# Ruslan361/iterative_solvers

Hardware: AMD Instinct MI355X
Metric: cg_iters_per_sec (higher is better)
Workload: dtype f64; 1 GPU; 4096x4096 L-shaped Dirichlet Poisson fp64, matrix-free CG, fixed 2641 iterations; n=4096, unknowns=12574721, rule=rel2

## Files before the change

### include/mi355cg.h

```cpp
#ifndef MI355CG_H
#define MI355CG_H

#include <stddef.h>

#ifdef __cplusplus
extern "C" {
#endif

#define MI355CG_OK            0
#define MI355CG_ERR_INVALID   1
#define MI355CG_ERR_HIP       2
#define MI355CG_ERR_STATE     3

#define MI355CG_F64           0
#define MI355CG_F32_MIXED     1

#define MI355CG_RULE_MSG_MAXNORM  0
#define MI355CG_RULE_REL_2NORM    1

#define MI355CG_STOP_ITERATIONS   0
#define MI355CG_STOP_PRECISION    1
#define MI355CG_STOP_RESIDUAL     2
#define MI355CG_STOP_EXACT_ERROR  3
#define MI355CG_STOP_INTERRUPTED  4
// ... 3 lines not shown
typedef void (*mi355cg_iter_cb)(void *user, int iteration, double precision, double residual, double error);

typedef struct mi355cg_params {
    int    rule;
    int    max_iterations;
    double eps_precision;
    double eps_residual;
    double eps_exact_error;
    double eps_rel;
    int    use_true_solution;
    int    callback_every;
    int    diagnostics;
    int    sync_every;
    int    fixed_iterations;
    double inner_eps;
} mi355cg_params;

typedef struct mi355cg_results {
    int    iterations;
    int    converged;
    int    stop_reason;
    double final_residual_norm;
    double final_precision;
    double final_error_norm;
    double r_norm2;
    double initial_r_norm2;
    double solve_seconds;
    double refine_true_rel;
    int    refine_outer;
    double loop_seconds;
} mi355cg_results;

int  mi355cg_create(int n, int m, double a, double b, double c, double d,
                    int dtype, int device, mi355cg_handle *out);
int  mi355cg_create_csr(long long nrows, const int *row_map, const int *entries, const double *values,
                        int device, mi355cg_handle *out);
int  mi355cg_set_true_solution(mi355cg_handle h, const double *u);
void mi355cg_destroy(mi355cg_handle h);
const char *mi355cg_last_error(void);
const char *mi355cg_version(void);

long long mi355cg_size(mi355cg_handle h);
int  mi355cg_get_rhs(mi355cg_handle h, double *out);
int  mi355cg_get_true_solution(mi355cg_handle h, double *out);
int  mi355cg_get_node_coords(mi355cg_handle h, double *xs, double *ys);
int  mi355cg_set_rhs(mi355cg_handle h, const double *b);
int  mi355cg_setup_on_device(mi355cg_handle h);

int  mi355cg_apply(mi355cg_handle h, const double *x, double *y);
int  mi355cg_apply_device(mi355cg_handle h, const double *x_dev, double *y_dev);

void mi355cg_default_params(mi355cg_params *p, int rule);
int  mi355cg_solve(mi355cg_handle h, const mi355cg_params *params,
                   mi355cg_iter_cb cb, void *user, const volatile int *stop_flag,
                   mi355cg_results *out);
int  mi355cg_get_solution(mi355cg_handle h, double *x);
int  mi355cg_get_recursive_residual(mi355cg_handle h, double *r);
int  mi355cg_get_true_residual(mi355cg_handle h, double *ax_minus_b);

#define MI355CG_PRECOND_NONE    0
#define MI355CG_PRECOND_MG      1
#define MI355CG_PRECOND_MG_ANY  2
int  mi355cg_set_preconditioner(mi355cg_handle h, int kind);
int  mi355cg_apply_preconditioner(mi355cg_handle h, const double *r, double *z);
int  mi355cg_mg_levels(int n, int *levels, int *coarsest_n);
int  mi355cg_mg_hierarchy(int kind, int n, int max_levels, int *levels, int *level_n);

#define MI355CG_CYCLE_F64 0
#define MI355CG_CYCLE_F32 1
int  mi355cg_set_preconditioner_ex(mi355cg_handle h, int kind, int cycle);
int  mi355cg_preconditioner_info(mi355cg_handle h, int *kind, int *cycle, int *levels);

#define MI355CG_BATCH_MAX 64
int  mi355cg_solve_batch(mi355cg_handle h, const mi355cg_params *params, int nrhs, const double *b, double *x,
                         const volatile int *stop_flag, mi355cg_results *out);
int  mi355cg_solve_batch_device(mi355cg_handle h, const mi355cg_params *params, int nrhs, const double *b_dev, double *x_dev,
                                const volatile int *stop_flag, mi355cg_results *out);
int  mi355cg_batch_release(mi355cg_handle h);

int  mi355cg_set_profiling(mi355cg_handle h, int enable);
int  mi355cg_get_kernel_time(mi355cg_handle h, int kernel, double *avg_ms, long long *launches);
int  mi355cg_get_layout(mi355cg_handle h, long long *padded_len, int *pitch_bottom, int *pitch_upper,
                        int *grid_stencil, int *grid_update, int *rows_per_item);

int  mi355cg_slab_rows(int n, int world, int rank, int *y_lo, int *y_hi);
int  mi355cg_create_part(int n, int m, double a, double b, double c, double d, int dtype, int device,
                         int y_lo, int y_hi, int x_lo, int x_hi, mi355cg_handle *out);
int  mi355cg_checksum(mi355cg_handle h, int which, double *out2);
int  mi355cg_create_slab(int n, int m, double a, double b, double c, double d, int dtype, int device,
                         int y_lo, int y_hi, mi355cg_handle *out);
int  mi355cg_owned_range(mi355cg_handle h, long long *packed_begin, long long *packed_len, int *y_lo, int *y_hi);
int  mi355cg_dist_begin(mi355cg_handle h, const mi355cg_params *params, void *stream);
int  mi355cg_dist_reduce(mi355cg_handle h, int which , int with_rows, void *stream);
int  mi355cg_dist_sums_ptr(mi355cg_handle h, int which, void **dev_ptr, int *count );
int  mi355cg_dist_record_layout(mi355cg_handle h, int *header, int *row_slot, int *width);
int  mi355cg_dist_scatter_ghosts(mi355cg_handle h, int vector ,
                                 const double *gathered_records, int nranks, int rank, void *stream);
int  mi355cg_dist_stencil(mi355cg_handle h, const double *gathered_update_sums, int nranks, int estride,
                          int rows , void *stream);
int  mi355cg_dist_flip(mi355cg_handle h);
int  mi355cg_dist_update(mi355cg_handle h, const double *gathered_stencil_sums, int nranks, int estride,
                         int rows , void *stream);
int  mi355cg_dist_update_reads_ghosts(mi355cg_handle h);
int  mi355cg_dist_check(mi355cg_handle h, const double *gathered_update_sums, int nranks, int estride, void *stream);
int  mi355cg_dist_summary(mi355cg_handle h, mi355cg_results *out, int *done);
int  mi355cg_dist_finish(mi355cg_handle h, void *stream);
int  mi355cg_dist_history(mi355cg_handle h, int iteration, double *precision, double *residual, double *error);
int  mi355cg_dist_halo(mi355cg_handle h, int vector ,
                       void **send_lo, void **recv_lo, long long *n_send_lo,
                       void **send_hi, void **recv_hi, long long *n_send_hi);
int  mi355cg_dist_halo_recv_counts(mi355cg_handle h, long long *n_from_lo, long long *n_from_hi);

#define MI355CG_DECOMP_ROWS 0
#define MI355CG_DECOMP_2D   1
typedef struct mi355cg_team_s *mi355cg_team;
typedef struct mi355cg_halo_msg {
    int id;
    int peer;
    int send;
    int kind;
    int y0, y1, x0, x1;
    long long count;
} mi355cg_halo_msg;
int  mi355cg_decompose(int n, int world, int decomp, int rank, int *y_lo, int *y_hi, int *x_lo, int *x_hi);
int  mi355cg_halo_plan(int n, int world, int decomp, int rank, int max_msgs, int *n_msgs, mi355cg_halo_msg *msgs);
int  mi355cg_debug_plan(int n, int world, int decomp, int rank, int which, int *n_panels, int *panels,
                        int *grid, int *n_items, int *cls);
int  mi355cg_team_create_local(int n, int m, double a, double b, double c, double d, int world,
                               const int *devices, int ndevices, int decomp, mi355cg_team *out);
int  mi355cg_team_unique_id(void *id128);
int  mi355cg_team_create_rccl(int n, int m, double a, double b, double c, double d, int world, int rank, int device,
                              const void *id128, int decomp, mi355cg_team *out);
void mi355cg_team_destroy(mi355cg_team t);
int  mi355cg_team_solve(mi355cg_team t, const mi355cg_params *params, mi355cg_iter_cb cb, void *user,
                        const volatile int *stop_flag, mi355cg_results *out);
int  mi355cg_team_info(mi355cg_team t, int *world, int *nlocal, int *decomp, long long *size);
int  mi355cg_team_describe(mi355cg_team t, char *buf, int len);
int  mi355cg_team_part(mi355cg_team t, int local_index, mi355cg_handle *part, int *rank);
int  mi355cg_team_get_vector(mi355cg_team t, int which, double *global_packed);
int  mi355cg_team_checksum(mi355cg_team t, int which, double *out2);
int  mi355cg_team_set_vector(mi355cg_team t, int which, const double *global_packed);
int  mi355cg_team_set_dtype(mi355cg_team t, int dtype);
int  mi355cg_team_setup_on_device(mi355cg_team t);
int  mi355cg_team_set_profiling(mi355cg_team t, int enable);
int  mi355cg_team_phase_times(mi355cg_team t, double *kernel_ms, double *comm_ms, double *wall_ms);

#ifdef __cplusplus
}
#endif
#endif
```

### iterative_solvers_amd/_capi.py

```python
from __future__ import annotations

import ctypes as C
import os

import numpy as np

from . import build as _build

OK, ERR_INVALID, ERR_HIP, ERR_STATE = 0, 1, 2, 3
F64, F32_MIXED = 0, 1
RULE_MSG_MAXNORM, RULE_REL_2NORM = 0, 1
STOP_ITERATIONS, STOP_PRECISION, STOP_RESIDUAL, STOP_EXACT_ERROR, STOP_INTERRUPTED = range(5)

EXPORTS = [
    "mi355cg_create", "mi355cg_create_csr", "mi355cg_set_true_solution", "mi355cg_destroy", "mi355cg_last_error", "mi355cg_version", "mi355cg_size",
    "mi355cg_get_rhs", "mi355cg_get_true_solution", "mi355cg_get_node_coords", "mi355cg_set_rhs",
    "mi355cg_apply", "mi355cg_apply_device", "mi355cg_default_params", "mi355cg_solve",
    "mi355cg_get_solution", "mi355cg_get_recursive_residual", "mi355cg_get_true_residual",
    "mi355cg_set_profiling", "mi355cg_get_kernel_time", "mi355cg_get_layout",
    "mi355cg_slab_rows", "mi355cg_create_slab", "mi355cg_owned_range", "mi355cg_dist_begin",
    "mi355cg_dist_reduce", "mi355cg_dist_sums_ptr", "mi355cg_dist_record_layout", "mi355cg_dist_scatter_ghosts", "mi355cg_dist_stencil", "mi355cg_dist_flip",
    "mi355cg_dist_update", "mi355cg_dist_update_reads_ghosts", "mi355cg_dist_check", "mi355cg_dist_summary", "mi355cg_dist_finish", "mi355cg_dist_history",
    "mi355cg_dist_halo", "mi355cg_dist_halo_recv_counts",
    "mi355cg_create_part", "mi355cg_checksum", "mi355cg_decompose", "mi355cg_halo_plan",
    "mi355cg_team_create_local", "mi355cg_team_unique_id", "mi355cg_team_create_rccl", "mi355cg_team_destroy",
    "mi355cg_team_solve", "mi355cg_team_info", "mi355cg_team_part", "mi355cg_team_get_vector", "mi355cg_team_set_vector", "mi355cg_team_checksum",
    "mi355cg_team_set_profiling", "mi355cg_team_phase_times", "mi355cg_team_describe", "mi355cg_setup_on_device", "mi355cg_team_setup_on_device", "mi355cg_debug_plan",
    "mi355cg_team_set_dtype", "mi355cg_set_preconditioner", "mi355cg_apply_preconditioner", "mi355cg_mg_levels",
    "mi355cg_mg_hierarchy", "mi355cg_set_preconditioner_ex", "mi355cg_preconditioner_info",
    "mi355cg_solve_batch", "mi355cg_solve_batch_device", "mi355cg_batch_release",
]
DECOMP_ROWS, DECOMP_2D = 0, 1
PRECOND_NONE, PRECOND_MG, PRECOND_MG_ANY = 0, 1, 2
CYCLE_F64, CYCLE_F32 = 0, 1
BATCH_MAX = 64


class Params(C.Structure):
    _fields_ = [("rule", C.c_int), ("max_iterations", C.c_int),
                ("eps_precision", C.c_double), ("eps_residual", C.c_double),
                ("eps_exact_error", C.c_double), ("eps_rel", C.c_double),
                ("use_true_solution", C.c_int), ("callback_every", C.c_int),
                ("diagnostics", C.c_int), ("sync_every", C.c_int), ("fixed_iterations", C.c_int),
                ("inner_eps", C.c_double)]


class Results(C.Structure):
    _fields_ = [("iterations", C.c_int), ("converged", C.c_int), ("stop_reason", C.c_int),
                ("final_residual_norm", C.c_double), ("final_precision", C.c_double),
                ("final_error_norm", C.c_double), ("r_norm2", C.c_double),
                ("initial_r_norm2", C.c_double), ("solve_seconds", C.c_double),
                ("refine_true_rel", C.c_double), ("refine_outer", C.c_int), ("loop_seconds", C.c_double)]


class HaloMsg(C.Structure):
    _fields_ = [("id", C.c_int), ("peer", C.c_int), ("send", C.c_int), ("kind", C.c_int),
                ("y0", C.c_int), ("y1", C.c_int), ("x0", C.c_int), ("x1", C.c_int), ("count", C.c_longlong)]


ITER_CB = C.CFUNCTYPE(None, C.c_void_p, C.c_int, C.c_double, C.c_double, C.c_double)
_DP = np.ctypeslib.ndpointer(dtype=np.float64, flags="C_CONTIGUOUS")

_lib = None


class Mi355cgError(RuntimeError):
    def __init__(self, code: int, text: str):
        super().__init__(f"mi355cg error {code}: {text}")
        self.code = code


def lib_path() -> str:
    return _build.LIB_PATH


def load():
    global _lib
    if _lib is not None:
        return _lib
    path = os.environ.get("MI355CG_LIB") or _build.LIB_PATH
    if path == _build.LIB_PATH and _build.needs_build():
        try:
            _build.build()
        except Exception as e:
            if not os.path.exists(path):
                raise RuntimeError(f"libmi355cg.so is missing and could not be built: {e}") from e
    try:
        import torch
    except ImportError:
        pass
    L = C.CDLL(path)
    H = C.c_void_p
    L.mi355cg_create.argtypes = [C.c_int, C.c_int] + [C.c_double] * 4 + [C.c_int, C.c_int, C.POINTER(H)]
    _IPn = np.ctypeslib.ndpointer(dtype=np.int32, flags="C_CONTIGUOUS")
    L.mi355cg_create_csr.argtypes = [C.c_longlong, _IPn, _IPn, _DP, C.c_int, C.POINTER(H)]
    L.mi355cg_set_true_solution.argtypes = [H, _DP]
    L.mi355cg_destroy.argtypes = [H]
    L.mi355cg_destroy.restype = None
    L.mi355cg_last_error.restype = C.c_char_p
    L.mi355cg_version.restype = C.c_char_p
    L.mi355cg_size.argtypes = [H]
    L.mi355cg_size.restype = C.c_longlong
    for name in ("mi355cg_get_rhs", "mi355cg_get_true_solution", "mi355cg_set_rhs",
                 "mi355cg_get_solution", "mi355cg_get_recursive_residual", "mi355cg_get_true_residual"):
        getattr(L, name).argtypes = [H, _DP]
    L.mi355cg_get_node_coords.argtypes = [H, _DP, _DP]
    L.mi355cg_apply.argtypes = [H, _DP, _DP]
    L.mi355cg_apply_device.argtypes = [H, C.c_void_p, C.c_void_p]
    L.mi355cg_default_params.argtypes = [C.POINTER(Params), C.c_int]
    L.mi355cg_default_params.restype = None
    L.mi355cg_solve.argtypes = [H, C.POINTER(Params), ITER_CB, C.c_void_p, C.c_void_p, C.POINTER(Results)]
    L.mi355cg_set_profiling.argtypes = [H, C.c_int]
    L.mi355cg_get_kernel_time.argtypes = [H, C.c_int, C.POINTER(C.c_double), C.POINTER(C.c_longlong)]
    L.mi355cg_get_layout.argtypes = [H, C.POINTER(C.c_longlong)] + [C.POINTER(C.c_int)] * 5
    LLP, IP, VPP = C.POINTER(C.c_longlong), C.POINTER(C.c_int), C.POINTER(C.c_void_p)
    L.mi355cg_slab_rows.argtypes = [C.c_int, C.c_int, C.c_int, IP, IP]
    L.mi355cg_create_slab.argtypes = [C.c_int, C.c_int] + [C.c_double] * 4 + [C.c_int] * 4 + [C.POINTER(H)]
    L.mi355cg_owned_range.argtypes = [H, LLP, LLP, IP, IP]
    L.mi355cg_dist_begin.argtypes = [H, C.POINTER(Params), C.c_void_p]
    L.mi355cg_dist_reduce.argtypes = [H, C.c_int, C.c_int, C.c_void_p]
    L.mi355cg_dist_sums_ptr.argtypes = [H, C.c_int, VPP, IP]
    L.mi355cg_dist_record_layout.argtypes = [H, IP, IP, IP]
    L.mi355cg_dist_scatter_ghosts.argtypes = [H, C.c_int, C.c_void_p, C.c_int, C.c_int, C.c_void_p]
    L.mi355cg_dist_stencil.argtypes = [H, C.c_void_p, C.c_int, C.c_int, C.c_int, C.c_void_p]
    L.mi355cg_dist_flip.argtypes = [H]
    L.mi355cg_dist_update.argtypes = [H, C.c_void_p, C.c_int, C.c_int, C.c_int, C.c_void_p]
    L.mi355cg_dist_update_reads_ghosts.argtypes = [H]
    L.mi355cg_dist_check.argtypes = [H, C.c_void_p, C.c_int, C.c_int, C.c_void_p]
    L.mi355cg_dist_summary.argtypes = [H, C.POINTER(Results), IP]
    L.mi355cg_dist_finish.argtypes = [H, C.c_void_p]
    DBP = C.POINTER(C.c_double)
    L.mi355cg_dist_history.argtypes = [H, C.c_int, DBP, DBP, DBP]
    L.mi355cg_dist_halo.argtypes = [H, C.c_int, VPP, VPP, LLP, VPP, VPP, LLP]
    L.mi355cg_dist_halo_recv_counts.argtypes = [H, LLP, LLP]
    L.mi355cg_create_part.argtypes = [C.c_int, C.c_int] + [C.c_double] * 4 + [C.c_int] * 6 + [C.POINTER(H)]
    L.mi355cg_checksum.argtypes = [H, C.c_int, DBP]
    L.mi355cg_decompose.argtypes = [C.c_int] * 4 + [IP] * 4
    L.mi355cg_halo_plan.argtypes = [C.c_int] * 5 + [IP, C.POINTER(HaloMsg)]
    L.mi355cg_team_create_local.argtypes = [C.c_int, C.c_int] + [C.c_double] * 4 + [C.c_int, IP, C.c_int, C.c_int, C.POINTER(H)]
    L.mi355cg_team_unique_id.argtypes = [C.c_void_p]
    L.mi355cg_team_create_rccl.argtypes = [C.c_int, C.c_int] + [C.c_double] * 4 + [C.c_int, C.c_int, C.c_int, C.c_void_p, C.c_int, C.POINTER(H)]
    L.mi355cg_team_destroy.argtypes = [H]
    L.mi355cg_team_destroy.restype = None
    L.mi355cg_team_solve.argtypes = [H, C.POINTER(Params), ITER_CB, C.c_void_p, C.c_void_p, C.POINTER(Results)]
    L.mi355cg_team_info.argtypes = [H, IP, IP, IP, LLP]
    L.mi355cg_team_part.argtypes = [H, C.c_int, C.POINTER(H), IP]
    L.mi355cg_team_get_vector.argtypes = [H, C.c_int, _DP]
    L.mi355cg_team_set_vector.argtypes = [H, C.c_int, _DP]
    L.mi355cg_team_checksum.argtypes = [H, C.c_int, DBP]
    L.mi355cg_debug_plan.argtypes = [C.c_int] * 5 + [IP, IP, IP, IP, IP]
    L.mi355cg_setup_on_device.argtypes = [H]
    L.mi355cg_team_setup_on_device.argtypes = [H]
    L.mi355cg_team_set_dtype.argtypes = [H, C.c_int]
    L.mi355cg_team_set_profiling.argtypes = [H, C.c_int]
    L.mi355cg_team_phase_times.argtypes = [H, DBP, DBP, DBP]
    L.mi355cg_team_describe.argtypes = [H, C.c_char_p, C.c_int]
    L.mi355cg_set_preconditioner.argtypes = [H, C.c_int]
    L.mi355cg_set_preconditioner_ex.argtypes = [H, C.c_int, C.c_int]
    L.mi355cg_preconditioner_info.argtypes = [H, IP, IP, IP]
    L.mi355cg_apply_preconditioner.argtypes = [H, _DP, _DP]
    L.mi355cg_mg_levels.argtypes = [C.c_int, IP, IP]
    L.mi355cg_mg_hierarchy.argtypes = [C.c_int, C.c_int, C.c_int, IP, IP]
    L.mi355cg_solve_batch.argtypes = [H, C.POINTER(Params), C.c_int, C.c_void_p, C.c_void_p, C.c_void_p, C.POINTER(Results)]
    L.mi355cg_solve_batch_device.argtypes = [H, C.POINTER(Params), C.c_int, C.c_void_p, C.c_void_p, C.c_void_p, C.POINTER(Results)]
    L.mi355cg_batch_release.argtypes = [H]
    _lib = L
    return L


def check(rc: int):
    if rc != OK:
        raise Mi355cgError(rc, load().mi355cg_last_error().decode("utf-8", "replace"))
```

### iterative_solvers_amd/csrc/cg_kernels.h

```cpp
#pragma once
#include <hip/hip_runtime.h>
#include <cfloat>
#include <cmath>

namespace mi355cg {

constexpr int kBlock = 256;
constexpr int kWave = 64;
constexpr int kWaves = kBlock / kWave;
constexpr int kHist = 512;
constexpr int kMaxPanels = 8;
constexpr int kRing = 8;

#ifdef MI355CG_WAVE_TIMING
constexpr int kWtWaves = 16384, kWtStamps = 6;
__device__ unsigned long long g_wave_dbg[2][kWtStamps * kWtWaves];
#define MI355CG_WT_BEGIN unsigned long long wt_[kWtStamps]; for (int i_ = 0; i_ < kWtStamps; ++i_) wt_[i_] = 0; wt_[0] = wall_clock64();
#define MI355CG_WT_STAMP(I) wt_[I] = wall_clock64();
#define MI355CG_WT_MID wt_[kWtStamps - 2] = wall_clock64();
#define MI355CG_WT_END(K) do { if ((threadIdx.x & 63) == 0) { const int w_ = blockIdx.x * 4 + threadIdx.x / 64; \
    if (w_ < kWtWaves) { wt_[kWtStamps - 1] = wall_clock64(); for (int i_ = 0; i_ < kWtStamps; ++i_) g_wave_dbg[K][kWtStamps * w_ + i_] = wt_[i_]; } } } while (0)
#else
#define MI355CG_WT_BEGIN
#define MI355CG_WT_STAMP(I)
// ... 63 lines not shown
struct RuleParams {
    int rule;
    int max_iterations;
    double eps_precision, eps_residual, eps_exact_error, eps_rel;
    int use_u;
    int fixed_iterations;
};

enum { FA_PAP = 0, FA_RZ = 1, FA_LO = 2, FA_COUNT = 4 };
enum { FB_RR = 0, FB_D2 = 1, FB_E2 = 2, FB_LO = 3, FB_RMAX = 6, FB_DMAX = 7, FB_EMAX = 8, FB_COUNT = 9 };
constexpr int kNumSumsA = 2, kNumSumsB = 3;
constexpr int FB_STOP = FB_COUNT, FB_LL_COUNT = FB_COUNT + 1;

struct dd { double hi, lo; };
__device__ inline dd dd_zero() { return dd{0.0, 0.0}; }
__device__ inline dd two_sum(double a, double b) { const double s = a + b, bb = s - a; return dd{s, (a - (s - bb)) + (b - bb)}; }
__device__ inline dd dd_add(dd a, dd b) {
    const dd s = two_sum(a.hi, b.hi);
    const double lo = s.lo + (a.lo + b.lo);
    const double hi = s.hi + lo;
    return dd{hi, lo - (hi - s.hi)};
}
__device__ inline void dd_acc_prod(dd& acc, double a, double b) {
#ifdef MI355CG_PLAIN_DOT
    acc.hi += a * b;
#elif defined(MI355CG_DOT2)
    const double p = a * b;
    const dd s = two_sum(acc.hi, p);
    acc.hi = s.hi;
    acc.lo += s.lo + fma(a, b, -p);
#else
    const double p = a * b;
    acc = dd_add(acc, dd{p, fma(a, b, -p)});
#endif
}
__device__ inline double dd_value(dd a) { return a.hi + a.lo; }

__device__ inline double wave_sum(double v) {
#pragma unroll
    for (int o = 32; o > 0; o >>= 1) v += __shfl_down(v, o, kWave);
    return v;
}
__device__ inline double wave_max(double v) {
#pragma unroll
    for (int o = 32; o > 0; o >>= 1) v = fmax(v, __shfl_down(v, o, kWave));
    return v;
}
template <bool IS_MAX>
__device__ inline double block_reduce(double v, double* lds ) {
    v = IS_MAX ? wave_max(v) : wave_sum(v);
    const int lane = threadIdx.x & (kWave - 1), w = threadIdx.x / kWave;
    __syncthreads();
    if (lane == 0) lds[w] = v;
    __syncthreads();
    double t = lds[0];
#pragma unroll
    for (int k = 1; k < kWaves; ++k) t = IS_MAX ? fmax(t, lds[k]) : t + lds[k];
    return t;
}
template <bool IS_MAX>
__device__ inline double reduce_parts(const double* __restrict__ part, int n, int es, double* lds) {
    double v = 0.0;
    for (int i = threadIdx.x; i < n; i += kBlock) v = IS_MAX ? fmax(v, part[(long long)i * es]) : v + part[(long long)i * es];
    return block_reduce<IS_MAX>(v, lds);
}

__device__ inline dd wave_sum_dd(dd v) {
#pragma unroll
    for (int o = 32; o > 0; o >>= 1) v = dd_add(v, dd{__shfl_down(v.hi, o, kWave), __shfl_down(v.lo, o, kWave)});
    return v;
}
__device__ inline dd block_reduce_dd(dd v, double* lds) {
    v = wave_sum_dd(v);
    const int lane = threadIdx.x & (kWave - 1), w = threadIdx.x / kWave;
    __syncthreads();
    if (lane == 0) { lds[2 * w] = v.hi; lds[2 * w + 1] = v.lo; }
    __syncthreads();
    dd t{lds[0], lds[1]};
#pragma unroll
    for (int k = 1; k < kWaves; ++k) t = dd_add(t, dd{lds[2 * k], lds[2 * k + 1]});
    return t;
}
struct PreParts { double hi0, lo0, hi1, lo1; };
__device__ inline PreParts prefetch_parts(const double* __restrict__ part_hi, const double* __restrict__ part_lo, int n, int es) {
    PreParts p{0.0, 0.0, 0.0, 0.0};
    const int i0 = threadIdx.x, i1 = threadIdx.x + kBlock;
    if (i0 < n) { p.hi0 = part_hi[(long long)i0 * es]; p.lo0 = part_lo[(long long)i0 * es]; }
    if (i1 < n) { p.hi1 = part_hi[(long long)i1 * es]; p.lo1 = part_lo[(long long)i1 * es]; }
    return p;
}
__device__ inline dd reduce_parts_dd_pre(const PreParts& pre, const double* __restrict__ part_hi, const double* __restrict__ part_lo, int n, int es, double* lds) {
    dd v = dd_zero();
    if ((int)threadIdx.x < n) v = dd_add(v, dd{pre.hi0, pre.lo0});
    if ((int)threadIdx.x + kBlock < n) v = dd_add(v, dd{pre.hi1, pre.lo1});
    for (int i = threadIdx.x + 2 * kBlock; i < n; i += kBlock) v = dd_add(v, dd{part_hi[(long long)i * es], part_lo[(long long)i * es]});
    return block_reduce_dd(v, lds);
}
struct PreMax { double v0, v1; };
__device__ inline PreMax prefetch_max(const double* __restrict__ part, int n, int es) {
    PreMax p{0.0, 0.0};
    if ((int)threadIdx.x < n) p.v0 = part[(long long)threadIdx.x * es];
    if ((int)threadIdx.x + kBlock < n) p.v1 = part[(long long)(threadIdx.x + kBlock) * es];
    return p;
}
template <bool IS_MAX> __device__ inline double block_reduce(double v, double* lds);
__device__ inline double reduce_max_pre(const PreMax& pre, const double* __restrict__ part, int n, int es, double* lds) {
    double v = fmax(pre.v0, pre.v1);
    for (int i = threadIdx.x + 2 * kBlock; i < n; i += kBlock) v = fmax(v, part[(long long)i * es]);
    return block_reduce<true>(v, lds);
}
__device__ inline dd reduce_parts_dd(const double* __restrict__ part_hi, const double* __restrict__ part_lo, int n, int es, double* lds) {
    dd v = dd_zero();
    for (int i = threadIdx.x; i < n; i += kBlock) v = dd_add(v, dd{part_hi[(long long)i * es], part_lo[(long long)i * es]});
    return block_reduce_dd(v, lds);
}

struct Decision { int done, reason, converged; double beta, rr, rnorm2, r0norm, rmax, dmax, emax, d2, e2; };

__device__ inline Decision decide_after_update(const StateLite& s, const RuleParams& rp, double rr, double rmax,
                                               double dmax, double emax, double d2, double e2, bool stop = false) {
    Decision d;
    d.rr = rr; d.rnorm2 = sqrt(rr); d.rmax = rmax; d.dmax = dmax; d.emax = emax; d.d2 = d2; d.e2 = e2;
    d.r0norm = s.first ? d.rnorm2 : s.r0norm;
    d.done = 0; d.reason = 0 ; d.converged = 0; d.beta = 0.0;
    if (rp.rule == 1 ) {
        const bool go = s.it < rp.max_iterations && (rp.fixed_iterations || d.rnorm2 > rp.eps_rel * d.r0norm);
        if (!go) { d.done = 1; d.converged = d.rnorm2 <= rp.eps_rel * d.r0norm; }
        if (!s.first) d.beta = rr / s.rr;
    } else {
        if (s.it >= 1 && !rp.fixed_iterations) {
            if (rp.eps_precision > 0 && dmax < rp.eps_precision) { d.done = 1; d.converged = 1; d.reason = 1; }
            else if (rp.eps_residual > 0 && rmax < rp.eps_residual) { d.done = 1; d.converged = 1; d.reason = 2; }
            else if (rp.eps_exact_error > 0 && rp.use_u && emax < rp.eps_exact_error) { d.done = 1; d.converged = 1; d.reason = 3; }
        }
        if (!d.done && !(s.it < rp.max_iterations)) d.done = 1;
        if (!s.first) d.beta = (d.rnorm2 * d.rnorm2) / s.rz;
    }
    if (!d.done && (stop || s.stop)) { d.done = 1; d.reason = 4 ; d.converged = 0; }
    return d;
}

__device__ inline void write_state_after_decision(CgState* out, HistEntry* hist, const CgState* in, const StateLite& s, const Decision& d) {
    copy_state(out, in);
    CgState* o = out;
    o->rr_prev = s.rr; o->rr = d.rr; o->rnorm2 = d.rnorm2; o->r0norm = d.r0norm; o->beta = d.beta;
    o->rmax = d.rmax; o->dmax = d.dmax; o->emax = d.emax; o->d2 = d.d2; o->e2 = d.e2;
    o->done = d.done; o->reason = d.reason; o->converged = d.converged;
    if (hist) {
        HistEntry* h = hist + (s.it % kHist);
        h->dmax = d.dmax; h->rmax = d.rmax; h->emax = d.emax; h->rnorm2 = d.rnorm2; h->d2 = d.d2; h->e2 = d.e2;
    }
}

__device__ inline Decision reduce_and_decide(const StateLite& s, const RuleParams& rp, const double* partB,
                                             int nB, int strideB, int esB, int want_diag, double* lds, const PreParts* pre_rr = nullptr,
                                             const PreMax* pre_max = nullptr ) {
    const double rr = pre_rr ? dd_value(reduce_parts_dd_pre(*pre_rr, partB + FB_RR * strideB, partB + (FB_RR + FB_LO) * strideB, nB, esB, lds))
                             : dd_value(reduce_parts_dd(partB + FB_RR * strideB, partB + (FB_RR + FB_LO) * strideB, nB, esB, lds));
    double rmax = 0, dmax = 0, emax = 0, d2 = 0, e2 = 0;
    if (rp.rule == 0 || want_diag) {
        if (pre_max) {
            rmax = reduce_max_pre(pre_max[0], partB + FB_RMAX * strideB, nB, esB, lds);
            dmax = reduce_max_pre(pre_max[1], partB + FB_DMAX * strideB, nB, esB, lds);
            if (rp.use_u) emax = reduce_max_pre(pre_max[2], partB + FB_EMAX * strideB, nB, esB, lds);
        } else {
            rmax = reduce_parts<true>(partB + FB_RMAX * strideB, nB, esB, lds);
            dmax = reduce_parts<true>(partB + FB_DMAX * strideB, nB, esB, lds);
            if (rp.use_u) emax = reduce_parts<true>(partB + FB_EMAX * strideB, nB, esB, lds);
        }
    }
    if (want_diag) {
        d2 = dd_value(reduce_parts_dd(partB + FB_D2 * strideB, partB + (FB_D2 + FB_LO) * strideB, nB, esB, lds));
        if (rp.use_u) e2 = dd_value(reduce_parts_dd(partB + FB_E2 * strideB, partB + (FB_E2 + FB_LO) * strideB, nB, esB, lds));
    }
    return decide_after_update(s, rp, rr, rmax, dmax, emax, d2, e2);
}
typedef unsigned long long u64;
constexpr int kRecWords = 16;
// ... 125 lines not shown
    }
    if (a.which == 1) {
#pragma unroll
        for (int k = 0; k < 4; ++k) {
            const double t = block_reduce<true>(mx[k], lds);
            if (threadIdx.x == 0) rec[k < 3 ? FB_RMAX + k : kRecStopWord] = t;
        }
    }
    __syncthreads();
    publish_record(rec, a.rs);
}

__device__ inline Decision decide_from_records(const StateLite& s, const RuleParams& rp, const double* recs, int world, bool use_max, bool want_diag) {
    dd rr = dd_zero(), d2 = dd_zero(), e2 = dd_zero();
    double rmax = 0, dmax = 0, emax = 0, stop = 0;
    for (int j = 0; j < world; ++j) {
        const double* R = recs + j * kRecWords;
        rr = dd_add(rr, dd{R[FB_RR], R[FB_RR + FB_LO]});
        d2 = dd_add(d2, dd{R[FB_D2], R[FB_D2 + FB_LO]});
        e2 = dd_add(e2, dd{R[FB_E2], R[FB_E2 + FB_LO]});
        rmax = fmax(rmax, R[FB_RMAX]); dmax = fmax(dmax, R[FB_DMAX]); emax = fmax(emax, R[FB_EMAX]);
        stop = fmax(stop, R[kRecStopWord]);
    }
    if (!use_max) { rmax = 0; dmax = 0; emax = 0; }
    if (!rp.use_u) { emax = 0; e2 = dd_zero(); }
    if (!want_diag) { d2 = dd_zero(); e2 = dd_zero(); }
    return decide_after_update(s, rp, dd_value(rr), rmax, dmax, emax, dd_value(d2), dd_value(e2), stop > 0.0);
}
__device__ inline void alpha_from_records(const StateLite& s, int rule, const double* recs, int world, double* alpha, double* rz_out) {
    dd pap = dd_zero(), rz = dd_zero();
    for (int j = 0; j < world; ++j) {
        const double* R = recs + j * kRecWords;
        pap = dd_add(pap, dd{R[FA_PAP], R[FA_PAP + FA_LO]});
        rz = dd_add(rz, dd{R[FA_RZ], R[FA_RZ + FA_LO]});
    }
    if (rule == 0) { *rz_out = dd_value(rz); *alpha = *rz_out / dd_value(pap); }
    else { *rz_out = 0.0; *alpha = s.rr / dd_value(pap); }
}
__device__ inline void own_record_B(double* recs, int me, const double* partB, int nB, int strideB, int level, double* lds,
                                    const PreParts* pre_rr = nullptr, const PreMax* pre_max = nullptr) {
    double* R = recs + me * kRecWords;
    if (threadIdx.x < kRecWords) R[threadIdx.x] = 0.0;
    const dd rr = pre_rr ? reduce_parts_dd_pre(*pre_rr, partB + FB_RR * strideB, partB + (FB_RR + FB_LO) * strideB, nB, 1, lds)
                         : reduce_parts_dd(partB + FB_RR * strideB, partB + (FB_RR + FB_LO) * strideB, nB, 1, lds);
    double rmax = 0, dmax = 0, emax = 0;
    dd d2 = dd_zero(), e2 = dd_zero();
    if (level >= 1) {
        if (pre_max) {
            rmax = reduce_max_pre(pre_max[0], partB + FB_RMAX * strideB, nB, 1, lds);
            dmax = reduce_max_pre(pre_max[1], partB + FB_DMAX * strideB, nB, 1, lds);
            emax = reduce_max_pre(pre_max[2], partB + FB_EMAX * strideB, nB, 1, lds);
        } else {
            rmax = reduce_parts<true>(partB + FB_RMAX * strideB, nB, 1, lds);
            dmax = reduce_parts<true>(partB + FB_DMAX * strideB, nB, 1, lds);
            emax = reduce_parts<true>(partB + FB_EMAX * strideB, nB, 1, lds);
        }
    }
    if (level >= 2) {
        d2 = reduce_parts_dd(partB + FB_D2 * strideB, partB + (FB_D2 + FB_LO) * strideB, nB, 1, lds);
        e2 = reduce_parts_dd(partB + FB_E2 * strideB, partB + (FB_E2 + FB_LO) * strideB, nB, 1, lds);
    }
    __syncthreads();
    if (threadIdx.x == 0) {
        R[FB_RR] = rr.hi; R[FB_RR + FB_LO] = rr.lo; R[FB_D2] = d2.hi; R[FB_D2 + FB_LO] = d2.lo; R[FB_E2] = e2.hi; R[FB_E2 + FB_LO] = e2.lo;
        R[FB_RMAX] = rmax; R[FB_DMAX] = dmax; R[FB_EMAX] = emax;
    }
}
__device__ inline void fail_transport(CgState* out, const CgState* in) {
    copy_state(out, in);
    out->done = 1; out->reason = kReasonTransport; out->converged = 0;
}

constexpr int kQueueSubs = 8;
constexpr int kQueuePitch = 64;
struct QueueSpec {
    int* mine;
    int* other;
};
__device__ inline int queue_take(int* q, int lane) {
    int v = 0;
    if (lane == 0) v = __hip_atomic_fetch_add(q, 1, __ATOMIC_RELAXED, __HIP_MEMORY_SCOPE_AGENT);
    return v;
}

template <typename T>
struct StencilArgs {
    Geom g;
    WorkList wl;
    const T* r;
    const T* pin;
    T* pout;
    T* ap;
    const double* partB; int nB, strideB, esB;
    RecSrc src;
    double* partA; int strideA, slotA;
    const CgState* s_in; CgState* s_out;
    HistEntry* hist;
    RuleParams rp;
    int want_diag;
    int store_ghosts;
    FlagSpec fl;
    QueueSpec dq;
};

template <typename T, int VEC> struct VecOf { typedef T type __attribute__((ext_vector_type(VEC))); };

constexpr int kOob = (int)0x80000000;
typedef __amdgpu_buffer_rsrc_t rsrc_t;
__device__ inline rsrc_t make_rsrc(const void* base) {
    return __builtin_amdgcn_make_buffer_rsrc(const_cast<void*>(base), 0, 0x7fffffff, 0x00020000);
}
template <typename V> __device__ inline V buf_load(rsrc_t r, int voff, int soff) {
    if constexpr (sizeof(V) == 16) return __builtin_bit_cast(V, __builtin_amdgcn_raw_buffer_load_b128(r, voff, soff, 0));
    else if constexpr (sizeof(V) == 8) return __builtin_bit_cast(V, __builtin_amdgcn_raw_buffer_load_b64(r, voff, soff, 0));
    else { static_assert(sizeof(V) == 4, "buf_load: 4, 8 or 16 bytes"); return __builtin_bit_cast(V, __builtin_amdgcn_raw_buffer_load_b32(r, voff, soff, 0)); }
}
template <typename V> __device__ inline void buf_store(V v, rsrc_t r, int voff, int soff) {
    typedef unsigned int u4 __attribute__((ext_vector_type(4)));
    typedef unsigned int u2 __attribute__((ext_vector_type(2)));
    if constexpr (sizeof(V) == 16) {
        u4 d = __builtin_bit_cast(u4, v);
        __builtin_amdgcn_raw_buffer_store_b128(d, r, voff, soff, 0);
        asm volatile("s_nop 1" : "+v"(d));
    }
    else if constexpr (sizeof(V) == 8) __builtin_amdgcn_raw_buffer_store_b64(__builtin_bit_cast(u2, v), r, voff, soff, 0);
    else { static_assert(sizeof(V) == 4, "buf_store: 4, 8 or 16 bytes"); __builtin_amdgcn_raw_buffer_store_b32(__builtin_bit_cast(unsigned int, v), r, voff, soff, 0); }
}
__device__ inline int dpp_from_below(int v) { return __builtin_amdgcn_update_dpp(0, v, 0x138 , 0xf, 0xf, false); }
__device__ inline int dpp_from_above(int v) { return __builtin_amdgcn_update_dpp(0, v, 0x130 , 0xf, 0xf, false); }
__device__ inline float lane_below(float v) { return __builtin_bit_cast(float, dpp_from_below(__builtin_bit_cast(int, v))); }
__device__ inline float lane_above(float v) { return __builtin_bit_cast(float, dpp_from_above(__builtin_bit_cast(int, v))); }
__device__ inline double lane_below(double v) {
    const unsigned long long u = __builtin_bit_cast(unsigned long long, v);
    const unsigned lo = (unsigned)dpp_from_below((int)(unsigned)u), hi = (unsigned)dpp_from_below((int)(unsigned)(u >> 32));
    return __builtin_bit_cast(double, ((unsigned long long)hi << 32) | lo);
}
__device__ inline double lane_above(double v) {
    const unsigned long long u = __builtin_bit_cast(unsigned long long, v);
    const unsigned lo = (unsigned)dpp_from_above((int)(unsigned)u), hi = (unsigned)dpp_from_above((int)(unsigned)(u >> 32));
    return __builtin_bit_cast(double, ((unsigned long long)hi << 32) | lo);
}
template <typename T> __device__ inline int row_step(const Geom& g, int y) { return (y + 1 <= g.half ? g.Pb : g.Pu) * (int)sizeof(T); }

template <typename T> __device__ inline int lane_off(const Geom& g, int x, bool bottom_row) {
    return (x < g.xlim && x >= (bottom_row ? g.cb : 0)) ? x * (int)sizeof(T) : kOob;
}
template <typename T, int VEC> __device__ inline int edge_off(const Geom& g, int x, int lane, bool bottom_row) {
    const int xe = lane == 0 ? x - 1 : x + VEC;
    const bool edge = lane == 0 || lane == kWave - 1;
    return (edge && xe >= (bottom_row ? g.cb : 0) && xe < g.xlim) ? xe * (int)sizeof(T) : kOob;
}

struct Item { int strip, ya, yb, gc; };
__device__ inline Item decode_item(const WorkList& wl, int item) {
    Panel P = wl.p[0];
#pragma unroll
    for (int k = 1; k < kMaxPanels; ++k) if (k < wl.np && item >= wl.p[k].item0) P = wl.p[k];
    const int local = item - P.item0;
    const int chunk = local / P.ns;
    Item it;
    it.strip = P.s0 + (local - chunk * P.ns);
    it.ya = P.y0 + chunk * P.ty;
    it.yb = min(P.y1, it.ya + P.ty - 1);
    it.gc = (it.strip == P.s0 ? (P.gc & 1) : 0) | (it.strip == P.s0 + P.ns - 1 ? (P.gc & 2) : 0);
    return it;
}

struct ItemAddr {
    int nrows, ystart;
    long long base_el;
    int so_first, so_c0;
    int gc; bool bot;
    int x;
    int vo_own, ve_own, vo_first, vo_last;
};
template <typename T, int VEC, bool DESC>
__device__ inline ItemAddr item_addr(const Geom& g, const Item& it, int lane) {
    constexpr int DIR = DESC ? -1 : 1;
    ItemAddr A;
    A.x = it.strip * (kWave * VEC) + lane * VEC;
    A.nrows = it.yb - it.ya + 1;
    A.ystart = DESC ? it.yb : it.ya;
    const int y0 = it.ya - 1;
    A.base_el = row_off(g, y0) - g.base0;
    A.bot = it.ya <= g.half;
    A.vo_own = lane_off<T>(g, A.x, A.bot);
    A.ve_own = edge_off<T, VEC>(g, A.x, lane, A.bot);
    A.vo_first = lane_off<T>(g, A.x, A.ystart - DIR <= g.half);
    A.vo_last = lane_off<T>(g, A.x, A.ystart + DIR * A.nrows <= g.half);
    A.so_first = DESC ? (int)((row_off(g, it.yb + 1) - row_off(g, y0)) * (long long)sizeof(T)) : 0;
    A.so_c0 = DESC ? (int)((row_off(g, it.yb) - row_off(g, y0)) * (long long)sizeof(T)) : row_step<T>(g, y0);
    A.gc = it.gc;
    return A;
}

template <typename T, int VEC, bool FUSED, bool MSG, int DEPTH, bool NOAP, bool GC>
__global__ __launch_bounds__(kBlock) void k_stencil(const StencilArgs<T> a) {
    static_assert(DEPTH >= 1 && DEPTH <= 3, "the compute cursor takes its item from the fetch cursor: DEPTH <= rows fetched per item (>= 3)");
    typedef typename VecOf<T, VEC>::type vec_t;
    __shared__ double lds[2 * kWaves];
    const Geom& g = a.g;
    const int lane = threadIdx.x & (kWave - 1);
    const int wave = __builtin_amdgcn_readfirstlane(threadIdx.x / kWave);
    const ItemSeq seq = item_seq(a.wl, wave);
    MI355CG_WT_BEGIN
    struct Raw { vec_t r, p; T re, pe; };

    int f_item = seq.first;
    bool f_have = f_item < seq.end;
    ItemAddr F{};
    int f_idx = 0, f_so = 0, f_y = 0;
    rsrc_t rs_p = make_rsrc(a.pin), rs_r = make_rsrc(a.pin);
    const int dq_nsub = min(kQueueSubs, (int)(gridDim.x / kXcds)), dq_sub = (int)(blockIdx.x / kXcds) % dq_nsub;
    int* const dq = a.dq.mine ? a.dq.mine + ((int)(blockIdx.x % kXcds) * kQueueSubs + dq_sub) * kQueuePitch : nullptr;
    if (a.dq.other && blockIdx.x == 0 && threadIdx.x < kXcds * kQueueSubs) a.dq.other[threadIdx.x * kQueuePitch] = 0;
    int dq_ticket = 0;
    auto enter = [&](int item) {
        if (dq) dq_ticket = queue_take(dq, lane);
        F = item_addr<T, VEC, false>(g, decode_item(a.wl, item), lane);
        rs_p = make_rsrc(a.pin + F.base_el);
        rs_r = make_rsrc(FUSED ? a.r + F.base_el : a.pin + F.base_el);
        f_idx = -1; f_so = F.so_first; f_y = F.ystart - 1;
    };
    auto fetch = [&]() -> Raw {
        if (f_have && f_idx > F.nrows) {
            f_item = dq ? seq.begin + seq.step + __builtin_amdgcn_readfirstlane(dq_ticket) * dq_nsub + dq_sub : f_item + seq.step;
            f_have = f_item < seq.end;
            if (f_have) enter(f_item);
        }
        const bool own = f_idx >= 0 && f_idx < F.nrows;
        int vo = own ? F.vo_own : (f_idx < 0 ? F.vo_first : F.vo_last);
        int ve = own ? F.ve_own : kOob;
        if (!f_have) { vo = kOob; ve = kOob; }
        Raw w;
        w.p = buf_load<vec_t>(rs_p, vo, f_so);
        if (FUSED) w.r = buf_load<vec_t>(rs_r, vo, f_so);
        else for (int j = 0; j < VEC; ++j) w.r[j] = (T)0;
        w.pe = buf_load<T>(rs_p, ve, f_so);
        if (FUSED) w.re = buf_load<T>(rs_r, ve, f_so); else w.re = (T)0;
        f_so += row_step<T>(g, f_y); ++f_y; ++f_idx;
        return w;
    };

    bool c_have = f_have;
    ItemAddr C{};
    int c_idx = -1, c_so = 0, c_y = 0, c_ve_gc = kOob;
    bool in_j[VEC];
#pragma unroll
    for (int j = 0; j < VEC; ++j) in_j[j] = false;
    rsrc_t rs_po = make_rsrc(a.pin), rs_ap = make_rsrc(a.pin);
    auto promote = [&]() {
        C = F;
        rs_po = make_rsrc(FUSED ? a.pout + C.base_el : a.pin + C.base_el);
        rs_ap = make_rsrc(NOAP ? a.pin + C.base_el : a.ap + C.base_el);
        c_idx = -1; c_so = C.so_c0; c_y = C.ystart;
        const int xint0 = C.bot ? g.half + 1 : 1;
#pragma unroll
        for (int j = 0; j < VEC; ++j) in_j[j] = (C.x + j >= xint0) && (C.x + j <= g.N - 1);
        if (GC) c_ve_gc = ((lane == 0 && (C.gc & 1)) || (lane == kWave - 1 && (C.gc & 2))) ? C.ve_own : kOob;
    };

    if (f_have) { enter(f_item); promote(); }
    Raw q[DEPTH];
#pragma unroll
    for (int k = 0; k < DEPTH; ++k) q[k] = fetch();

    T beta = (T)0;
    if (FUSED && a.src.mbox) {
        __shared__ double recs[kMaxRecDst * kRecWords];
        const PreParts pre = prefetch_parts(a.partB + FB_RR * a.strideB, a.partB + (FB_RR + FB_LO) * a.strideB, a.nB, 1);
        PreMax pmax[3] = {{0, 0}, {0, 0}, {0, 0}};
        if (MSG) {
#pragma unroll
            for (int k = 0; k < 3; ++k) pmax[k] = prefetch_max(a.partB + (FB_RMAX + k) * a.strideB, a.nB, 1);
        }
        const StateLite s = load_state_lite(a.s_in);
        if (s.done) {
            if (threadIdx.x == 0) { store_flagged_zero(a.fl, a.slotA + blockIdx.x, FA_COUNT); if (blockIdx.x == 0) copy_state(a.s_out, a.s_in); }
            return;
        }
        MI355CG_WT_STAMP(1)
        own_record_B(recs, a.src.me, a.partB, a.nB, a.strideB, MSG ? 1 : 0, lds, &pre, MSG ? pmax : nullptr);
        if (!gather_records(a.src, recs)) {
            if (threadIdx.x == 0) { store_flagged_zero(a.fl, a.slotA + blockIdx.x, FA_COUNT); if (blockIdx.x == 0) fail_transport(a.s_out, a.s_in); }
            return;
        }
        const Decision d = decide_from_records(s, a.rp, recs, a.src.world, MSG, false);
        MI355CG_WT_STAMP(2)
        if (blockIdx.x == 0 && threadIdx.x == 0) write_state_after_decision(a.s_out, a.hist, a.s_in, s, d);
        if (d.done) { if (threadIdx.x == 0) store_flagged_zero(a.fl, a.slotA + blockIdx.x, FA_COUNT); return; }
        beta = (T)d.beta;
    } else if (FUSED) {
        const PreParts pre = prefetch_parts(a.partB + FB_RR * a.strideB, a.partB + (FB_RR + FB_LO) * a.strideB, a.nB, a.esB);
        PreMax pmax[3] = {{0, 0}, {0, 0}, {0, 0}};
        if (MSG) {
#pragma unroll
            for (int k = 0; k < 3; ++k) pmax[k] = prefetch_max(a.partB + (FB_RMAX + k) * a.strideB, a.nB, a.esB);
        }
        const StateLite s = load_state_lite(a.s_in);
        if (s.done) { if (blockIdx.x == 0 && threadIdx.x == 0) copy_state(a.s_out, a.s_in); return; }
        MI355CG_WT_STAMP(1)
        const Decision d = reduce_and_decide(s, a.rp, a.partB, a.nB, a.strideB, a.esB, a.want_diag, lds, &pre, MSG ? pmax : nullptr);
        MI355CG_WT_STAMP(2)
        if (blockIdx.x == 0 && threadIdx.x == 0) write_state_after_decision(a.s_out, a.hist, a.s_in, s, d);
        if (d.done) return;
        beta = (T)d.beta;
    }

    MI355CG_WT_MID
    const T cA = (T)g.A, cxk = (T)g.xk, cyk = (T)g.yk;
    dd acc_pap = dd_zero(), acc_rz = dd_zero();
    auto is_ghost = [&](int yy) { return (yy == g.y_lo - 1 || yy == g.y_hi + 1) && yy >= 1 && yy <= g.N - 1; };
    vec_t pn_b, pn_c, r_c;
    T pne_c = (T)0;
#pragma unroll
    for (int j = 0; j < VEC; ++j) { pn_b[j] = (T)0; pn_c[j] = (T)0; r_c[j] = (T)0; }

    while (c_have) {
#pragma unroll
        for (int k = 0; k < DEPTH; ++k) {
            if (c_have) {
                const Raw w = q[k];
                q[k] = fetch();
                vec_t pn; T pne;
                if (FUSED) {
#pragma unroll
                    for (int j = 0; j < VEC; ++j) pn[j] = w.r[j] + beta * w.p[j];
                    pne = w.re + beta * w.pe;
                } else { pn = w.p; pne = w.pe; }

                if (c_idx < 0) {
                    pn_b = pn;
                    if (FUSED && a.store_ghosts && is_ghost(C.ystart - 1)) buf_store(pn, rs_po, C.vo_first, C.so_first);
                } else if (c_idx == 0) {
                    pn_c = pn; pne_c = pne; r_c = w.r;
                } else {
                    T left0 = lane_below(pn_c[VEC - 1]);
                    T rightL = lane_above(pn_c[0]);
                    if (lane == 0) left0 = pne_c;
                    if (lane == kWave - 1) rightL = pne_c;
                    vec_t out;
#pragma unroll
                    for (int j = 0; j < VEC; ++j) {
                        const T c = pn_c[j];
                        const T L = j == 0 ? left0 : pn_c[j - 1];
                        const T R = j == VEC - 1 ? rightL : pn_c[j + 1];
                        T v = cA * c;
                        v = v + cxk * L;
                        v = v + cxk * R;
                        v = v + cyk * pn[j];
                        v = v + cyk * pn_b[j];
                        out[j] = in_j[j] ? v : (T)0;
                        dd_acc_prod(acc_pap, (double)c, (double)out[j]);
                        if (MSG) dd_acc_prod(acc_rz, (double)r_c[j], (double)c);
                    }
                    if (!NOAP) buf_store(out, rs_ap, C.vo_own, c_so);
                    if (FUSED) buf_store(pn_c, rs_po, C.vo_own, c_so);
                    if (FUSED && GC) buf_store(pne_c, rs_po, c_ve_gc, c_so);
                    c_so += row_step<T>(g, c_y); ++c_y;
                    pn_b = pn_c; pn_c = pn; pne_c = pne; r_c = w.r;
                }
                if (c_idx == C.nrows) {
                    if (FUSED && a.store_ghosts && is_ghost(c_y)) buf_store(pn, rs_po, C.vo_last, c_so);
                    c_have = f_have;
                    if (c_have) promote();
                } else ++c_idx;
            }
        }
    }

    MI355CG_WT_END(0);
    const dd tp = block_reduce_dd(acc_pap, lds);
    dd tz = dd_zero();
    if (MSG) tz = block_reduce_dd(acc_rz, lds);
    if (threadIdx.x == 0 && a.partA) {
        const int b = a.slotA + blockIdx.x, st = a.strideA;
        a.partA[FA_PAP * st + b] = tp.hi; a.partA[(FA_PAP + FA_LO) * st + b] = tp.lo;
        a.partA[FA_RZ * st + b] = tz.hi;  a.partA[(FA_RZ + FA_LO) * st + b] = tz.lo;
        if (FUSED && a.fl.part) { const double v[FA_COUNT] = {tp.hi, tz.hi, tp.lo, tz.lo}; store_flagged(a.fl, b, FA_COUNT, v); }
    }
}

template <typename T>
struct UpdateArgs {
    long long begin, nvec;
    T* x; T* r; const T* p; const T* ap; const T* u;
    const double* partA; int nA, strideA, esA;
    double* partB; int strideB;
    const CgState* s_in; CgState* s_out;
    int rule;
    int init;
    double r0norm_resume;
};

template <typename T, int VEC, bool HAS_U>
__global__ __launch_bounds__(kBlock) void k_update(const UpdateArgs<T> a) {
    typedef typename VecOf<T, VEC>::type vec_t;
    __shared__ double lds[2 * kWaves];
    StateLite s{};
    double alpha_d = 0.0, rz = 0.0;
    if (a.init == 1) {
        s.first = 1; s.it = 0;
    } else if (a.init == 2) {
        s = load_state_lite(a.s_in);
    } else {
        s = load_state_lite(a.s_in);
        if (s.done) { if (blockIdx.x == 0 && threadIdx.x == 0) copy_state(a.s_out, a.s_in); return; }
        const double pap = dd_value(reduce_parts_dd(a.partA + FA_PAP * a.strideA, a.partA + (FA_PAP + FA_LO) * a.strideA, a.nA, a.esA, lds));
        if (a.rule == 0) {
            rz = dd_value(reduce_parts_dd(a.partA + FA_RZ * a.strideA, a.partA + (FA_RZ + FA_LO) * a.strideA, a.nA, a.esA, lds));
            alpha_d = rz / pap;
        } else {
            alpha_d = s.rr / pap;
        }
    }
    const T alpha = (T)alpha_d;

    dd s_rr = dd_zero(), s_d2 = dd_zero(), s_e2 = dd_zero();
    double s_rmax = 0, s_dmax = 0, s_emax = 0;
    const long long stride = (long long)gridDim.x * kBlock;
    vec_t* __restrict__ X = reinterpret_cast<vec_t*>(a.x);
    vec_t* __restrict__ R = reinterpret_cast<vec_t*>(a.r);
    const vec_t* __restrict__ Pp = reinterpret_cast<const vec_t*>(a.p);
    const vec_t* __restrict__ Q = reinterpret_cast<const vec_t*>(a.ap);
    const vec_t* __restrict__ Uu = reinterpret_cast<const vec_t*>(a.u);

    auto elem = [&](long long i, const vec_t& x0, const vec_t& pv, const vec_t& r0, const vec_t& qv, const vec_t& uv) {
        vec_t xn, rn;
#pragma unroll
        for (int j = 0; j < VEC; ++j) {
            xn[j] = x0[j] + alpha * pv[j];
            rn[j] = r0[j] - alpha * qv[j];
            const double rd = (double)rn[j];
            dd_acc_prod(s_rr, rd, rd);
            s_rmax = fmax(s_rmax, fabs(rd));
            const double dx = (double)(xn[j] - x0[j]);
            s_dmax = fmax(s_dmax, fabs(dx));
            dd_acc_prod(s_d2, dx, dx);
            if (HAS_U) {
                const double ee = (double)(xn[j] - uv[j]);
                s_emax = fmax(s_emax, fabs(ee));
                dd_acc_prod(s_e2, ee, ee);
            }
        }
        X[i] = xn; R[i] = rn;
    };
    long long i = a.begin + (long long)blockIdx.x * kBlock + threadIdx.x;
    const long long end = a.begin + a.nvec;
    for (; i + stride < end; i += 2 * stride) {
        const long long j0 = i, j1 = i + stride;
        const vec_t xa = X[j0], pa = Pp[j0], ra = R[j0], qa = Q[j0];
        const vec_t xb = X[j1], pb = Pp[j1], rb = R[j1], qb = Q[j1];
        vec_t ua{}, ub{}; if (HAS_U) { ua = Uu[j0]; ub = Uu[j1]; }
        elem(j0, xa, pa, ra, qa, ua);
        elem(j1, xb, pb, rb, qb, ub);
    }
    if (i < end) {
        const vec_t x0 = X[i], pv = Pp[i], r0 = R[i], qv = Q[i];
        vec_t uv{}; if (HAS_U) uv = Uu[i];
        elem(i, x0, pv, r0, qv, uv);
    }

    const dd t_rr = block_reduce_dd(s_rr, lds);
// ... 16 lines not shown
            } else {
                copy_state(a.s_out, a.s_in);
                if (a.init == 2) {
                    if (s.done) o->rr = s.rr_prev;
                    o->done = 0; o->reason = 0; o->converged = 0; o->alpha = 0.0; o->r0norm = a.r0norm_resume;
                    for (int i = 0; i < kRing; ++i) o->alpha_hist[i] = 0.0;
                } else { o->it = s.it + 1; o->first = 0; o->alpha = alpha_d; o->rz = rz; o->alpha_hist[(s.it + 1) & (kRing - 1)] = alpha_d; }
            }
        }
    }
}

template <typename T>
struct FreshArgs {
    long long begin, nvec;
    const T* b; T* x; T* r; T* p0; const T* u;
    double* partB; int strideB;
    CgState* s_out;
};
template <typename T, int VEC, bool HAS_U>
__global__ __launch_bounds__(kBlock) void k_init_fresh(const FreshArgs<T> a) {
    typedef typename VecOf<T, VEC>::type vec_t;
    __shared__ double lds[2 * kWaves];
    dd s_rr = dd_zero(), s_e2 = dd_zero();
    double s_rmax = 0, s_emax = 0;
    const long long stride = (long long)gridDim.x * kBlock;
    const vec_t* __restrict__ B = reinterpret_cast<const vec_t*>(a.b);
    const vec_t* __restrict__ Uu = reinterpret_cast<const vec_t*>(a.u);
    vec_t* __restrict__ X = reinterpret_cast<vec_t*>(a.x);
    vec_t* __restrict__ R = reinterpret_cast<vec_t*>(a.r);
    vec_t* __restrict__ P = reinterpret_cast<vec_t*>(a.p0);
    vec_t zero;
#pragma unroll
    for (int j = 0; j < VEC; ++j) zero[j] = (T)0;
    const long long end = a.begin + a.nvec;
    for (long long i = a.begin + (long long)blockIdx.x * kBlock + threadIdx.x; i < end; i += stride) {
        const vec_t bv = B[i];
        vec_t uv; if (HAS_U) uv = Uu[i];
#pragma unroll
        for (int j = 0; j < VEC; ++j) {
            const double rd = (double)bv[j];
            dd_acc_prod(s_rr, rd, rd);
            s_rmax = fmax(s_rmax, fabs(rd));
            if (HAS_U) {
                const double ee = (double)((T)0 - uv[j]);
                s_emax = fmax(s_emax, fabs(ee));
                dd_acc_prod(s_e2, ee, ee);
            }
        }
        X[i] = zero; R[i] = bv; P[i] = zero;
    }
    const dd t_rr = block_reduce_dd(s_rr, lds);
    const double t_rmax = block_reduce<true>(s_rmax, lds);
    double t_emax = 0; dd t_e2 = dd_zero();
    if (HAS_U) { t_emax = block_reduce<true>(s_emax, lds); t_e2 = block_reduce_dd(s_e2, lds); }
    if (threadIdx.x == 0) {
        const int b = blockIdx.x, st = a.strideB;
        a.partB[FB_RR * st + b] = t_rr.hi; a.partB[(FB_RR + FB_LO) * st + b] = t_rr.lo;
        a.partB[FB_D2 * st + b] = 0.0; a.partB[(FB_D2 + FB_LO) * st + b] = 0.0;
        a.partB[FB_E2 * st + b] = t_e2.hi; a.partB[(FB_E2 + FB_LO) * st + b] = t_e2.lo;
        a.partB[FB_RMAX * st + b] = t_rmax; a.partB[FB_DMAX * st + b] = 0.0; a.partB[FB_EMAX * st + b] = t_emax;
        if (blockIdx.x == 0) { *a.s_out = CgState{}; a.s_out->first = 1; }
    }
}

template <typename T>
struct UpdateStArgs {
    Geom g;
    WorkList wl;
    const T* p;
    const T* pprev[kRing - 1];
    T* r; T* x; const T* u;
    const double* partA; int nA, strideA, esA;
    RecSrc src;
    double* partB; int strideB, slotB;
    const CgState* s_in; CgState* s_out;
    int rule;
    int reverse;
    const int* stop_req;
    FlagSpec fl;
    QueueSpec dq;
};

template <typename T, int VEC, int XM, bool HAS_U, int DEPTH, bool DESC>
__global__ __launch_bounds__(kBlock) void k_update_st(const UpdateStArgs<T> a) {
    static_assert(DEPTH >= 1 && DEPTH <= 3, "see k_stencil");
    typedef typename VecOf<T, VEC>::type vec_t;
    __shared__ double lds[2 * kWaves];
    const Geom& g = a.g;
    const int lane = threadIdx.x & (kWave - 1);
    const int wave = __builtin_amdgcn_readfirstlane(threadIdx.x / kWave);
    const ItemSeq seq = item_seq(a.wl, wave);
    MI355CG_WT_BEGIN
    int stop_word = 0;
    if (blockIdx.x == 0 && a.stop_req) stop_word = scalar_load(a.stop_req);
    constexpr bool FULL = XM == 1;
    constexpr int NP = XM >= 2 ? XM - 1 : 0;
    struct Raw { vec_t p, r, x, u, pp[NP > 0 ? NP : 1]; T pe; };

    int f_item = seq.first;
    bool f_have = f_item < seq.end;
    ItemAddr F{};
    int f_idx = 0, f_so = 0, f_y = 0;
    rsrc_t rs_p = make_rsrc(a.p), rs_r = rs_p, rs_x = rs_p, rs_u = rs_p;
    rsrc_t rs_pp[NP > 0 ? NP : 1] = {rs_p};
    const int dq_nsub = min(kQueueSubs, (int)(gridDim.x / kXcds)), dq_sub = (int)(blockIdx.x / kXcds) % dq_nsub;
    int* const dq = a.dq.mine ? a.dq.mine + ((int)(blockIdx.x % kXcds) * kQueueSubs + dq_sub) * kQueuePitch : nullptr;
    if (a.dq.other && blockIdx.x == 0 && threadIdx.x < kXcds * kQueueSubs) a.dq.other[threadIdx.x * kQueuePitch] = 0;
    int dq_ticket = 0;
    auto enter = [&](int idx) {
        if (dq) dq_ticket = queue_take(dq, lane);
        F = item_addr<T, VEC, DESC>(g, decode_item(a.wl, a.reverse ? seq.end - 1 - (idx - seq.begin) : idx), lane);
        rs_p = make_rsrc(a.p + F.base_el);
        rs_r = make_rsrc(a.r + F.base_el);
        rs_x = make_rsrc(XM != 0 ? a.x + F.base_el : a.p + F.base_el);
#pragma unroll
        for (int i = 0; i < NP; ++i) rs_pp[i] = make_rsrc(a.pprev[i] + F.base_el);
        rs_u = make_rsrc((FULL && HAS_U) ? a.u + F.base_el : a.p + F.base_el);
        f_idx = -1; f_so = F.so_first; f_y = DESC ? F.ystart + 1 : F.ystart - 1;
    };
    auto fetch = [&]() -> Raw {
        if (f_have && f_idx > F.nrows) {
            f_item = dq ? seq.begin + seq.step + __builtin_amdgcn_readfirstlane(dq_ticket) * dq_nsub + dq_sub : f_item + seq.step;
            f_have = f_item < seq.end;
            if (f_have) enter(f_item);
        }
        const bool own = f_have && f_idx >= 0 && f_idx < F.nrows;
        int vo = own ? F.vo_own : (f_idx < 0 ? F.vo_first : F.vo_last);
        if (!f_have) vo = kOob;
        const int vown = own ? F.vo_own : kOob;
        Raw w;
        w.p = buf_load<vec_t>(rs_p, vo, f_so);
        w.r = buf_load<vec_t>(rs_r, vown, f_so);
        if (XM != 0) w.x = buf_load<vec_t>(rs_x, vown, f_so);
#pragma unroll
        for (int i = 0; i < NP; ++i) w.pp[i] = buf_load<vec_t>(rs_pp[i], vown, f_so);
        if (FULL && HAS_U) w.u = buf_load<vec_t>(rs_u, vown, f_so);
        w.pe = buf_load<T>(rs_p, own ? F.ve_own : kOob, f_so);
        if (DESC) { f_so -= row_step<T>(g, f_y - 1); --f_y; } else { f_so += row_step<T>(g, f_y); ++f_y; }
        ++f_idx;
        return w;
    };

    bool c_have = f_have;
    ItemAddr C{};
    int c_idx = -1, c_so = 0, c_y = 0;
    bool in_j[VEC];
#pragma unroll
    for (int j = 0; j < VEC; ++j) in_j[j] = false;
    rsrc_t rs_ro = rs_p, rs_xo = rs_p;
    auto promote = [&]() {
        C = F;
        rs_ro = make_rsrc(a.r + C.base_el);
        rs_xo = make_rsrc(XM != 0 ? a.x + C.base_el : a.p + C.base_el);
        c_idx = -1; c_so = C.so_c0; c_y = C.ystart;
        const int xint0 = C.bot ? g.half + 1 : 1;
#pragma unroll
        for (int j = 0; j < VEC; ++j) in_j[j] = (C.x + j >= xint0) && (C.x + j <= g.N - 1);
    };

    if (f_have) { enter(f_item); promote(); }
    Raw q[DEPTH];
#pragma unroll
    for (int k = 0; k < DEPTH; ++k) q[k] = fetch();

    double alpha_d, rz = 0.0;
    StateLite s;
    if (a.src.mbox) {
        __shared__ double recs[kMaxRecDst * kRecWords];
        const PreParts pre = prefetch_parts(a.partA + FA_PAP * a.strideA, a.partA + (FA_PAP + FA_LO) * a.strideA, a.nA, 1);
        PreParts pre_rz{0, 0, 0, 0};
        if (FULL) pre_rz = prefetch_parts(a.partA + FA_RZ * a.strideA, a.partA + (FA_RZ + FA_LO) * a.strideA, a.nA, 1);
        s = load_state_lite(a.s_in);
        if (s.done) {
            if (threadIdx.x == 0) { store_flagged_zero(a.fl, a.slotB + blockIdx.x, FB_LL_COUNT); if (blockIdx.x == 0) copy_state(a.s_out, a.s_in); }
            return;
        }
        {
            double* R = recs + a.src.me * kRecWords;
            if (threadIdx.x < kRecWords) R[threadIdx.x] = 0.0;
            const dd pap = reduce_parts_dd_pre(pre, a.partA + FA_PAP * a.strideA, a.partA + (FA_PAP + FA_LO) * a.strideA, a.nA, 1, lds);
            dd rzd = dd_zero();
            if (a.rule == 0) rzd = FULL ? reduce_parts_dd_pre(pre_rz, a.partA + FA_RZ * a.strideA, a.partA + (FA_RZ + FA_LO) * a.strideA, a.nA, 1, lds)
                                        : reduce_parts_dd(a.partA + FA_RZ * a.strideA, a.partA + (FA_RZ + FA_LO) * a.strideA, a.nA, 1, lds);
            __syncthreads();
            if (threadIdx.x == 0) { R[FA_PAP] = pap.hi; R[FA_PAP + FA_LO] = pap.lo; R[FA_RZ] = rzd.hi; R[FA_RZ + FA_LO] = rzd.lo; }
        }
        if (!gather_records(a.src, recs)) {
            if (threadIdx.x == 0) { store_flagged_zero(a.fl, a.slotB + blockIdx.x, FB_LL_COUNT); if (blockIdx.x == 0) fail_transport(a.s_out, a.s_in); }
            return;
        }
        alpha_from_records(s, a.rule, recs, a.src.world, &alpha_d, &rz);
    } else {
        const PreParts pre = prefetch_parts(a.partA + FA_PAP * a.strideA, a.partA + (FA_PAP + FA_LO) * a.strideA, a.nA, a.esA);
        PreParts pre_rz{0, 0, 0, 0};
        if (FULL) pre_rz = prefetch_parts(a.partA + FA_RZ * a.strideA, a.partA + (FA_RZ + FA_LO) * a.strideA, a.nA, a.esA);
        s = load_state_lite(a.s_in);
        if (s.done) { if (blockIdx.x == 0 && threadIdx.x == 0) copy_state(a.s_out, a.s_in); return; }
        const double pap = dd_value(reduce_parts_dd_pre(pre, a.partA + FA_PAP * a.strideA, a.partA + (FA_PAP + FA_LO) * a.strideA, a.nA, a.esA, lds));
        if (a.rule == 0) {
            rz = FULL ? dd_value(reduce_parts_dd_pre(pre_rz, a.partA + FA_RZ * a.strideA, a.partA + (FA_RZ + FA_LO) * a.strideA, a.nA, a.esA, lds))
                      : dd_value(reduce_parts_dd(a.partA + FA_RZ * a.strideA, a.partA + (FA_RZ + FA_LO) * a.strideA, a.nA, a.esA, lds));
            alpha_d = rz / pap;
        } else {
            alpha_d = s.rr / pap;
        }
    }
    const T alpha = (T)alpha_d;
    MI355CG_WT_MID
    T aprev[NP > 0 ? NP : 1] = {(T)0};
#pragma unroll
    for (int i = 0; i < NP; ++i) aprev[i] = (T)scalar_load(&a.s_in->alpha_hist[(s.it - i) & (kRing - 1)]);
    const T cA = (T)g.A, cxk = (T)g.xk, cyk = (T)g.yk;
    dd s_rr = dd_zero(), s_d2 = dd_zero(), s_e2 = dd_zero();
    double s_rmax = 0, s_dmax = 0, s_emax = 0;
    vec_t p_b;
    Raw c;
#pragma unroll
    for (int j = 0; j < VEC; ++j) { p_b[j] = (T)0; c.p[j] = (T)0; c.r[j] = (T)0; c.x[j] = (T)0; c.u[j] = (T)0; for (int i = 0; i < (NP > 0 ? NP : 1); ++i) c.pp[i][j] = (T)0; }
    c.pe = (T)0;

    while (c_have) {
#pragma unroll
        for (int k = 0; k < DEPTH; ++k) {
            if (c_have) {
                const Raw w = q[k];
                q[k] = fetch();
                if (c_idx < 0) {
                    p_b = w.p;
                } else if (c_idx == 0) {
                    c = w;
                } else {
                    T left0 = lane_below(c.p[VEC - 1]);
                    T rightL = lane_above(c.p[0]);
                    if (lane == 0) left0 = c.pe;
                    if (lane == kWave - 1) rightL = c.pe;
                    const vec_t& top = DESC ? p_b : w.p;
                    const vec_t& bot = DESC ? w.p : p_b;
                    vec_t rn, xn;
#pragma unroll
                    for (int j = 0; j < VEC; ++j) {
                        const T cc = c.p[j];
                        const T L = j == 0 ? left0 : c.p[j - 1];
                        const T R = j == VEC - 1 ? rightL : c.p[j + 1];
                        T v = cA * cc;
                        v = v + cxk * L;
                        v = v + cxk * R;
                        v = v + cyk * top[j];
                        v = v + cyk * bot[j];
                        const T apj = in_j[j] ? v : (T)0;
                        rn[j] = c.r[j] - alpha * apj;
                        const double rd = (double)rn[j];
                        dd_acc_prod(s_rr, rd, rd);
                        s_rmax = fmax(s_rmax, fabs(rd));
                        if (XM >= 2) {
                            T t = c.x[j];
#pragma unroll
                            for (int i = NP - 1; i >= 0; --i) t = t + aprev[i] * c.pp[i][j];
                            xn[j] = t + alpha * cc;
                        }
                        if (FULL) {
                            xn[j] = c.x[j] + alpha * cc;
                            const double dx = (double)(xn[j] - c.x[j]);
                            s_dmax = fmax(s_dmax, fabs(dx));
                            dd_acc_prod(s_d2, dx, dx);
                            if (HAS_U) {
                                const double ee = (double)(xn[j] - c.u[j]);
                                s_emax = fmax(s_emax, fabs(ee));
                                dd_acc_prod(s_e2, ee, ee);
                            }
                        }
                    }
                    buf_store(rn, rs_ro, C.vo_own, c_so);
                    if (XM != 0) buf_store(xn, rs_xo, C.vo_own, c_so);
                    if (DESC) { c_so -= row_step<T>(g, c_y - 1); --c_y; } else { c_so += row_step<T>(g, c_y); ++c_y; }
                    p_b = c.p; c = w;
                }
                if (c_idx == C.nrows) {
                    c_have = f_have;
                    if (c_have) promote();
                } else ++c_idx;
            }
        }
    }

    MI355CG_WT_END(1);
    const dd t_rr = block_reduce_dd(s_rr, lds);
    const double t_rmax = block_reduce<true>(s_rmax, lds);
    double t_dmax = 0, t_emax = 0; dd t_d2 = dd_zero(), t_e2 = dd_zero();
    if (FULL) { t_dmax = block_reduce<true>(s_dmax, lds); t_d2 = block_reduce_dd(s_d2, lds); }
    if (FULL && HAS_U) { t_emax = block_reduce<true>(s_emax, lds); t_e2 = block_reduce_dd(s_e2, lds); }
    if (threadIdx.x == 0) {
        const int b = a.slotB + blockIdx.x, st = a.strideB;
        a.partB[FB_RR * st + b] = t_rr.hi; a.partB[(FB_RR + FB_LO) * st + b] = t_rr.lo;
        a.partB[FB_D2 * st + b] = t_d2.hi; a.partB[(FB_D2 + FB_LO) * st + b] = t_d2.lo;
        a.partB[FB_E2 * st + b] = t_e2.hi; a.partB[(FB_E2 + FB_LO) * st + b] = t_e2.lo;
        a.partB[FB_RMAX * st + b] = t_rmax; a.partB[FB_DMAX * st + b] = t_dmax; a.partB[FB_EMAX * st + b] = t_emax;
        if (a.fl.part) {
            const double v[FB_LL_COUNT] = {t_rr.hi, t_d2.hi, t_e2.hi, t_rr.lo, t_d2.lo, t_e2.lo, t_rmax, t_dmax, t_emax, (blockIdx.x == 0 && stop_word) ? 1.0 : 0.0};
            store_flagged(a.fl, b, FB_LL_COUNT, v);
        }
        if (blockIdx.x == 0) {
            copy_state(a.s_out, a.s_in);
            CgState* o = a.s_out;
            o->it = s.it + 1; o->first = 0; o->alpha = alpha_d; o->rz = rz; o->alpha_hist[(s.it + 1) & (kRing - 1)] = alpha_d;
            o->stop = stop_word != 0;
        }
    }
}

struct CheckArgs {
    const double* partB; int nB, strideB, esB;
    RecSrc src;
    const CgState* s_in;
    CgState* summary;
    HistEntry* hist;
    RuleParams rp;
    int want_diag;
};
__global__ __launch_bounds__(kBlock) void k_check(const CheckArgs a) {
    __shared__ double lds[2 * kWaves];
    const StateLite s = load_state_lite(a.s_in);
    if (s.done) { if (threadIdx.x == 0) copy_state(a.summary, a.s_in); return; }
    Decision d;
    if (a.src.mbox) {
        __shared__ double recs[kMaxRecDst * kRecWords];
        own_record_B(recs, a.src.me, a.partB, a.nB, a.strideB, 2, lds);
        if (!gather_records(a.src, recs)) { if (threadIdx.x == 0) fail_transport(a.summary, a.s_in); return; }
        d = decide_from_records(s, a.rp, recs, a.src.world, true, true);
    } else d = reduce_and_decide(s, a.rp, a.partB, a.nB, a.strideB, a.esB, 1, lds);
    if (threadIdx.x == 0) write_state_after_decision(a.summary, a.hist, a.s_in, s, d);
}

template <typename T> struct FlushArgs { const T* p[kRing - 1]; T a[kRing - 1]; int n; };
template <typename T, int VEC>
__global__ __launch_bounds__(kBlock) void k_flush_x(const Geom g, const WorkList wl, T* x, const FlushArgs<T> f) {
    typedef typename VecOf<T, VEC>::type vec_t;
    const int lane = threadIdx.x & (kWave - 1);
    const int wave = __builtin_amdgcn_readfirstlane(threadIdx.x / kWave);
    for (int item = blockIdx.x * kWaves + wave; item < wl.nitems; item += gridDim.x * kWaves) {
        const Item it = decode_item(wl, item);
        const int x0 = it.strip * (kWave * VEC) + lane * VEC;
        if (x0 < (it.ya <= g.half ? g.cb : 0) || x0 >= g.xlim) continue;
        for (int y = it.ya; y <= it.yb; ++y) {
            const long long off = row_off(g, y) - g.base0 + x0;
            vec_t xn = *reinterpret_cast<const vec_t*>(x + off);
#pragma unroll
            for (int k = 0; k < kRing - 1; ++k) if (k < f.n) {
                const vec_t pv = *reinterpret_cast<const vec_t*>(f.p[k] + off);
#pragma unroll
                for (int j = 0; j < VEC; ++j) xn[j] = xn[j] + f.a[k] * pv[j];
            }
            *reinterpret_cast<vec_t*>(x + off) = xn;
        }
    }
}

template <typename T, int VEC>
__global__ __launch_bounds__(kBlock) void k_checksum(const Geom g, const WorkList wl, const T* v, double* part) {
    typedef typename VecOf<T, VEC>::type vec_t;
    __shared__ double lds[2 * kWaves];
    const int lane = threadIdx.x & (kWave - 1);
    const int wave = __builtin_amdgcn_readfirstlane(threadIdx.x / kWave);
    dd s1 = dd_zero(), s2 = dd_zero();
    for (int item = blockIdx.x * kWaves + wave; item < wl.nitems; item += gridDim.x * kWaves) {
        const Item it = decode_item(wl, item);
        const int x0 = it.strip * (kWave * VEC) + lane * VEC;
        if (x0 < (it.ya <= g.half ? g.cb : 0) || x0 >= g.xlim) continue;
        for (int y = it.ya; y <= it.yb; ++y) {
            const vec_t t = *reinterpret_cast<const vec_t*>(v + (row_off(g, y) - g.base0 + x0));
#pragma unroll
            for (int j = 0; j < VEC; ++j) { s1 = dd_add(s1, dd{(double)t[j], 0.0}); dd_acc_prod(s2, (double)t[j], (double)t[j]); }
        }
    }
    const dd t1 = block_reduce_dd(s1, lds), t2 = block_reduce_dd(s2, lds);
    if (threadIdx.x == 0) {
        const int n = gridDim.x, b = blockIdx.x;
        part[b] = t1.hi; part[n + b] = t1.lo; part[2 * n + b] = t2.hi; part[3 * n + b] = t2.lo;
    }
}

template <typename T>
__global__ __launch_bounds__(kBlock) void k_err_maxnorm(long long begin, long long len, const T* x, const T* u, double* part) {
    __shared__ double lds[2 * kWaves];
    const long long stride = (long long)gridDim.x * kBlock;
    double m = 0.0;
    for (long long i = begin + (long long)blockIdx.x * kBlock + threadIdx.x; i < begin + len; i += stride)
        m = fmax(m, fabs((double)(x[i] - u[i])));
    const double t = block_reduce<true>(m, lds);
    if (threadIdx.x == 0) part[blockIdx.x] = t;
}
// ... 130 lines not shown
```

### iterative_solvers_amd/csrc/mi355cg.hip

```cpp
#include "../../include/mi355cg.h"
#include "cg_kernels.h"
#include "csr_kernels.h"
#include "grid_setup.h"
#include "mg_kernels.h"
#include "mg_batch_kernels.h"
#include "mg_kernels_f32.h"

#include <algorithm>
#include <cfloat>
#include <chrono>
#include <cstdarg>
#include <cstdint>
#include <cstdio>
#include <cstdlib>
#include <cstring>
#include <string>
#include <thread>
#include <vector>

using namespace mi355cg;

namespace {

thread_local std::string g_err;
// ... 39 lines not shown
struct MgLevel32 { float *rhs = nullptr, *a = nullptr, *out = nullptr; MgCoef32 c{}; float scale = 0.f; int vec = 1; };
struct MgHier {
    int kind = 0;
    int cycle = MI355CG_CYCLE_F64;
    std::vector<MgLevel> lv;
    std::vector<MgLevel32> lv32;
    float* inv32 = nullptr;
    int ncoarse = 0;
    double* inv = nullptr;
    int* coff = nullptr;
    double *z = nullptr, *p[2] = {nullptr, nullptr}, *q = nullptr;
    double* part = nullptr;
    double* part_h = nullptr;
};

struct MgBatchLevel { long long rhs = -1, a = -1, out = -1; };
struct MgBatchWs {
    int cap = 0;
    long long stride = 0;
    double* base = nullptr;
    long long x = 0, r = 0, z = 0, p[2] = {0, 0}, q = 0;
    std::vector<MgBatchLevel> lv;
    double* part = nullptr;
    double* red = nullptr;
    double* red_h = nullptr;
    double* stage = nullptr;
    int stage_cap = 0;
};

}

struct mi355cg_ctx {
    int device = 0;
    int dtype = MI355CG_F64;
    hipStream_t stream = nullptr;
    GridParams gp;
    Geom g{};
    int s_lo = 0, s_hi = 0;
    long long storage_len = 0;
    long long pk_begin = 0, pk_len = 0;
    PackGeom pg{};
    Plan whole, interior, edge;
    Plan whole32;
    int depth = 2;
    bool has_gc = false;
    int nB_own = 0;
    int strideA = 0, strideB = 0;

    double *x = nullptr, *r = nullptr, *p[kRing] = {}, *ap = nullptr, *b = nullptr, *u = nullptr;
    int xsteps = 4;
    double* scratch[2] = {nullptr, nullptr};
    float *xf = nullptr, *rf = nullptr, *pf[kRing] = {}, *apf = nullptr;
    double* packed = nullptr;
    double *partA = nullptr, *partB = nullptr, *partR = nullptr;
    double *sumsA = nullptr, *sumsB = nullptr;
    int rec_width = 0;
    mi355cg_params dist_prm{};
    bool dist_active = false, is_slab = false;
    CgState *sA = nullptr, *sB = nullptr, *summary = nullptr;
    int* qctr = nullptr;
    int dyn_rows = 0;
    int* stop_h = nullptr;
    int* stop_dev = nullptr;
    HistEntry* hist = nullptr;
    CgState* summary_h = nullptr;
    HistEntry* hist_h = nullptr;
    double* partR_h = nullptr;

    std::vector<double> rhs_h, u_h;
    bool host_rhs_valid = true, host_u_valid = true;
    bool have_u_dev = false, solved = false;
    bool is_csr = false;
    long long csr_n = 0, csr_nnz = 0;
    int *csr_row_map = nullptr, *csr_entries = nullptr; double* csr_values = nullptr;
    int grid_csr = 0, grid_update = 0;
    int cur = 0;
    int nA_dist = 0;

    struct ChunkGraph { int m, cur; std::vector<char> flags; hipGraphExec_t exec; };
    std::vector<ChunkGraph> graphs;
    mi355cg_params graph_prm{};
    bool graph_stop = false;
    int use_graph = -1;

    hipEvent_t ev_loop[2] = {nullptr, nullptr};
    MgHier* mg = nullptr;
    MgBatchWs* batch = nullptr;
    bool profiling = false;
    EventPool events;
    std::vector<std::pair<hipEvent_t, hipEvent_t>> ev_pairs[2];
    double kernel_ms[2] = {0, 0};
    long long kernel_launches[2] = {0, 0};
};

namespace {

long long phys_start(const Geom& g, int y) { return row_off(g, y) + (y <= g.half ? g.cb : 0); }
long long phys_end(const Geom& g, int y) { return phys_start(g, y) + (y <= g.half ? g.Pb : g.Pu); }
int strips_total(const GridParams& gp, int vec) { return (gp.n - 1) / (kWave * vec) + 1; }
int first_bottom_strip(const GridParams& gp, int vec) { return (gp.half + 1) / (kWave * vec); }

void own_cols(const mi355cg_ctx* c, int y, int* xa, int* xb) {
    const int lo = y <= c->gp.half ? c->gp.half + 1 : 1, hi = c->gp.n;
    *xa = std::max(lo, c->s_lo * kStripCols);
    *xb = std::max(*xa, std::min(hi, c->s_hi * kStripCols));
}

void build_geom(mi355cg_ctx* c, int vec, int y_lo, int y_hi) {
    Geom& g = c->g;
    const GridParams& gp = c->gp;
    g.N = gp.n; g.half = gp.half;
    g.Pu = (int)round_up(g.N + 1, 32);
    g.cb = g.half & ~31;
    g.Pb = g.Pu - g.cb;
    g.xlim = (int)round_up(g.N + 1, vec);
    g.y_lo = y_lo; g.y_hi = y_hi;
    g.base0 = 0;
    g.base0 = phys_start(g, y_lo - 1);
    c->storage_len = phys_end(g, y_hi + 1) - g.base0;
    g.own_begin = phys_start(g, y_lo) - g.base0;
    g.own_len = phys_end(g, y_hi) - phys_start(g, y_lo);
    g.A = gp.A; g.xk = gp.x_k; g.yk = gp.y_k;
    PackGeom& pg = c->pg;
    pg.g = g;
    const int yb0 = y_lo, yb1 = std::min(y_hi, gp.half), yu0 = std::max(y_lo, gp.half + 1), yu1 = y_hi;
    int xa = 0, xb = 0;
    pg.nb_rows = std::max(0, yb1 - yb0 + 1); pg.yb0 = yb0;
    own_cols(c, gp.half, &xa, &xb); pg.xb0 = xa; pg.wb = pg.nb_rows ? xb - xa : 0;
    pg.nu_rows = std::max(0, yu1 - yu0 + 1); pg.yu0 = yu0;
    own_cols(c, gp.half + 1, &xa, &xb); pg.xu0 = xa; pg.wu = pg.nu_rows ? xb - xa : 0;
    pg.pk_len = (long long)pg.nb_rows * pg.wb + (long long)pg.nu_rows * pg.wu;
    c->pk_len = pg.pk_len;
    c->pk_begin = packed_row_begin(gp, y_lo);
}

struct Rect { int y0, y1, s0, s1, gc; };
int region_rects(const GridParams& gp, int vec, int ya, int yb, int sa, int sb, Rect out[2]) {
    const int ns_all = strips_total(gp, vec), s0b = first_bottom_strip(gp, vec);
    int nr = 0;
    sb = std::min(sb, ns_all);
    if (ya <= gp.half && yb >= 1) {
        const int s0 = std::max(sa, s0b);
        if (s0 < sb) out[nr++] = Rect{std::max(ya, 1), std::min(yb, gp.half), s0, sb, (sa > s0b ? 1 : 0) | (sb < ns_all ? 2 : 0)};
    }
    if (yb > gp.half && sa < sb)
        out[nr++] = Rect{std::max(ya, gp.half + 1), std::min(yb, gp.n - 1), sa, sb, (sa > 0 ? 1 : 0) | (sb < ns_all ? 2 : 0)};
    return nr;
}

long long add_panel(WorkList& wl, int y0, int y1, int s0, int s1, int ty, int gc) {
    const int rows = y1 - y0 + 1, ns = s1 - s0;
    if (rows <= 0 || ns <= 0) return 0;
    if (ty <= 0) return (long long)rows * ns;
    if (wl.np >= kMaxPanels) return 0;
    Panel& P = wl.p[wl.np++];
    P.y0 = y0; P.y1 = y1; P.s0 = s0; P.ns = ns; P.gc = gc;
    P.nchunks = (rows + ty - 1) / ty;
    P.ty = (rows + P.nchunks - 1) / P.nchunks;
    P.nchunks = (rows + P.ty - 1) / P.ty;
    P.item0 = wl.nitems;
    wl.nitems += P.ns * P.nchunks;
    return (long long)rows * ns;
}

Plan make_plan(const std::vector<Rect>& rects, int max_rows, int fixed_ty = 0, int dyn_rows = 0) {
    Plan pl{};
    const int target_waves = std::max(kWaves, env_int("MI355CG_WAVES", 2048));
    const int max_blocks = std::max(1, env_int("MI355CG_BLOCKS", 512));
    const int waves = std::min(target_waves, max_blocks * kWaves);
    const long long item_rows = std::max(1, env_int("MI355CG_ITEM_ROWS", max_rows));
    long long strip_rows = 0;
    WorkList dry{};
    for (auto& r : rects) strip_rows += add_panel(dry, r.y0, r.y1, r.s0, r.s1, 0, 0);
    if (strip_rows == 0) return pl;
    const bool classes = env_int("MI355CG_XCD_CLASSES", 1) != 0 && fixed_ty == 0 && max_blocks >= kXcds && strip_rows >= 4LL * waves;
    auto build = [&](int ty) {
        WorkList wl{};
        wl.ncls = 1;
        for (auto& r : rects) add_panel(wl, r.y0, r.y1, r.s0, r.s1, ty, r.gc);
        if (classes) {
            wl.ncls = kXcds;
            for (int k = 0; k <= kXcds; ++k) wl.cls0[k] = (int)((long long)wl.nitems * k / kXcds);
        }
        return wl;
    };
    auto fits = [&](const WorkList& wl, long long rounds) {
        if (wl.ncls == kXcds) { for (int k = 0; k < kXcds; ++k) if (wl.cls0[k + 1] - wl.cls0[k] > rounds * (waves / kXcds)) return false; return true; }
        return wl.nitems <= rounds * waves;
    };
    int ty = fixed_ty;
    if (ty <= 0 && dyn_rows > 0 && classes) {
        ty = dyn_rows;
        pl.wl = build(ty);
    } else if (ty <= 0) {
        const long long rounds = std::max<long long>(1, (strip_rows + waves * item_rows - 1) / (waves * item_rows));
        ty = (int)std::max<long long>(std::min<long long>(8, item_rows), (strip_rows + rounds * waves - 1) / (rounds * waves));
        for (int tries = 0; tries < 64; ++tries) {
            pl.wl = build(ty);
            if (fits(pl.wl, rounds)) break;
            ++ty;
        }
    } else {
        pl.wl = build(ty);
    }
    pl.ty = ty;
    pl.grid = std::max(1, std::min(max_blocks, (pl.wl.nitems + kWaves - 1) / kWaves));
    if (pl.wl.ncls == kXcds) pl.grid = std::min(max_blocks / kXcds * kXcds, (pl.grid + kXcds - 1) / kXcds * kXcds);
    return pl;
}
constexpr int kMaxRowsF64 = 800, kMaxRowsF32 = 64;

void build_plans(mi355cg_ctx* c) {
    const Geom& g = c->g;
    const GridParams& gp = c->gp;
    Rect rr[2];
    const int nr = region_rects(gp, 2, g.y_lo, g.y_hi, c->s_lo, c->s_hi, rr);
    std::vector<Rect> whole(rr, rr + nr);
    c->whole = make_plan(whole, kMaxRowsF64);
    c->dyn_rows = std::max(0, env_int("MI355CG_DYN_ROWS", c->whole.ty >= 96 ? 16 : 0));
    if (c->dyn_rows > 0) {
        const Plan dyn = make_plan(whole, kMaxRowsF64, 0, c->dyn_rows);
        if (dyn.wl.ncls == kXcds && dyn.wl.nitems >= 2 * kWaves * dyn.grid) c->whole = dyn; else c->dyn_rows = 0;
    }
    c->has_gc = false;
    for (auto& r : whole) if (r.gc) c->has_gc = true;
    std::vector<Rect> inner, rows, cols;
    for (auto& r : whole) {
        const int yi0 = std::max(r.y0, g.y_lo + 1), yi1 = std::min(r.y1, g.y_hi - 1);
        const int si0 = r.s0 + ((r.gc & 1) ? 1 : 0), si1 = r.s1 - ((r.gc & 2) ? 1 : 0);
        if (r.y0 <= g.y_lo && g.y_lo <= r.y1) rows.push_back(Rect{g.y_lo, g.y_lo, r.s0, r.s1, r.gc});
        if (g.y_hi > g.y_lo && r.y0 <= g.y_hi && g.y_hi <= r.y1) rows.push_back(Rect{g.y_hi, g.y_hi, r.s0, r.s1, r.gc});
        if (yi0 > yi1) continue;
        if (si0 < si1) inner.push_back(Rect{yi0, yi1, si0, si1, 0});
        if (si0 >= si1) { cols.push_back(Rect{yi0, yi1, r.s0, r.s1, r.gc}); continue; }
        if (r.gc & 1) cols.push_back(Rect{yi0, yi1, r.s0, r.s0 + 1, 1});
        if (r.gc & 2) cols.push_back(Rect{yi0, yi1, r.s1 - 1, r.s1, 2});
    }
    c->interior = make_plan(inner, kMaxRowsF64);
    Plan e_rows = make_plan(rows, kMaxRowsF64, 1), e_cols = make_plan(cols, kMaxRowsF64, c->interior.ty > 0 ? c->interior.ty : 0);
    c->edge = e_rows;
    c->edge.wl.ncls = 1;
    for (int k = 0; k < e_cols.wl.np && c->edge.wl.np < kMaxPanels; ++k) {
        Panel P = e_cols.wl.p[k];
        P.item0 = c->edge.wl.nitems;
        c->edge.wl.p[c->edge.wl.np++] = P;
        c->edge.wl.nitems += P.ns * P.nchunks;
    }
    c->edge.grid = std::max(1, std::min(std::max(1, env_int("MI355CG_BLOCKS", 512)), (c->edge.wl.nitems + kWaves - 1) / kWaves));
    if (c->edge.wl.nitems == 0) c->edge.grid = 0;
    if (c->dtype == MI355CG_F32_MIXED || (c->s_lo == 0 && c->s_hi == strips_total(gp, 2))) {
        Rect r4[2];
        const int n4 = region_rects(gp, 4, g.y_lo, g.y_hi, 0, strips_total(gp, 4), r4);
        c->whole32 = make_plan(std::vector<Rect>(r4, r4 + n4), kMaxRowsF32);
    }
    c->depth = env_int("MI355CG_DEPTH", 3) == 2 ? 2 : 3;
    c->use_graph = env_int("MI355CG_GRAPH", -1);
    c->nB_own = c->whole.grid;
}

int flat_grid(long long n) { return (int)std::max<long long>(1, std::min<long long>(2048, (n + kBlock - 1) / kBlock)); }

struct PartSrc { const double* ptr; int n, fstride, estride; RecSrc rec; };
struct Where { hipStream_t stream; const Plan* plan; int slot; };

Where whole_part(const mi355cg_ctx* c) { return Where{c->stream, &c->whole, 0}; }
PartSrc own_partB(const mi355cg_ctx* c) { return PartSrc{c->partB, c->nB_own, c->strideB, 1}; }
PartSrc own_partA(const mi355cg_ctx* c) { return PartSrc{c->partA, c->whole.grid, c->strideA, 1}; }

template <typename T, int VEC> Geom kernel_geom(const mi355cg_ctx* c) { Geom g = c->g; g.xlim = (int)round_up(c->g.N + 1, VEC); return g; }

template <typename T, int VEC>
void launch_apply(const mi355cg_ctx* c, const T* v, T* out, const Where& w) {
    if (w.plan->wl.nitems == 0) return;
    StencilArgs<T> a{};
    a.g = kernel_geom<T, VEC>(c); a.wl = w.plan->wl;
    a.pin = v; a.ap = out; a.partA = nullptr;
    hipLaunchKernelGGL((k_stencil<T, VEC, false, false, 2, false, false>), dim3(w.plan->grid), dim3(kBlock), 0, w.stream, a);
}

struct IterCfg { RuleParams rp; int want_diag; bool has_u; bool x2 = false; };

template <typename T, int VEC>
void launch_iteration_stencil(mi355cg_ctx* c, const IterCfg& cfg, const T* r, T* const p[kRing], const Where& w, const PartSrc& pb, const FlagSpec* fl = nullptr) {
    if (w.plan->wl.nitems == 0) return;
    StencilArgs<T> a{};
    a.g = kernel_geom<T, VEC>(c); a.wl = w.plan->wl;
    a.r = r; a.pin = p[c->cur]; a.pout = p[(c->cur + 1) % c->xsteps]; a.ap = nullptr;
    a.partB = pb.ptr; a.nB = pb.n; a.strideB = pb.fstride; a.esB = pb.estride; a.src = pb.rec;
    a.partA = c->partA; a.strideA = c->strideA; a.slotA = w.slot;
    a.s_in = c->sB; a.s_out = c->sA; a.hist = c->hist; a.rp = cfg.rp; a.want_diag = cfg.want_diag;
    a.store_ghosts = c->is_slab ? 1 : 0;
    if (fl) a.fl = *fl;
    if (VEC == 2 && c->dyn_rows > 0 && w.plan == &c->whole) a.dq = QueueSpec{c->qctr, c->qctr + kXcds * kQueueSubs * kQueuePitch};
    const dim3 grid(w.plan->grid), block(kBlock);
    const bool msg = cfg.rp.rule == MI355CG_RULE_MSG_MAXNORM, gc = c->has_gc, d3 = c->depth == 3;
#define MI355CG_ST(MSG, D, GC) hipLaunchKernelGGL((k_stencil<T, VEC, true, MSG, D, true, GC>), grid, block, 0, w.stream, a)
    if constexpr (VEC == 2) {
        if (msg) { if (gc) { if (d3) MI355CG_ST(true, 3, true); else MI355CG_ST(true, 2, true); } else { if (d3) MI355CG_ST(true, 3, false); else MI355CG_ST(true, 2, false); } }
        else     { if (gc) { if (d3) MI355CG_ST(false, 3, true); else MI355CG_ST(false, 2, true); } else { if (d3) MI355CG_ST(false, 3, false); else MI355CG_ST(false, 2, false); } }
    } else {
        if (d3) MI355CG_ST(false, 3, false); else MI355CG_ST(false, 2, false);
    }
#undef MI355CG_ST
}

template <typename T, int VEC>
void launch_iteration_update(mi355cg_ctx* c, const IterCfg& cfg, T* x, T* r, T* const p[kRing], const T* u, const Where& w, const PartSrc& pa, const FlagSpec* fl = nullptr) {
    if (w.plan->wl.nitems == 0) return;
    UpdateStArgs<T> a{};
    a.g = kernel_geom<T, VEC>(c); a.wl = w.plan->wl;
    a.p = p[c->cur]; a.r = r; a.x = x; a.u = u;
    for (int i = 0; i < kRing - 1; ++i) a.pprev[i] = p[(c->cur + 2 * kRing * c->xsteps - 1 - i) % c->xsteps];
    a.partA = pa.ptr; a.nA = pa.n; a.strideA = pa.fstride; a.esA = pa.estride; a.src = pa.rec;
    a.partB = c->partB; a.strideB = c->strideB; a.slotB = w.slot;
    a.s_in = c->sA; a.s_out = c->sB; a.rule = cfg.rp.rule; a.reverse = 1;
    if (fl) a.fl = *fl;
    if (VEC == 2 && c->dyn_rows > 0 && w.plan == &c->whole) a.dq = QueueSpec{c->qctr + kXcds * kQueueSubs * kQueuePitch, c->qctr};
    a.stop_req = w.slot == 0 ? c->stop_dev : nullptr;
    const dim3 grid(w.plan->grid), block(kBlock);
    const bool d3 = c->depth == 3 && !(cfg.x2 && c->cur == 0 && c->xsteps == 8);
#define MI355CG_UST(XM, HASU) do { if (d3) hipLaunchKernelGGL((k_update_st<T, VEC, XM, HASU, 3, true>), grid, block, 0, w.stream, a); \
                                   else hipLaunchKernelGGL((k_update_st<T, VEC, XM, HASU, 2, true>), grid, block, 0, w.stream, a); } while (0)
    if (cfg.x2) {
        if (c->cur != 0) MI355CG_UST(0, false); else if (c->xsteps == 8) MI355CG_UST(8, false); else if (c->xsteps == 4) MI355CG_UST(4, false); else MI355CG_UST(2, false);
    }
    else if constexpr (VEC == 2) { if (cfg.has_u) MI355CG_UST(1, true); else MI355CG_UST(1, false); }
#undef MI355CG_UST
}

template <typename T, int VEC>
void launch_update_flat(mi355cg_ctx* c, const IterCfg& cfg, T* x, T* r, const T* p, const T* ap, const T* u, hipStream_t stream,
                        int grid, double resume_r0norm = -1.0) {
    UpdateArgs<T> a{};
    a.begin = c->g.own_begin / VEC; a.nvec = c->g.own_len / VEC;
    a.x = x; a.r = r; a.p = p; a.ap = ap; a.u = u;
    a.partA = c->partA; a.nA = 0; a.strideA = c->strideA; a.esA = 1;
    a.partB = c->partB; a.strideB = c->strideB;
    a.s_in = c->sA; a.s_out = c->sB; a.rule = cfg.rp.rule; a.init = 1;
    if (resume_r0norm >= 0.0) { a.init = 2; a.r0norm_resume = resume_r0norm; a.s_in = c->sB; }
    if (cfg.has_u) hipLaunchKernelGGL((k_update<T, VEC, true>), dim3(grid), dim3(kBlock), 0, stream, a);
    else hipLaunchKernelGGL((k_update<T, VEC, false>), dim3(grid), dim3(kBlock), 0, stream, a);
}

template <typename T, int VEC>
void launch_flush_x(const mi355cg_ctx* c, const Plan& plan, T* x, T* const p[kRing], const CgState& fin, hipStream_t stream) {
    const int pending = fin.it % c->xsteps;
    if (plan.wl.nitems == 0 || pending == 0) return;
    FlushArgs<T> f{};
    f.n = pending;
    for (int j = 0; j < pending; ++j) { const int k = fin.it - pending + 1 + j; f.p[j] = p[k % c->xsteps]; f.a[j] = (T)fin.alpha_hist[k & (kRing - 1)]; }
    hipLaunchKernelGGL((k_flush_x<T, VEC>), dim3(std::max(1, std::min(1024, (plan.wl.nitems + kWaves - 1) / kWaves))), dim3(kBlock), 0, stream,
                       kernel_geom<T, VEC>(c), plan.wl, x, f);
}

void launch_check(mi355cg_ctx* c, const IterCfg& cfg, hipStream_t stream, const PartSrc& pb) {
    CheckArgs a{};
    a.partB = pb.ptr; a.nB = pb.n; a.strideB = pb.fstride; a.esB = pb.estride; a.src = pb.rec;
    a.s_in = c->sB; a.summary = c->summary; a.hist = c->hist; a.rp = cfg.rp; a.want_diag = cfg.want_diag;
    hipLaunchKernelGGL(k_check, dim3(1), dim3(kBlock), 0, stream, a);
}

IterCfg make_cfg(const mi355cg_params* prm) {
    IterCfg cfg{};
    const bool msg = prm->rule == MI355CG_RULE_MSG_MAXNORM;
    cfg.rp.rule = prm->rule; cfg.rp.max_iterations = prm->max_iterations;
    cfg.rp.eps_precision = prm->eps_precision; cfg.rp.eps_residual = prm->eps_residual;
    cfg.rp.eps_exact_error = prm->eps_exact_error; cfg.rp.eps_rel = prm->eps_rel;
    cfg.rp.fixed_iterations = prm->fixed_iterations;
    const bool diag = !msg && prm->diagnostics;
    cfg.has_u = (msg && prm->use_true_solution) || diag;
    cfg.rp.use_u = cfg.has_u ? 1 : 0;
    cfg.want_diag = diag ? 1 : 0;
    cfg.x2 = !msg && !diag;
    return cfg;
}

template <typename T>
int upload_packed(mi355cg_ctx* c, const double* host_packed, T* storage) {
    if (c->is_csr) {
        HIPCK(hipMemcpyAsync(storage, host_packed, sizeof(double) * c->pk_len, hipMemcpyHostToDevice, c->stream));
        HIPCK(hipStreamSynchronize(c->stream));
        return MI355CG_OK;
    }
    if (c->is_slab) HIPCK(hipDeviceSynchronize());
    if (c->pk_len == 0) return MI355CG_OK;
    HIPCK(hipMemcpyAsync(c->packed, host_packed, sizeof(double) * c->pk_len, hipMemcpyHostToDevice, c->stream));
    hipLaunchKernelGGL((k_unpack<T>), dim3(flat_grid(c->pk_len)), dim3(kBlock), 0, c->stream, c->pg, c->packed, storage);
    HIPCK(hipGetLastError());
    HIPCK(hipStreamSynchronize(c->stream));
    return MI355CG_OK;
}
template <typename T>
int download_packed(mi355cg_ctx* c, const T* storage, double* host_packed) {
    if (c->is_csr) {
        HIPCK(hipMemcpyAsync(host_packed, storage, sizeof(double) * c->pk_len, hipMemcpyDeviceToHost, c->stream));
        HIPCK(hipStreamSynchronize(c->stream));
        return MI355CG_OK;
    }
    if (c->is_slab) HIPCK(hipDeviceSynchronize());
    if (c->pk_len == 0) return MI355CG_OK;
    hipLaunchKernelGGL((k_pack<T>), dim3(flat_grid(c->pk_len)), dim3(kBlock), 0, c->stream, c->pg, storage, c->packed);
    HIPCK(hipGetLastError());
    HIPCK(hipMemcpyAsync(host_packed, c->packed, sizeof(double) * c->pk_len, hipMemcpyDeviceToHost, c->stream));
    HIPCK(hipStreamSynchronize(c->stream));
    return MI355CG_OK;
}

int alloc_vec(double** p, long long n) {
    HIPCK(hipMalloc((void**)p, sizeof(double) * n));
    HIPCK(hipMemset(*p, 0, sizeof(double) * n));
    return MI355CG_OK;
}

int ensure_host_copies(mi355cg_ctx* c) {
    if (!c->host_rhs_valid) { c->rhs_h.resize(c->pk_len); if (int rc = download_packed<double>(c, c->b, c->rhs_h.data())) return rc; c->host_rhs_valid = true; }
    if (!c->host_u_valid) { c->u_h.resize(c->pk_len); if (int rc = download_packed<double>(c, c->u, c->u_h.data())) return rc; c->host_u_valid = true; }
    return MI355CG_OK;
}
int ensure_f32_vectors(mi355cg_ctx* c) {
    if (c->xsteps > 4) return fail(MI355CG_ERR_INVALID, "MI355CG_XSTEPS=8 is fp64 only");
    if (c->whole32.wl.nitems == 0) return fail(MI355CG_ERR_INVALID, "the fp32 kernels march 256-column strips: a part of a 2-D decomposition (cut on 128 columns) cannot run them; use row slabs");
    if (c->g.own_begin % 4 != 0 || c->g.own_len % 4 != 0) return fail(MI355CG_ERR_STATE, "a part's owned range is not a whole number of float4");
    float** fv[] = {&c->xf, &c->apf, &c->pf[0], &c->pf[1], &c->pf[2], &c->pf[3]};
    for (int k = 0; k < 2 + c->xsteps; ++k) {
        if (*fv[k]) continue;
        if (hipMalloc((void**)fv[k], sizeof(float) * c->storage_len) != hipSuccess || hipMemset(*fv[k], 0, sizeof(float) * c->storage_len) != hipSuccess)
            return fail(MI355CG_ERR_HIP, "fp32 vector allocation failed");
    }
    HIPCK(hipDeviceSynchronize());
    return MI355CG_OK;
}

int ensure_u_on_device(mi355cg_ctx* c) {
    if (c->have_u_dev) return MI355CG_OK;
    if (!c->host_u_valid) return fail(MI355CG_ERR_STATE, "no exact solution on host or device");
    if (int rc = upload_packed<double>(c, c->u_h.data(), c->u)) return rc;
    c->have_u_dev = true;
    return MI355CG_OK;
}
int ensure_scratch(mi355cg_ctx* c) {
    for (auto& s : c->scratch) if (!s) { if (int rc = alloc_vec(&s, c->storage_len)) return rc; }
    HIPCK(hipDeviceSynchronize());
// ... 819 lines not shown
    if (nrhs < 1 || nrhs > MI355CG_BATCH_MAX) return fail(MI355CG_ERR_INVALID, "a batch has 1 .. %d right-hand sides, not %d", MI355CG_BATCH_MAX, nrhs);
    if (prm->rule != MI355CG_RULE_MSG_MAXNORM && prm->rule != MI355CG_RULE_REL_2NORM) return fail(MI355CG_ERR_INVALID, "unknown rule %d", prm->rule);
    if (prm->use_true_solution) return fail(MI355CG_ERR_INVALID, "a batch has no per-system exact solution: use_true_solution must be 0");
    if (prm->diagnostics) return fail(MI355CG_ERR_INVALID, "a batch has no callbacks: diagnostics must be 0");
    const size_t bytes = sizeof(double) * (size_t)c->gp.size * (size_t)nrhs;
    const uintptr_t bb = (uintptr_t)b, xb = (uintptr_t)x;
    if (bb < xb + bytes && xb < bb + bytes) return fail(MI355CG_ERR_INVALID, "x overlaps b");
    if (!c->mg) return fail(MI355CG_ERR_STATE, "no preconditioner is set on this handle (mi355cg_set_preconditioner): a batch is multigrid-preconditioned CG");
    if (c->mg->cycle != MI355CG_CYCLE_F64) return fail(MI355CG_ERR_INVALID, "a batch runs the fp64 V-cycle: this handle's preconditioner was set with MI355CG_CYCLE_F32");
    return MI355CG_OK;
}

}

extern "C" {

const char* mi355cg_last_error(void) { return g_err.c_str(); }
const char* mi355cg_version(void) { return "mi355cg 0.2 (gfx950)"; }

static int create_impl(int n, int m, double a, double b, double c_, double d, int dtype, int device,
                       int y_lo, int y_hi, int s_lo, int s_hi, bool part, mi355cg_handle* out) {
    if (!out) return fail(MI355CG_ERR_INVALID, "out is null");
    *out = nullptr;
    if (dtype != MI355CG_F64 && dtype != MI355CG_F32_MIXED) return fail(MI355CG_ERR_INVALID, "unknown dtype %d", dtype);
    GridParams gp;
    if (!grid_params_init(&gp, n, m, a, b, c_, d))
        return fail(MI355CG_ERR_INVALID, "grid %dx%d rejected: the L-shaped index map is only consistent for n == m, even, >= 6", n, m);
    int ndev = 0;
    if (hipGetDeviceCount(&ndev) != hipSuccess || ndev <= 0)
        return fail(MI355CG_ERR_HIP, "no HIP device available (libmi355cg has no CPU fallback)");
    if (device < 0 || device >= ndev) return fail(MI355CG_ERR_INVALID, "device %d out of range (0..%d)", device, ndev - 1);
    HIPCK(hipSetDevice(device));

    const int ns_all = strips_total(gp, 2);
    if (!part) { y_lo = 1; y_hi = gp.n - 1; s_lo = 0; s_hi = ns_all; }
    if (y_lo < 1 || y_hi > gp.n - 1 || y_lo > y_hi)
        return fail(MI355CG_ERR_INVALID, "part rows [%d, %d] outside 1..%d", y_lo, y_hi, gp.n - 1);
    if (s_lo < 0 || s_hi > ns_all || s_lo >= s_hi)
        return fail(MI355CG_ERR_INVALID, "part strips [%d, %d) outside 0..%d", s_lo, s_hi, ns_all);
    if (dtype == MI355CG_F32_MIXED && part) return fail(MI355CG_ERR_INVALID, "F32_MIXED is single-GPU only");
    mi355cg_ctx* c = new mi355cg_ctx();
    c->device = device; c->dtype = dtype; c->gp = gp; c->is_slab = part;
    c->s_lo = s_lo; c->s_hi = s_hi;
    build_geom(c, 2, y_lo, y_hi);
    build_plans(c);
    c->strideA = std::max({c->whole.grid, c->interior.grid + c->edge.grid, c->whole32.grid, 1});
    c->strideB = c->strideA;

    int rc = MI355CG_OK;
    auto cleanup = [&]() { mi355cg_destroy(c); return rc; };
    if (hipStreamCreateWithFlags(&c->stream, hipStreamNonBlocking) != hipSuccess) { rc = fail(MI355CG_ERR_HIP, "hipStreamCreate failed"); return cleanup(); }
    const long long L = c->storage_len;
    { const int m = env_int("MI355CG_XSTEPS", 4); c->xsteps = m == 2 ? 2 : ((m == 8 && dtype == MI355CG_F64) ? 8 : 4); }
    double** vecs[] = {&c->x, &c->r, &c->p[0], &c->p[1], &c->ap, &c->b, &c->u, &c->p[2], &c->p[3], &c->p[4], &c->p[5], &c->p[6], &c->p[7]};
    for (int k = 0; k < 7 + (c->xsteps - 2); ++k) if ((rc = alloc_vec(vecs[k], L))) return cleanup();
    if (dtype == MI355CG_F32_MIXED) {
        float** fv[] = {&c->xf, &c->rf, &c->pf[0], &c->pf[1], &c->apf, &c->pf[2], &c->pf[3], &c->pf[4], &c->pf[5], &c->pf[6], &c->pf[7]};
        const int nfv = 5 + (c->xsteps - 2);
        for (int k = 0; k < nfv; ++k) {
            float** v = fv[k];
            if (hipMalloc((void**)v, sizeof(float) * L) != hipSuccess || hipMemset(*v, 0, sizeof(float) * L) != hipSuccess) {
                rc = fail(MI355CG_ERR_HIP, "fp32 vector allocation failed"); return cleanup();
            }
        }
    }
    if ((rc = alloc_vec(&c->packed, std::max<long long>(c->pk_len, 1)))) return cleanup();
    if ((rc = alloc_vec(&c->partA, (long long)FA_COUNT * c->strideA))) return cleanup();
    if ((rc = alloc_vec(&c->partB, (long long)FB_COUNT * c->strideB))) return cleanup();
    if ((rc = alloc_vec(&c->partR, 2048))) return cleanup();
    c->rec_width = kRecHeader + 2 * c->g.Pu;
    if ((rc = alloc_vec(&c->sumsA, c->rec_width))) return cleanup();
    if ((rc = alloc_vec(&c->sumsB, c->rec_width))) return cleanup();
    if (hipMalloc((void**)&c->sA, sizeof(CgState)) != hipSuccess || hipMalloc((void**)&c->sB, sizeof(CgState)) != hipSuccess ||
        hipMalloc((void**)&c->summary, sizeof(CgState)) != hipSuccess || hipMalloc((void**)&c->hist, sizeof(HistEntry) * kHist) != hipSuccess ||
        hipHostMalloc((void**)&c->summary_h, sizeof(CgState)) != hipSuccess || hipHostMalloc((void**)&c->hist_h, sizeof(HistEntry) * kHist) != hipSuccess ||
        hipHostMalloc((void**)&c->partR_h, sizeof(double) * 2048) != hipSuccess) {
        rc = fail(MI355CG_ERR_HIP, "state allocation failed"); return cleanup();
    }
    hipMemset(c->sA, 0, sizeof(CgState)); hipMemset(c->sB, 0, sizeof(CgState)); hipMemset(c->summary, 0, sizeof(CgState));
    hipMemset(c->hist, 0, sizeof(HistEntry) * kHist);
    if (hipMalloc((void**)&c->qctr, sizeof(int) * 2 * kXcds * kQueueSubs * kQueuePitch) != hipSuccess || hipMemset(c->qctr, 0, sizeof(int) * 2 * kXcds * kQueueSubs * kQueuePitch) != hipSuccess) { rc = fail(MI355CG_ERR_HIP, "queue counter allocation failed"); return cleanup(); }
    if (hipHostMalloc((void**)&c->stop_h, sizeof(int)) != hipSuccess) { rc = fail(MI355CG_ERR_HIP, "stop word allocation failed"); return cleanup(); }
    *c->stop_h = 0;
    HIPCK(hipDeviceSynchronize());

    if (env_int("MI355CG_DEVICE_SETUP", 0)) {
        c->host_rhs_valid = false; c->host_u_valid = false;
        if ((rc = mi355cg_setup_on_device(c))) return cleanup();
    } else {
        c->rhs_h.resize(c->pk_len); c->u_h.resize(c->pk_len);
        grid_fill_box(gp, c->g.y_lo, c->g.y_hi, s_lo * kStripCols, s_hi == ns_all ? gp.n : s_hi * kStripCols, c->rhs_h.data(), c->u_h.data(), nullptr, nullptr);
        if ((rc = upload_packed<double>(c, c->rhs_h.data(), c->b))) return cleanup();
    }
    *out = c;
    return MI355CG_OK;
}

int mi355cg_create(int n, int m, double a, double b, double c_, double d, int dtype, int device, mi355cg_handle* out) {
    return create_impl(n, m, a, b, c_, d, dtype, device, 0, 0, 0, 0, false, out);
}
int mi355cg_create_slab(int n, int m, double a, double b, double c_, double d, int dtype, int device,
                        int y_lo, int y_hi, mi355cg_handle* out) {
    GridParams gp;
    if (!grid_params_init(&gp, n, m, a, b, c_, d)) return fail(MI355CG_ERR_INVALID, "grid %dx%d rejected: the L-shaped index map is only consistent for n == m, even, >= 6", n, m);
    return create_impl(n, m, a, b, c_, d, dtype, device, y_lo, y_hi, 0, strips_total(gp, 2), true, out);
}
int mi355cg_create_part(int n, int m, double a, double b, double c_, double d, int dtype, int device,
                        int y_lo, int y_hi, int x_lo, int x_hi, mi355cg_handle* out) {
    GridParams gp;
    if (!grid_params_init(&gp, n, m, a, b, c_, d)) return fail(MI355CG_ERR_INVALID, "grid %dx%d rejected: the L-shaped index map is only consistent for n == m, even, >= 6", n, m);
    const int ns_all = strips_total(gp, 2);
    if (x_lo % kStripCols != 0 || (x_hi % kStripCols != 0 && x_hi < gp.n))
        return fail(MI355CG_ERR_INVALID, "part columns [%d, %d): x-cuts must be multiples of %d", x_lo, x_hi, kStripCols);
    return create_impl(n, m, a, b, c_, d, dtype, device, y_lo, y_hi, x_lo / kStripCols, x_hi >= gp.n ? ns_all : x_hi / kStripCols, true, out);
}

int mi355cg_create_csr(long long nrows, const int* row_map, const int* entries, const double* values,
                       int device, mi355cg_handle* out) {
    if (!out) return fail(MI355CG_ERR_INVALID, "out is null");
    *out = nullptr;
    if (nrows <= 0 || !row_map || !entries || !values) return fail(MI355CG_ERR_INVALID, "bad CSR arguments");
    if (row_map[0] != 0) return fail(MI355CG_ERR_INVALID, "row_map[0] must be 0");
    const long long nnz = row_map[nrows];
    for (long long i = 0; i < nrows; ++i) if (row_map[i + 1] < row_map[i]) return fail(MI355CG_ERR_INVALID, "row_map is not monotone at row %lld", i);
    for (long long j = 0; j < nnz; ++j) if (entries[j] < 0 || entries[j] >= nrows) return fail(MI355CG_ERR_INVALID, "column index %d out of range at entry %lld", entries[j], j);
    int ndev = 0;
    if (hipGetDeviceCount(&ndev) != hipSuccess || ndev <= 0) return fail(MI355CG_ERR_HIP, "no HIP device available (libmi355cg has no CPU fallback)");
    if (device < 0 || device >= ndev) return fail(MI355CG_ERR_INVALID, "device %d out of range (0..%d)", device, ndev - 1);
    HIPCK(hipSetDevice(device));
    mi355cg_ctx* c = new mi355cg_ctx();
    c->device = device; c->dtype = MI355CG_F64; c->is_csr = true;
    c->csr_n = nrows; c->csr_nnz = nnz;
    c->gp.size = nrows; c->pk_begin = 0; c->pk_len = nrows; c->storage_len = nrows; c->pg.pk_len = nrows;
    c->g.own_begin = 0; c->g.own_len = nrows;
    const long long nblk = (nrows + kBlock - 1) / kBlock;
    c->grid_csr = (int)std::max<long long>(1, std::min<long long>(2048, nblk));
    c->grid_update = (int)std::max<long long>(1, std::min<long long>(512, nblk));
    c->strideA = c->grid_csr; c->strideB = c->grid_update; c->nB_own = c->grid_update;
    int rc = MI355CG_OK;
    auto cleanup = [&]() { mi355cg_destroy(c); return rc; };
    if (hipStreamCreateWithFlags(&c->stream, hipStreamNonBlocking) != hipSuccess) { rc = fail(MI355CG_ERR_HIP, "hipStreamCreate failed"); return cleanup(); }
    double** vecs[] = {&c->x, &c->r, &c->p[0], &c->p[1], &c->ap, &c->b, &c->u};
    for (auto v : vecs) if ((rc = alloc_vec(v, nrows))) return cleanup();
    if ((rc = alloc_vec(&c->partA, (long long)FA_COUNT * c->strideA))) return cleanup();
    if ((rc = alloc_vec(&c->partB, (long long)FB_COUNT * c->strideB))) return cleanup();
    if ((rc = alloc_vec(&c->partR, 2048))) return cleanup();
    if (hipMalloc((void**)&c->csr_row_map, sizeof(int) * (nrows + 1)) != hipSuccess || hipMalloc((void**)&c->csr_entries, sizeof(int) * std::max<long long>(nnz, 1)) != hipSuccess ||
        hipMalloc((void**)&c->csr_values, sizeof(double) * std::max<long long>(nnz, 1)) != hipSuccess ||
        hipMalloc((void**)&c->sA, sizeof(CgState)) != hipSuccess || hipMalloc((void**)&c->sB, sizeof(CgState)) != hipSuccess ||
        hipMalloc((void**)&c->summary, sizeof(CgState)) != hipSuccess || hipMalloc((void**)&c->hist, sizeof(HistEntry) * kHist) != hipSuccess ||
        hipHostMalloc((void**)&c->summary_h, sizeof(CgState)) != hipSuccess || hipHostMalloc((void**)&c->hist_h, sizeof(HistEntry) * kHist) != hipSuccess ||
        hipHostMalloc((void**)&c->partR_h, sizeof(double) * 2048) != hipSuccess) {
        rc = fail(MI355CG_ERR_HIP, "allocation failed"); return cleanup();
    }
    if (hipMemcpy(c->csr_row_map, row_map, sizeof(int) * (nrows + 1), hipMemcpyHostToDevice) != hipSuccess ||
        hipMemcpy(c->csr_entries, entries, sizeof(int) * nnz, hipMemcpyHostToDevice) != hipSuccess ||
        hipMemcpy(c->csr_values, values, sizeof(double) * nnz, hipMemcpyHostToDevice) != hipSuccess) {
        rc = fail(MI355CG_ERR_HIP, "CSR upload failed"); return cleanup();
    }
    hipMemset(c->sA, 0, sizeof(CgState)); hipMemset(c->sB, 0, sizeof(CgState)); hipMemset(c->summary, 0, sizeof(CgState));
    hipMemset(c->hist, 0, sizeof(HistEntry) * kHist);
    HIPCK(hipDeviceSynchronize());
    c->rhs_h.assign(nrows, 0.0); c->u_h.assign(nrows, 0.0);
    *out = c;
    return MI355CG_OK;
}

int mi355cg_set_true_solution(mi355cg_handle c, const double* u) {
    if (!c || !u) return fail(MI355CG_ERR_INVALID, "null argument");
    HIPCK(hipSetDevice(c->device));
    c->host_u_valid = true;
    c->u_h.resize(c->pk_len);
    std::memcpy(c->u_h.data(), u, sizeof(double) * c->pk_len);
    if (int rc = upload_packed<double>(c, c->u_h.data(), c->u)) return rc;
    c->have_u_dev = true;
    return MI355CG_OK;
}

void mi355cg_destroy(mi355cg_handle c) {
    if (!c) return;
    hipSetDevice(c->device);
    if (c->stream) hipStreamSynchronize(c->stream);
    void* dev[] = {c->x, c->r, c->p[0], c->p[1], c->p[2], c->p[3], c->p[4], c->p[5], c->p[6], c->p[7], c->ap, c->b, c->u, c->scratch[0], c->scratch[1], c->xf, c->rf,
                   c->pf[0], c->pf[1], c->pf[2], c->pf[3], c->pf[4], c->pf[5], c->pf[6], c->pf[7], c->apf,
                   c->packed, c->partA, c->partB, c->partR, c->sumsA, c->sumsB, c->sA, c->sB, c->summary, c->hist, c->qctr};
    for (void* p : dev) if (p) hipFree(p);
    if (c->csr_row_map) hipFree(c->csr_row_map);
    if (c->csr_entries) hipFree(c->csr_entries);
    if (c->csr_values) hipFree(c->csr_values);
    if (c->summary_h) hipHostFree(c->summary_h);
    if (c->hist_h) hipHostFree(c->hist_h);
    if (c->partR_h) hipHostFree(c->partR_h);
    if (c->stop_h) hipHostFree(c->stop_h);
    clear_graphs(c);
    mg_batch_free(c);
    mg_free(c->mg);
    c->events.destroy();
    for (hipEvent_t e : c->ev_loop) if (e) hipEventDestroy(e);
    if (c->stream) hipStreamDestroy(c->stream);
    delete c;
}

long long mi355cg_size(mi355cg_handle c) { return c ? c->gp.size : -1; }

int mi355cg_get_rhs(mi355cg_handle c, double* out) {
    if (!c || !out) return fail(MI355CG_ERR_INVALID, "null argument");
    if (int rc = ensure_host_copies(c)) return rc;
    std::memcpy(out, c->rhs_h.data(), sizeof(double) * c->pk_len);
    return MI355CG_OK;
}
int mi355cg_get_true_solution(mi355cg_handle c, double* out) {
    if (!c || !out) return fail(MI355CG_ERR_INVALID, "null argument");
    if (int rc = ensure_host_copies(c)) return rc;
    std::memcpy(out, c->u_h.data(), sizeof(double) * c->pk_len);
    return MI355CG_OK;
}
int mi355cg_get_node_coords(mi355cg_handle c, double* xs, double* ys) {
    if (!c || !xs || !ys) return fail(MI355CG_ERR_INVALID, "null argument");
    if (c->is_csr) return fail(MI355CG_ERR_INVALID, "a CSR handle has no grid coordinates");
    const int ns_all = strips_total(c->gp, 2);
    grid_fill_box(c->gp, c->g.y_lo, c->g.y_hi, c->s_lo * kStripCols, c->s_hi == ns_all ? c->gp.n : c->s_hi * kStripCols, nullptr, nullptr, xs, ys);
    return MI355CG_OK;
}
int mi355cg_setup_on_device(mi355cg_handle c) {
    if (!c) return fail(MI355CG_ERR_INVALID, "null handle");
    if (c->is_csr) return fail(MI355CG_ERR_INVALID, "a CSR handle has no grid to set up");
    HIPCK(hipSetDevice(c->device));
    if (c->is_slab) HIPCK(hipDeviceSynchronize());
    SetupArgs s{};
    s.pg = c->pg; s.a = c->gp.a; s.c = c->gp.c; s.x_step = c->gp.x_step; s.y_step = c->gp.y_step; s.xk = c->gp.x_k; s.yk = c->gp.y_k;
    s.n = c->gp.n; s.m = c->gp.m;
    if (c->pk_len > 0) hipLaunchKernelGGL(k_setup, dim3(flat_grid(c->pk_len)), dim3(kBlock), 0, c->stream, s, c->b, c->u);
    HIPCK(hipGetLastError());
    HIPCK(hipStreamSynchronize(c->stream));
    c->have_u_dev = true; c->host_rhs_valid = false; c->host_u_valid = false;
    return MI355CG_OK;
}
int mi355cg_set_rhs(mi355cg_handle c, const double* b) {
    if (!c || !b) return fail(MI355CG_ERR_INVALID, "null argument");
    HIPCK(hipSetDevice(c->device));
    c->host_rhs_valid = true;
    c->rhs_h.resize(c->pk_len);
    std::memcpy(c->rhs_h.data(), b, sizeof(double) * c->pk_len);
    return upload_packed<double>(c, c->rhs_h.data(), c->b);
}

int mi355cg_apply_device(mi355cg_handle c, const double* x_dev, double* y_dev) {
    if (!c || !x_dev || !y_dev) return fail(MI355CG_ERR_INVALID, "null argument");
    if (c->is_slab) return fail(MI355CG_ERR_STATE, "this handle owns one part of a decomposed grid: use the mi355cg_team_* / mi355cg_dist_* entry points");
    HIPCK(hipSetDevice(c->device));
    if (c->is_csr) {
        launch_csr_spmv(c, x_dev, y_dev, nullptr, nullptr, nullptr);
        HIPCK(hipGetLastError());
        HIPCK(hipStreamSynchronize(c->stream));
        return MI355CG_OK;
    }
    if (int rc = ensure_scratch(c)) return rc;
    hipLaunchKernelGGL((k_unpack<double>), dim3(flat_grid(c->pk_len)), dim3(kBlock), 0, c->stream, c->pg, x_dev, c->scratch[0]);
    launch_apply<double, 2>(c, c->scratch[0], c->scratch[1], whole_part(c));
    hipLaunchKernelGGL((k_pack<double>), dim3(flat_grid(c->pk_len)), dim3(kBlock), 0, c->stream, c->pg, c->scratch[1], y_dev);
    HIPCK(hipGetLastError());
    HIPCK(hipStreamSynchronize(c->stream));
    return MI355CG_OK;
}

int mi355cg_apply(mi355cg_handle c, const double* x, double* y) {
    if (!c || !x || !y) return fail(MI355CG_ERR_INVALID, "null argument");
    if (c->is_slab) return fail(MI355CG_ERR_STATE, "this handle owns one part of a decomposed grid: use the mi355cg_team_* / mi355cg_dist_* entry points");
// ... 38 lines not shown
    if (diag) if (int rc = ensure_scratch(c)) return rc;

    const auto t0 = std::chrono::steady_clock::now();
    c->events.reset(); c->ev_pairs[0].clear(); c->ev_pairs[1].clear();

    c->cur = 0;
    if (c->qctr && c->dyn_rows > 0) HIPCK(hipMemsetAsync(c->qctr, 0, sizeof(int) * 2 * kXcds * kQueueSubs * kQueuePitch, c->stream));
    {
        FreshArgs<double> f{};
        f.begin = c->g.own_begin / 2; f.nvec = c->g.own_len / 2;
        f.b = c->b; f.x = c->x; f.r = c->r; f.p0 = c->p[0]; f.u = c->u;
        f.partB = c->partB; f.strideB = c->strideB; f.s_out = c->sB;
        if (cfg.has_u) hipLaunchKernelGGL((k_init_fresh<double, 2, true>), dim3(c->whole.grid), dim3(kBlock), 0, c->stream, f);
        else hipLaunchKernelGGL((k_init_fresh<double, 2, false>), dim3(c->whole.grid), dim3(kBlock), 0, c->stream, f);
    }
    HIPCK(hipGetLastError());

    *c->stop_h = 0;
    c->stop_dev = nullptr;
    if (stop_flag) HIPCK(hipHostGetDevicePointer((void**)&c->stop_dev, c->stop_h, 0));
    auto wait_stream = [&]() -> int {
        if (!stop_flag) { HIPCK(hipStreamSynchronize(c->stream)); return MI355CG_OK; }
        for (;;) {
            if (*stop_flag) *c->stop_h = 1;
            const hipError_t q = hipStreamQuery(c->stream);
            if (q == hipSuccess) break;
            if (q != hipErrorNotReady) HIPCK(q);
            std::this_thread::yield();
        }
        return MI355CG_OK;
    };
    auto poll = [&]() -> int {
        launch_check(c, cfg, c->stream, own_partB(c));
        HIPCK(hipMemcpyAsync(c->summary_h, c->summary, sizeof(CgState), hipMemcpyDeviceToHost, c->stream));
        HIPCK(hipMemcpyAsync(c->hist_h, c->hist, sizeof(HistEntry) * kHist, hipMemcpyDeviceToHost, c->stream));
        return wait_stream();
    };
    *c->summary_h = CgState{};
    if (msg && cb) {
        if (int rc = poll()) return rc;
        cb(user, 0, DBL_MAX, c->summary_h->rmax, cfg.has_u ? c->summary_h->emax : DBL_MAX);
    }
    if (!c->ev_loop[0]) { HIPCK(hipEventCreate(&c->ev_loop[0])); HIPCK(hipEventCreate(&c->ev_loop[1])); }
    HIPCK(hipEventRecord(c->ev_loop[0], c->stream));

    const int every = prm->callback_every;
    auto need_u = [&](int it) { return diag || cfg.rp.eps_exact_error > 0 || it == 1 || (every > 0 && it % every == 0); };
    int sync_every = prm->sync_every > 0 ? prm->sync_every : (msg ? 100 : 200);
    sync_every = std::min(sync_every, kHist);
    int it_done = 0;
    bool interrupted = false;
    bool first_chunk = cb != nullptr || stop_flag != nullptr;
    if (std::memcmp(&c->graph_prm, prm, sizeof *prm) != 0 || c->graph_stop != (stop_flag != nullptr)) {
        clear_graphs(c); c->graph_prm = *prm; c->graph_stop = stop_flag != nullptr;
    }
    const bool graph_ok = !c->profiling && !diag &&
                          (c->use_graph == 1 || (c->use_graph < 0 && c->g.own_len < (4LL << 20) && prm->max_iterations >= 4 * sync_every));
    while (!c->summary_h->done) {
        if (stop_flag && *stop_flag) { interrupted = true; break; }
        int m = std::min(sync_every, prm->max_iterations - it_done);
        if (msg && every > 0) m = std::min(m, every - it_done % every);
        if (first_chunk) { m = 1; first_chunk = false; }
        if (m <= 0) m = 1;
        auto enqueue_chunk = [&]() -> int {
            for (int k = 0; k < m; ++k) {
                hipEvent_t e0 = nullptr;
                prof_begin(c, &e0);
                launch_iteration_stencil<double, 2>(c, cfg, c->r, c->p, whole_part(c), own_partB(c));
                c->cur = (c->cur + 1) % c->xsteps;
                prof_end(c, 0, e0);
                prof_begin(c, &e0);
                IterCfg ucfg = cfg;
                ucfg.has_u = cfg.has_u && need_u(it_done + k + 1);
                launch_iteration_update<double, 2>(c, ucfg, c->x, c->r, c->p, c->u, whole_part(c), own_partA(c));
                prof_end(c, 1, e0);
                if (diag) {
                    launch_apply<double, 2>(c, c->x, c->scratch[0], whole_part(c));
                    hipLaunchKernelGGL((k_resid2<double>), dim3(1024), dim3(kBlock), 0, c->stream, c->g.own_begin, c->g.own_len, c->b, c->scratch[0], c->partR);
                    hipLaunchKernelGGL(k_resid2_hist, dim3(1), dim3(kBlock), 0, c->stream, c->partR, 1024, c->sB, c->hist);
                }
            }
            return MI355CG_OK;
        };
        if (graph_ok && m >= 8) {
            std::vector<char> flags(m);
            for (int k = 0; k < m; ++k) flags[k] = cfg.has_u && need_u(it_done + k + 1);
            mi355cg_ctx::ChunkGraph* hit = nullptr;
            for (auto& g : c->graphs) if (g.m == m && g.cur == c->cur && g.flags == flags) hit = &g;
            if (!hit) {
                hipGraph_t graph = nullptr; hipGraphExec_t exec = nullptr;
                const int cur0 = c->cur;
                HIPCK(hipStreamBeginCapture(c->stream, hipStreamCaptureModeThreadLocal));
                const int rc = enqueue_chunk();
                const hipError_t e1 = hipStreamEndCapture(c->stream, &graph);
                c->cur = cur0;
                if (rc) return rc;
                HIPCK(e1);
                HIPCK(hipGraphInstantiate(&exec, graph, nullptr, nullptr, 0));
                HIPCK(hipGraphDestroy(graph));
                c->graphs.push_back({m, cur0, flags, exec});
                hit = &c->graphs.back();
            }
            HIPCK(hipGraphLaunch(hit->exec, c->stream));
            c->cur = (c->cur + m) % c->xsteps;
        } else {
            if (int rc = enqueue_chunk()) return rc;
        }
        HIPCK(hipGetLastError());
        if (int rc = poll()) return rc;
        const int it_now = c->summary_h->it;
        if (cb) for (int it = it_done + 1; it <= it_now; ++it) {
            const HistEntry& h = c->hist_h[it % kHist];
            if (diag) {
                cb(user, it - 1, std::sqrt(h.d2), std::sqrt(h.tr2), std::sqrt(h.e2));
            } else if (msg) {
                const bool stopped_here = c->summary_h->done && c->summary_h->reason != MI355CG_STOP_ITERATIONS &&
                                          c->summary_h->reason != MI355CG_STOP_INTERRUPTED && it == it_now;
                if ((it == 1 || (every > 0 && it % every == 0)) && !stopped_here) cb(user, it, h.dmax, h.rmax, cfg.has_u ? h.emax : DBL_MAX);
            }
        }
        it_done = it_now;
    }
    HIPCK(hipEventRecord(c->ev_loop[1], c->stream));
    CgState fin = *c->summary_h;
    c->stop_dev = nullptr;
    if (fin.done && fin.reason == MI355CG_STOP_INTERRUPTED) interrupted = true;
    c->cur = fin.it % c->xsteps;
    if (cfg.x2) {
        launch_flush_x<double, 2>(c, c->whole, c->x, c->p, fin, c->stream);
        HIPCK(hipGetLastError());
        HIPCK(hipStreamSynchronize(c->stream));
    }
    if (cfg.has_u && fin.it > 0 && !need_u(fin.it)) {
        hipLaunchKernelGGL((k_err_maxnorm<double>), dim3(1024), dim3(kBlock), 0, c->stream, c->g.own_begin, c->g.own_len, c->x, c->u, c->partR);
        HIPCK(hipGetLastError());
        HIPCK(hipMemcpyAsync(c->partR_h, c->partR, sizeof(double) * 1024, hipMemcpyDeviceToHost, c->stream));
        HIPCK(hipStreamSynchronize(c->stream));
        double m = 0; for (int i = 0; i < 1024; ++i) m = std::max(m, c->partR_h[i]);
        fin.emax = m;
    }
    c->solved = true;
    prof_collect(c);
#ifdef MI355CG_WAVE_TIMING
    if (const char* path = getenv("MI355CG_WAVE_TIMING_OUT")) {
        std::vector<unsigned long long> buf(2 * kWtStamps * kWtWaves);
        HIPCK(hipMemcpyFromSymbol(buf.data(), HIP_SYMBOL(g_wave_dbg), buf.size() * sizeof(unsigned long long)));
        if (FILE* f = fopen(path, "wb")) { fwrite(buf.data(), sizeof(unsigned long long), buf.size(), f); fclose(f); }
    }
#endif
    mi355cg_results res{};
    res.iterations = fin.it;
    res.converged = interrupted ? 0 : fin.converged;
    res.stop_reason = interrupted ? MI355CG_STOP_INTERRUPTED : fin.reason;
    res.final_residual_norm = fin.rmax;
    res.final_precision = fin.it > 0 ? fin.dmax : DBL_MAX;
    res.final_error_norm = cfg.has_u ? fin.emax : DBL_MAX;
    res.r_norm2 = fin.rnorm2;
    res.initial_r_norm2 = fin.r0norm;
    res.solve_seconds = std::chrono::duration<double>(std::chrono::steady_clock::now() - t0).count();
    { float ms = 0; HIPCK(hipEventSynchronize(c->ev_loop[1])); if (hipEventElapsedTime(&ms, c->ev_loop[0], c->ev_loop[1]) == hipSuccess) res.loop_seconds = 1e-3 * ms; }
    if (msg && cb) cb(user, res.iterations, res.final_precision, res.final_residual_norm, res.final_error_norm);
    if (out) *out = res;
    return MI355CG_OK;
}

int mi355cg_get_solution(mi355cg_handle c, double* x) {
    if (!c || !x) return fail(MI355CG_ERR_INVALID, "null argument");
    if (!c->solved) return fail(MI355CG_ERR_STATE, "no solve has run on this handle");
    HIPCK(hipSetDevice(c->device));
    return download_packed<double>(c, c->x, x);
}
int mi355cg_get_recursive_residual(mi355cg_handle c, double* r) {
    if (!c || !r) return fail(MI355CG_ERR_INVALID, "null argument");
    if (!c->solved) return fail(MI355CG_ERR_STATE, "no solve has run on this handle");
    HIPCK(hipSetDevice(c->device));
    return download_packed<double>(c, c->r, r);
}
int mi355cg_get_true_residual(mi355cg_handle c, double* out) {
    if (!c || !out) return fail(MI355CG_ERR_INVALID, "null argument");
    if (c->is_slab) return fail(MI355CG_ERR_STATE, "this handle owns one part of a decomposed grid: use the mi355cg_team_* / mi355cg_dist_* entry points");
    if (!c->solved) return fail(MI355CG_ERR_STATE, "no solve has run on this handle");
    HIPCK(hipSetDevice(c->device));
    if (int rc = ensure_scratch(c)) return rc;
    if (c->is_csr) launch_csr_spmv(c, c->x, c->scratch[0], nullptr, nullptr, nullptr);
    else launch_apply<double, 2>(c, c->x, c->scratch[0], whole_part(c));
    hipLaunchKernelGGL((k_sub<double>), dim3(flat_grid(c->g.own_len)), dim3(kBlock), 0, c->stream, c->g.own_begin, c->g.own_len, c->scratch[0], c->b, c->scratch[1]);
    HIPCK(hipGetLastError());
    return download_packed<double>(c, c->scratch[1], out);
}

int mi355cg_set_profiling(mi355cg_handle c, int enable) {
    if (!c) return fail(MI355CG_ERR_INVALID, "null handle");
    c->profiling = enable != 0;
    return MI355CG_OK;
}
int mi355cg_get_kernel_time(mi355cg_handle c, int kernel, double* avg_ms, long long* launches) {
    if (!c || kernel < 0 || kernel > 1) return fail(MI355CG_ERR_INVALID, "bad argument");
    if (avg_ms) *avg_ms = c->kernel_ms[kernel];
    if (launches) *launches = c->kernel_launches[kernel];
    return MI355CG_OK;
}
int mi355cg_get_layout(mi355cg_handle c, long long* padded_len, int* pitch_bottom, int* pitch_upper,
                       int* grid_stencil, int* grid_update, int* rows_per_item) {
    if (!c) return fail(MI355CG_ERR_INVALID, "null handle");
    if (padded_len) *padded_len = c->g.own_len;
    if (pitch_bottom) *pitch_bottom = c->g.Pb;
    if (pitch_upper) *pitch_upper = c->g.Pu;
    if (grid_stencil) *grid_stencil = c->whole.grid;
    if (grid_update) *grid_update = c->whole.grid;
    if (rows_per_item) *rows_per_item = c->whole.ty;
    return MI355CG_OK;
}

int mi355cg_mg_levels(int n, int* levels, int* coarsest_n) {
    std::vector<int> ns;
    if (int rc = mg_shape(MI355CG_PRECOND_MG, n, &ns)) return rc;
    if (levels) *levels = (int)ns.size();
    if (coarsest_n) *coarsest_n = ns.back();
    return MI355CG_OK;
}

int mi355cg_mg_hierarchy(int kind, int n, int max_levels, int* levels, int* level_n) {
    if (max_levels < 0 || (max_levels > 0 && !level_n)) return fail(MI355CG_ERR_INVALID, "level_n must hold max_levels >= 0 entries");
    std::vector<int> ns;
    if (int rc = mg_shape(kind, n, &ns)) return rc;
    if (levels) *levels = (int)ns.size();
    for (int l = 0; l < (int)ns.size() && l < max_levels; ++l) level_n[l] = ns[l];
    return MI355CG_OK;
}

int mi355cg_set_preconditioner(mi355cg_handle c, int kind) { return mi355cg_set_preconditioner_ex(c, kind, MI355CG_CYCLE_F64); }

int mi355cg_set_preconditioner_ex(mi355cg_handle c, int kind, int cycle) {
    if (!c) return fail(MI355CG_ERR_INVALID, "null handle");
    if (kind != MI355CG_PRECOND_NONE && kind != MI355CG_PRECOND_MG && kind != MI355CG_PRECOND_MG_ANY)
        return fail(MI355CG_ERR_INVALID, "unknown preconditioner kind %d (MI355CG_PRECOND_NONE = 0, MI355CG_PRECOND_MG = 1, "
                    "MI355CG_PRECOND_MG_ANY = 2)", kind);
    HIPCK(hipSetDevice(c->device));
    if (kind == MI355CG_PRECOND_NONE) {
        mg_batch_free(c);
        if (c->mg) { HIPCK(hipStreamSynchronize(c->stream)); mg_free(c->mg); c->mg = nullptr; }
        return MI355CG_OK;
    }
    if (c->is_csr) return fail(MI355CG_ERR_INVALID, "the multigrid preconditioner needs the grid operator: a CSR handle has no grid");
    if (c->is_slab) return fail(MI355CG_ERR_INVALID, "the multigrid preconditioner is single-GPU only: this handle owns one part of a decomposed grid");
    if (c->dtype != MI355CG_F64) return fail(MI355CG_ERR_INVALID, "the multigrid preconditioner is fp64 only: this handle was created with MI355CG_F32_MIXED");
    std::vector<int> ns;
    if (int rc = mg_shape(kind, c->gp.n, &ns)) return rc;
    if (cycle != MI355CG_CYCLE_F64 && cycle != MI355CG_CYCLE_F32)
        return fail(MI355CG_ERR_INVALID, "unknown V-cycle precision %d (MI355CG_CYCLE_F64 = 0, MI355CG_CYCLE_F32 = 1)", cycle);
    mg_batch_free(c);
    if (c->mg && c->mg->cycle == cycle) { c->mg->kind = kind; return MI355CG_OK; }
    if (!c->mg) return mg_build(c, kind, &c->mg, cycle);
    HIPCK(hipStreamSynchronize(c->stream));
    MgHier* H = nullptr;
    if (int rc = mg_build(c, kind, &H, cycle)) return rc;
    mg_free(c->mg);
    c->mg = H;
    return MI355CG_OK;
}

int mi355cg_preconditioner_info(mi355cg_handle c, int* kind, int* cycle, int* levels) {
    if (!c) return fail(MI355CG_ERR_INVALID, "null handle");
    if (kind) *kind = c->mg ? c->mg->kind : MI355CG_PRECOND_NONE;
    if (cycle) *cycle = c->mg ? c->mg->cycle : MI355CG_CYCLE_F64;
    if (levels) *levels = c->mg ? (int)c->mg->lv.size() : 0;
    return MI355CG_OK;
}

int mi355cg_apply_preconditioner(mi355cg_handle c, const double* r, double* z) {
    if (!c || !r || !z) return fail(MI355CG_ERR_INVALID, "null argument");
    if (!c->mg) return fail(MI355CG_ERR_STATE, "no preconditioner is set on this handle (mi355cg_set_preconditioner)");
    HIPCK(hipSetDevice(c->device));
    if (int rc = upload_packed<double>(c, r, c->mg->q)) return rc;
    if (c->mg->cycle == MI355CG_CYCLE_F32) {
        double rmax = 0;
        for (long long i = 0; i < c->pk_len; ++i) rmax = std::max(rmax, std::fabs(r[i]));
        if (int rc = mg_apply32(c, c->mg->q, c->mg->z, rmax)) return rc;
    } else
    mg_vcycle(c, 0, c->mg->q, c->mg->z, nullptr);
    HIPCK(hipGetLastError());
    return download_packed<double>(c, c->mg->z, z);
}

int mi355cg_solve_batch_device(mi355cg_handle c, const mi355cg_params* prm, int nrhs, const double* b_dev, double* x_dev,
                               const volatile int* stop_flag, mi355cg_results* out) {
    if (int rc = batch_check(c, prm, nrhs, b_dev, x_dev, out)) return rc;
    HIPCK(hipSetDevice(c->device));
    if (int rc = mg_batch_ensure(c, nrhs, 0)) return rc;
    return solve_mg_batch(c, prm, nrhs, b_dev, x_dev, stop_flag, out);
}

// ... 265 lines not shown
```

### iterative_solvers_amd/solver.py

```python
from __future__ import annotations

import ctypes as C
import enum
import sys
from dataclasses import dataclass, field
from typing import Callable, Optional

import numpy as np

from . import _capi

DBL_MAX = sys.float_info.max
BATCH_MAX = _capi.BATCH_MAX


class StopCriterion(enum.IntEnum):
    ITERATIONS = 0
    PRECISION = 1
    RESIDUAL = 2
    EXACT_ERROR = 3
    INTERRUPTED = 4


_STOP_TEXT = {
# ... 92 lines not shown
        return res

    def set_preconditioner(self, kind: int, cycle: int = _capi.CYCLE_F64):
        rc = self._lib.mi355cg_set_preconditioner_ex(self._h, int(kind), int(cycle))
        if rc == _capi.ERR_INVALID:
            raise ValueError(self._lib.mi355cg_last_error().decode())
        _capi.check(rc)

    def preconditioner_info(self):
        k, cy, lv = C.c_int(), C.c_int(), C.c_int()
        _capi.check(self._lib.mi355cg_preconditioner_info(self._h, C.byref(k), C.byref(cy), C.byref(lv)))
        return k.value, cy.value, lv.value

    def apply_preconditioner(self, r):
        r = np.ascontiguousarray(r, dtype=np.float64)
        if r.shape != (self.size,):
            raise ValueError(f"vector has shape {r.shape}, expected ({self.size},)")
        z = np.empty(self.size)
        _capi.check(self._lib.mi355cg_apply_preconditioner(self._h, r, z))
        return z

    @staticmethod
    def _check_batch(b, size):
        on_device = not isinstance(b, np.ndarray)
        if on_device:
            if not (type(b).__module__.split(".")[0] == "torch" and hasattr(b, "data_ptr")):
                raise ValueError(f"a batch of right-hand sides is a NumPy array or a CUDA torch tensor, not {type(b).__name__}")
            import torch
            if not b.is_cuda:
                raise ValueError("a torch batch must be in device memory (a CPU tensor: pass tensor.numpy())")
            if b.dtype != torch.float64:
                raise ValueError(f"batch has dtype {b.dtype}, expected torch.float64")
            if not b.is_contiguous():
                raise ValueError("batch tensor must be contiguous")
        elif b.dtype != np.float64:
            raise ValueError(f"batch has dtype {b.dtype}, expected float64")
        shape = tuple(b.shape)
        if len(shape) != 2 or shape[1] != size:
            raise ValueError(f"batch has shape {shape}, expected (nrhs, {size})")
        if not 1 <= shape[0] <= _capi.BATCH_MAX:
            raise ValueError(f"a batch has 1 .. {_capi.BATCH_MAX} right-hand sides, not {shape[0]}")
        return shape[0], on_device

    def solve_batch(self, params: _capi.Params, b, stop_flag: Optional[C.c_int] = None):
        nrhs, on_device = self._check_batch(b, self.size)
        res = (_capi.Results * nrhs)()
        sp = C.cast(C.pointer(stop_flag), C.c_void_p) if stop_flag is not None else None
        if on_device:
            import torch
            if b.device.index != self._device:
                raise ValueError(f"batch is on {b.device}, the handle on device {self._device}")
            x = torch.empty_like(b)
            torch.cuda.current_stream(b.device).synchronize()
            rc = self._lib.mi355cg_solve_batch_device(self._h, C.byref(params), nrhs, b.data_ptr(), x.data_ptr(), sp, res)
        else:
            b = np.ascontiguousarray(b)
            x = np.empty_like(b)
            rc = self._lib.mi355cg_solve_batch(self._h, C.byref(params), nrhs, b.ctypes.data, x.ctypes.data, sp, res)
        if rc == _capi.ERR_INVALID:
            raise ValueError(self._lib.mi355cg_last_error().decode())
        _capi.check(rc)
        return x, list(res)

    def batch_release(self):
        _capi.check(self._lib.mi355cg_batch_release(self._h))

    def setup_on_device(self):
        _capi.check(self._lib.mi355cg_setup_on_device(self._h))

    def set_profiling(self, on: bool):
        _capi.check(self._lib.mi355cg_set_profiling(self._h, 1 if on else 0))

    def kernel_time(self, kernel: int):
        ms, n = C.c_double(), C.c_longlong()
        _capi.check(self._lib.mi355cg_get_kernel_time(self._h, kernel, C.byref(ms), C.byref(n)))
        return ms.value, n.value

    def layout(self):
        L = C.c_longlong()
        v = [C.c_int() for _ in range(5)]
        _capi.check(self._lib.mi355cg_get_layout(self._h, C.byref(L), *[C.byref(i) for i in v]))
        return {"padded_len": L.value, "pitch_bottom": v[0].value, "pitch_upper": v[1].value,
                "grid_stencil": v[2].value, "grid_update": v[3].value, "rows_per_item": v[4].value}


def default_params(rule: int) -> _capi.Params:
    p = _capi.Params()
    _capi.load().mi355cg_default_params(C.byref(p), rule)
    return p


def mg_levels(n: int):
    L, nc = C.c_int(), C.c_int()
    lib = _capi.load()
    rc = lib.mi355cg_mg_levels(int(n), C.byref(L), C.byref(nc))
    if rc == _capi.ERR_INVALID:
        raise ValueError(lib.mi355cg_last_error().decode())
    _capi.check(rc)
    return L.value, nc.value


def mg_hierarchy(n: int, kind: int = _capi.PRECOND_MG_ANY):
    L = C.c_int()
    buf = (C.c_int * 64)()
    lib = _capi.load()
    rc = lib.mi355cg_mg_hierarchy(int(kind), int(n), len(buf), C.byref(L), buf)
    if rc == _capi.ERR_INVALID:
        raise ValueError(lib.mi355cg_last_error().decode())
    _capi.check(rc)
    return tuple(buf[:L.value])


class MatrixFreeSystem:

    def __init__(self, m, n, a, b, c, d, device: int = 0, dtype: int = _capi.F64):
        self.n, self.m = n, m
        self.domain = (a, b, c, d)
        self._handle = _Handle(n, m, a, b, c, d, dtype=dtype, device=device)

    def get_rhs(self) -> np.ndarray: return self._handle.rhs()
    def get_true_solution_vector(self) -> np.ndarray: return self._handle.true_solution()
    def size(self) -> int: return self._handle.size

    def apply(self, x, y=None) -> np.ndarray:
        out = self._handle.apply(x)
        if y is not None:
            y[...] = out
            return y
        return out

    def __mul__(self, x): return self.apply(x)

    def set_preconditioner(self, kind: int, cycle: int = _capi.CYCLE_F64):
        self._handle.set_preconditioner(kind, cycle)

    def preconditioner_info(self):
        return self._handle.preconditioner_info()

    def solve_batch(self, b, eps: float = 1e-6, max_iterations: int = 10000, rule: int = _capi.RULE_REL_2NORM, params=None):
        if params is None:
            params = default_params(rule)
            params.max_iterations = max_iterations
            params.eps_rel = params.eps_precision = params.eps_residual = eps
            params.use_true_solution = 0
        return self._handle.solve_batch(params, b)

    def batch_release(self):
        self._handle.batch_release()


class GridSystem(MatrixFreeSystem):

    def get_matrix(self): return self
    def get_x_coords(self): return self._handle.node_coords()[0]
    def get_y_coords(self): return self._handle.node_coords()[1]

    def get_node_coordinates(self, solution_index: int):
        if solution_index < 0 or solution_index >= self.size():
            return (0.0, 0.0)
        xs, ys = self._handle.node_coords()
        return (float(xs[solution_index]), float(ys[solution_index]))


class CrsMatrix:

    def __init__(self, row_map, entries, values, device: int = 0):
# ... 179 lines not shown
```

Before: 7144 iters/s.

## Add persistent chunk kernel fusing CG phases with grid seams and LDS-resident residual rows

Adds a persistent kernel that runs the stencil and update phases of several CG iterations in one launch. It separates them with grid-wide seam barriers instead of one launch per phase, and keeps part of each wave's residual rows resident in LDS so they are not re-read from HBM. The aim is to remove per-iteration launch and graph overhead and cut memory traffic on the memory-bound fp64 stencil. In exchange it relies on co-residency of all workgroups, adds a seam timeout fallback path, and lowers occupancy because of the large dynamic LDS.

```diff
diff --git a/include/mi355cg.h b/include/mi355cg.h
--- a/include/mi355cg.h
+++ b/include/mi355cg.h
@@ -109,6 +109,7 @@
 int  mi355cg_get_kernel_time(mi355cg_handle h, int kernel, double *avg_ms, long long *launches);
 int  mi355cg_get_layout(mi355cg_handle h, long long *padded_len, int *pitch_bottom, int *pitch_upper,
                         int *grid_stencil, int *grid_update, int *rows_per_item);
+int  mi355cg_get_loop_info(mi355cg_handle h, int *persistent, int *resident_rows, int *rows_per_item);
 
 int  mi355cg_slab_rows(int n, int world, int rank, int *y_lo, int *y_hi);
 int  mi355cg_create_part(int n, int m, double a, double b, double c, double d, int dtype, int device,
diff --git a/iterative_solvers_amd/_capi.py b/iterative_solvers_amd/_capi.py
--- a/iterative_solvers_amd/_capi.py
+++ b/iterative_solvers_amd/_capi.py
@@ -28,7 +28,7 @@
     "mi355cg_team_set_profiling", "mi355cg_team_phase_times", "mi355cg_team_describe", "mi355cg_setup_on_device", "mi355cg_team_setup_on_device", "mi355cg_debug_plan",
     "mi355cg_team_set_dtype", "mi355cg_set_preconditioner", "mi355cg_apply_preconditioner", "mi355cg_mg_levels",
     "mi355cg_mg_hierarchy", "mi355cg_set_preconditioner_ex", "mi355cg_preconditioner_info",
-    "mi355cg_solve_batch", "mi355cg_solve_batch_device", "mi355cg_batch_release",
+    "mi355cg_solve_batch", "mi355cg_solve_batch_device", "mi355cg_batch_release", "mi355cg_get_loop_info",
 ]
 DECOMP_ROWS, DECOMP_2D = 0, 1
 PRECOND_NONE, PRECOND_MG, PRECOND_MG_ANY = 0, 1, 2
@@ -164,6 +164,7 @@
     L.mi355cg_solve_batch.argtypes = [H, C.POINTER(Params), C.c_int, C.c_void_p, C.c_void_p, C.c_void_p, C.POINTER(Results)]
     L.mi355cg_solve_batch_device.argtypes = [H, C.POINTER(Params), C.c_int, C.c_void_p, C.c_void_p, C.c_void_p, C.POINTER(Results)]
     L.mi355cg_batch_release.argtypes = [H]
+    L.mi355cg_get_loop_info.argtypes = [H, IP, IP, IP]
     _lib = L
     return L
 
diff --git a/iterative_solvers_amd/csrc/cg_kernels.h b/iterative_solvers_amd/csrc/cg_kernels.h
--- a/iterative_solvers_amd/csrc/cg_kernels.h
+++ b/iterative_solvers_amd/csrc/cg_kernels.h
@@ -169,18 +169,24 @@
     return t;
 }
 struct PreParts { double hi0, lo0, hi1, lo1; };
+template <bool FRESH> __device__ inline double ld_part(const double* p) {
+    if constexpr (FRESH) return __builtin_bit_cast(double, __hip_atomic_load(reinterpret_cast<const unsigned long long*>(p), __ATOMIC_RELAXED, __HIP_MEMORY_SCOPE_AGENT));
+    else return *p;
+}
+template <bool FRESH = false>
 __device__ inline PreParts prefetch_parts(const double* __restrict__ part_hi, const double* __restrict__ part_lo, int n, int es) {
     PreParts p{0.0, 0.0, 0.0, 0.0};
     const int i0 = threadIdx.x, i1 = threadIdx.x + kBlock;
-    if (i0 < n) { p.hi0 = part_hi[(long long)i0 * es]; p.lo0 = part_lo[(long long)i0 * es]; }
-    if (i1 < n) { p.hi1 = part_hi[(long long)i1 * es]; p.lo1 = part_lo[(long long)i1 * es]; }
+    if (i0 < n) { p.hi0 = ld_part<FRESH>(part_hi + (long long)i0 * es); p.lo0 = ld_part<FRESH>(part_lo + (long long)i0 * es); }
+    if (i1 < n) { p.hi1 = ld_part<FRESH>(part_hi + (long long)i1 * es); p.lo1 = ld_part<FRESH>(part_lo + (long long)i1 * es); }
     return p;
 }
+template <bool FRESH = false>
 __device__ inline dd reduce_parts_dd_pre(const PreParts& pre, const double* __restrict__ part_hi, const double* __restrict__ part_lo, int n, int es, double* lds) {
     dd v = dd_zero();
     if ((int)threadIdx.x < n) v = dd_add(v, dd{pre.hi0, pre.lo0});
     if ((int)threadIdx.x + kBlock < n) v = dd_add(v, dd{pre.hi1, pre.lo1});
-    for (int i = threadIdx.x + 2 * kBlock; i < n; i += kBlock) v = dd_add(v, dd{part_hi[(long long)i * es], part_lo[(long long)i * es]});
+    for (int i = threadIdx.x + 2 * kBlock; i < n; i += kBlock) v = dd_add(v, dd{ld_part<FRESH>(part_hi + (long long)i * es), ld_part<FRESH>(part_lo + (long long)i * es)});
     return block_reduce_dd(v, lds);
 }
 struct PreMax { double v0, v1; };
@@ -472,6 +478,25 @@
     if (lane == 0) v = __hip_atomic_fetch_add(q, 1, __ATOMIC_RELAXED, __HIP_MEMORY_SCOPE_AGENT);
     return v;
 }
+
+enum { PHASE_RAN = 0, PHASE_OVER = 1 };
+struct ChunkLoop {
+    StateLite s;
+    double ah[3];
+    int res_off;
+    int rows;
+    int tail;
+    int fill;
+    unsigned* stopw;
+};
+__device__ __forceinline__ double uniform_f64(double v) {
+    const unsigned long long u = __builtin_bit_cast(unsigned long long, v);
+    const unsigned lo = __builtin_amdgcn_readfirstlane((unsigned)u), hi = __builtin_amdgcn_readfirstlane((unsigned)(u >> 32));
+    return __builtin_bit_cast(double, ((unsigned long long)hi << 32) | lo);
+}
+__device__ __forceinline__ double* chunk_lds() { extern __shared__ __attribute__((aligned(16))) double mi355cg_dyn_lds[]; return mi355cg_dyn_lds; }
+__device__ __forceinline__ int resident_first(const ChunkLoop& cl, int nrows) { return cl.tail ? max(nrows - cl.rows, 0) : 0; }
+__device__ __forceinline__ int resident_count(const ChunkLoop& cl, int nrows) { return min(cl.rows, nrows); }
 
 template <typename T>
 struct StencilArgs {
@@ -584,15 +609,14 @@
     return A;
 }
 
-template <typename T, int VEC, bool FUSED, bool MSG, int DEPTH, bool NOAP, bool GC>
-__global__ __launch_bounds__(kBlock) void k_stencil(const StencilArgs<T> a) {
+template <typename T, int VEC, bool FUSED, bool MSG, int DEPTH, bool NOAP, bool GC, bool PERSIST>
+__device__ __forceinline__ int stencil_phase(const StencilArgs<T>& a, const Geom& g, const WorkList& wl, const T* a_r, const T* a_pin, T* a_pout, double* lds, ChunkLoop* cl) {
     static_assert(DEPTH >= 1 && DEPTH <= 3, "the compute cursor takes its item from the fetch cursor: DEPTH <= rows fetched per item (>= 3)");
+    static_assert(!PERSIST || (FUSED && !MSG && NOAP && !GC && VEC == 2 && sizeof(T) == 8), "the persistent launch runs the fp64 REL_2NORM phases of one context");
     typedef typename VecOf<T, VEC>::type vec_t;
-    __shared__ double lds[2 * kWaves];
-    const Geom& g = a.g;
     const int lane = threadIdx.x & (kWave - 1);
     const int wave = __builtin_amdgcn_readfirstlane(threadIdx.x / kWave);
-    const ItemSeq seq = item_seq(a.wl, wave);
+    const ItemSeq seq = item_seq(wl, wave);
     MI355CG_WT_BEGIN
     struct Raw { vec_t r, p; T re, pe; };
 
@@ -600,17 +624,19 @@
     bool f_have = f_item < seq.end;
     ItemAddr F{};
     int f_idx = 0, f_so = 0, f_y = 0;
-    rsrc_t rs_p = make_rsrc(a.pin), rs_r = make_rsrc(a.pin);
+    int f_res0 = 0, f_resn = 0, f_last = 0, c_res0 = 0, c_resn = 0, c_last = 0;
+    rsrc_t rs_p = make_rsrc(a_pin), rs_r = make_rsrc(a_pin);
     const int dq_nsub = min(kQueueSubs, (int)(gridDim.x / kXcds)), dq_sub = (int)(blockIdx.x / kXcds) % dq_nsub;
     int* const dq = a.dq.mine ? a.dq.mine + ((int)(blockIdx.x % kXcds) * kQueueSubs + dq_sub) * kQueuePitch : nullptr;
     if (a.dq.other && blockIdx.x == 0 && threadIdx.x < kXcds * kQueueSubs) a.dq.other[threadIdx.x * kQueuePitch] = 0;
     int dq_ticket = 0;
     auto enter = [&](int item) {
         if (dq) dq_ticket = queue_take(dq, lane);
-        F = item_addr<T, VEC, false>(g, decode_item(a.wl, item), lane);
-        rs_p = make_rsrc(a.pin + F.base_el);
-        rs_r = make_rsrc(FUSED ? a.r + F.base_el : a.pin + F.base_el);
+        F = item_addr<T, VEC, false>(g, decode_item(wl, item), lane);
+        rs_p = make_rsrc(a_pin + F.base_el);
+        rs_r = make_rsrc(FUSED ? a_r + F.base_el : a_pin + F.base_el);
         f_idx = -1; f_so = F.so_first; f_y = F.ystart - 1;
+        if constexpr (PERSIST) { f_last = F.nrows - 1; f_res0 = resident_first(*cl, f_last + 1); f_resn = resident_count(*cl, f_last + 1); }
     };
     auto fetch = [&]() -> Raw {
         if (f_have && f_idx > F.nrows) {
@@ -622,9 +648,11 @@
         int vo = own ? F.vo_own : (f_idx < 0 ? F.vo_first : F.vo_last);
         int ve = own ? F.ve_own : kOob;
         if (!f_have) { vo = kOob; ve = kOob; }
+        int vo_r = vo;
+        if constexpr (PERSIST) { if (!cl->fill && (unsigned)(f_idx - f_res0) < (unsigned)f_resn) vo_r = kOob; }
         Raw w;
         w.p = buf_load<vec_t>(rs_p, vo, f_so);
-        if (FUSED) w.r = buf_load<vec_t>(rs_r, vo, f_so);
+        if (FUSED) w.r = buf_load<vec_t>(rs_r, vo_r, f_so);
         else for (int j = 0; j < VEC; ++j) w.r[j] = (T)0;
         w.pe = buf_load<T>(rs_p, ve, f_so);
         if (FUSED) w.re = buf_load<T>(rs_r, ve, f_so); else w.re = (T)0;
@@ -638,11 +666,12 @@
     bool in_j[VEC];
 #pragma unroll
     for (int j = 0; j < VEC; ++j) in_j[j] = false;
-    rsrc_t rs_po = make_rsrc(a.pin), rs_ap = make_rsrc(a.pin);
+    rsrc_t rs_po = make_rsrc(a_pin), rs_ap = make_rsrc(a_pin);
     auto promote = [&]() {
         C = F;
-        rs_po = make_rsrc(FUSED ? a.pout + C.base_el : a.pin + C.base_el);
-        rs_ap = make_rsrc(NOAP ? a.pin + C.base_el : a.ap + C.base_el);
+        if constexpr (PERSIST) { c_res0 = f_res0; c_resn = f_resn; c_last = f_last; }
+        rs_po = make_rsrc(FUSED ? a_pout + C.base_el : a_pin + C.base_el);
+        rs_ap = make_rsrc(NOAP ? a_pin + C.base_el : a.ap + C.base_el);
         c_idx = -1; c_so = C.so_c0; c_y = C.ystart;
         const int xint0 = C.bot ? g.half + 1 : 1;
 #pragma unroll
@@ -656,7 +685,19 @@
     for (int k = 0; k < DEPTH; ++k) q[k] = fetch();
 
     T beta = (T)0;
-    if (FUSED && a.src.mbox) {
+    if constexpr (PERSIST) {
+        const PreParts pre = prefetch_parts<true>(a.partB + FB_RR * a.strideB, a.partB + (FB_RR + FB_LO) * a.strideB, a.nB, a.esB);
+        StateLite s = cl->s;
+        if (!cl->fill) s.stop = (int)__hip_atomic_load(cl->stopw, __ATOMIC_RELAXED, __HIP_MEMORY_SCOPE_AGENT);
+        MI355CG_WT_STAMP(1)
+        const double rr = dd_value(reduce_parts_dd_pre<true>(pre, a.partB + FB_RR * a.strideB, a.partB + (FB_RR + FB_LO) * a.strideB, a.nB, a.esB, lds));
+        const Decision d = decide_after_update(s, a.rp, rr, 0, 0, 0, 0, 0);
+        MI355CG_WT_STAMP(2)
+        if (blockIdx.x == 0 && threadIdx.x == 0) write_state_after_decision(a.s_out, a.hist, a.s_in, s, d);
+        if (d.done) return PHASE_OVER;
+        cl->s.rr_prev = s.rr; cl->s.rr = uniform_f64(d.rr); cl->s.r0norm = uniform_f64(d.r0norm); cl->s.stop = __builtin_amdgcn_readfirstlane(s.stop);
+        beta = (T)d.beta;
+    } else if (FUSED && a.src.mbox) {
         __shared__ double recs[kMaxRecDst * kRecWords];
         const PreParts pre = prefetch_parts(a.partB + FB_RR * a.strideB, a.partB + (FB_RR + FB_LO) * a.strideB, a.nB, 1);
         PreMax pmax[3] = {{0, 0}, {0, 0}, {0, 0}};
@@ -667,18 +708,18 @@
         const StateLite s = load_state_lite(a.s_in);
         if (s.done) {
             if (threadIdx.x == 0) { store_flagged_zero(a.fl, a.slotA + blockIdx.x, FA_COUNT); if (blockIdx.x == 0) copy_state(a.s_out, a.s_in); }
-            return;
+            return PHASE_OVER;
         }
         MI355CG_WT_STAMP(1)
         own_record_B(recs, a.src.me, a.partB, a.nB, a.strideB, MSG ? 1 : 0, lds, &pre, MSG ? pmax : nullptr);
         if (!gather_records(a.src, recs)) {
             if (threadIdx.x == 0) { store_flagged_zero(a.fl, a.slotA + blockIdx.x, FA_COUNT); if (blockIdx.x == 0) fail_transport(a.s_out, a.s_in); }
-            return;
+            return PHASE_OVER;
         }
         const Decision d = decide_from_records(s, a.rp, recs, a.src.world, MSG, false);
         MI355CG_WT_STAMP(2)
         if (blockIdx.x == 0 && threadIdx.x == 0) write_state_after_decision(a.s_out, a.hist, a.s_in, s, d);
-        if (d.done) { if (threadIdx.x == 0) store_flagged_zero(a.fl, a.slotA + blockIdx.x, FA_COUNT); return; }
+        if (d.done) { if (threadIdx.x == 0) store_flagged_zero(a.fl, a.slotA + blockIdx.x, FA_COUNT); return PHASE_OVER; }
         beta = (T)d.beta;
     } else if (FUSED) {
         const PreParts pre = prefetch_parts(a.partB + FB_RR * a.strideB, a.partB + (FB_RR + FB_LO) * a.strideB, a.nB, a.esB);
@@ -688,12 +729,12 @@
             for (int k = 0; k < 3; ++k) pmax[k] = prefetch_max(a.partB + (FB_RMAX + k) * a.strideB, a.nB, a.esB);
         }
         const StateLite s = load_state_lite(a.s_in);
-        if (s.done) { if (blockIdx.x == 0 && threadIdx.x == 0) copy_state(a.s_out, a.s_in); return; }
+        if (s.done) { if (blockIdx.x == 0 && threadIdx.x == 0) copy_state(a.s_out, a.s_in); return PHASE_OVER; }
         MI355CG_WT_STAMP(1)
         const Decision d = reduce_and_decide(s, a.rp, a.partB, a.nB, a.strideB, a.esB, a.want_diag, lds, &pre, MSG ? pmax : nullptr);
         MI355CG_WT_STAMP(2)
         if (blockIdx.x == 0 && threadIdx.x == 0) write_state_after_decision(a.s_out, a.hist, a.s_in, s, d);
-        if (d.done) return;
+        if (d.done) return PHASE_OVER;
         beta = (T)d.beta;
     }
 
@@ -710,8 +751,15 @@
 #pragma unroll
         for (int k = 0; k < DEPTH; ++k) {
             if (c_have) {
-                const Raw w = q[k];
+                Raw w = q[k];
                 q[k] = fetch();
+                if constexpr (PERSIST) {
+                    const int slot = c_idx - c_res0;
+                    if ((unsigned)slot < (unsigned)c_resn) {
+                        vec_t* res = reinterpret_cast<vec_t*>(chunk_lds() + cl->res_off + slot * (kWave * VEC));
+                        if (cl->fill) *res = w.r; else w.r = *res;
+                    }
+                }
                 vec_t pn; T pne;
                 if (FUSED) {
 #pragma unroll
@@ -769,6 +817,13 @@
         a.partA[FA_RZ * st + b] = tz.hi;  a.partA[(FA_RZ + FA_LO) * st + b] = tz.lo;
         if (FUSED && a.fl.part) { const double v[FA_COUNT] = {tp.hi, tz.hi, tp.lo, tz.lo}; store_flagged(a.fl, b, FA_COUNT, v); }
     }
+    return PHASE_RAN;
+}
+
+template <typename T, int VEC, bool FUSED, bool MSG, int DEPTH, bool NOAP, bool GC>
+__global__ __launch_bounds__(kBlock) void k_stencil(const StencilArgs<T> a) {
+    __shared__ double lds[2 * kWaves];
+    stencil_phase<T, VEC, FUSED, MSG, DEPTH, NOAP, GC, false>(a, a.g, a.wl, a.r, a.pin, a.pout, lds, nullptr);
 }
 
 template <typename T>
@@ -951,18 +1006,20 @@
     QueueSpec dq;
 };
 
-template <typename T, int VEC, int XM, bool HAS_U, int DEPTH, bool DESC>
-__global__ __launch_bounds__(kBlock) void k_update_st(const UpdateStArgs<T> a) {
+template <typename T, int VEC, int XM, bool HAS_U, int DEPTH, bool DESC, bool PERSIST>
+__device__ __forceinline__ int update_phase(const UpdateStArgs<T>& a, const Geom& g, const WorkList& wl, const T* a_p, const T* const (&a_pprev)[kRing - 1], double* lds, ChunkLoop* cl) {
     static_assert(DEPTH >= 1 && DEPTH <= 3, "see k_stencil");
+    static_assert(!PERSIST || ((XM == 0 || XM == 4) && !HAS_U && VEC == 2 && sizeof(T) == 8), "the persistent launch runs the fp64 REL_2NORM phases of one context");
     typedef typename VecOf<T, VEC>::type vec_t;
-    __shared__ double lds[2 * kWaves];
-    const Geom& g = a.g;
     const int lane = threadIdx.x & (kWave - 1);
     const int wave = __builtin_amdgcn_readfirstlane(threadIdx.x / kWave);
-    const ItemSeq seq = item_seq(a.wl, wave);
+    const ItemSeq seq = item_seq(wl, wave);
     MI355CG_WT_BEGIN
     int stop_word = 0;
-    if (blockIdx.x == 0 && a.stop_req) stop_word = scalar_load(a.stop_req);
+    if (blockIdx.x == 0 && a.stop_req) {
+        if constexpr (PERSIST) stop_word = __hip_atomic_load(a.stop_req, __ATOMIC_RELAXED, __HIP_MEMORY_SCOPE_SYSTEM);
+        else stop_word = scalar_load(a.stop_req);
+    }
     constexpr bool FULL = XM == 1;
     constexpr int NP = XM >= 2 ? XM - 1 : 0;
     struct Raw { vec_t p, r, x, u, pp[NP > 0 ? NP : 1]; T pe; };
@@ -971,7 +1028,8 @@
     bool f_have = f_item < seq.end;
     ItemAddr F{};
     int f_idx = 0, f_so = 0, f_y = 0;
-    rsrc_t rs_p = make_rsrc(a.p), rs_r = rs_p, rs_x = rs_p, rs_u = rs_p;
+    int f_res0 = 0, f_resn = 0, f_last = 0, c_res0 = 0, c_resn = 0, c_last = 0;
+    rsrc_t rs_p = make_rsrc(a_p), rs_r = rs_p, rs_x = rs_p, rs_u = rs_p;
     rsrc_t rs_pp[NP > 0 ? NP : 1] = {rs_p};
     const int dq_nsub = min(kQueueSubs, (int)(gridDim.x / kXcds)), dq_sub = (int)(blockIdx.x / kXcds) % dq_nsub;
     int* const dq = a.dq.mine ? a.dq.mine + ((int)(blockIdx.x % kXcds) * kQueueSubs + dq_sub) * kQueuePitch : nullptr;
@@ -979,14 +1037,15 @@
     int dq_ticket = 0;
     auto enter = [&](int idx) {
         if (dq) dq_ticket = queue_take(dq, lane);
-        F = item_addr<T, VEC, DESC>(g, decode_item(a.wl, a.reverse ? seq.end - 1 - (idx - seq.begin) : idx), lane);
-        rs_p = make_rsrc(a.p + F.base_el);
+        F = item_addr<T, VEC, DESC>(g, decode_item(wl, a.reverse ? seq.end - 1 - (idx - seq.begin) : idx), lane);
+        rs_p = make_rsrc(a_p + F.base_el);
         rs_r = make_rsrc(a.r + F.base_el);
-        rs_x = make_rsrc(XM != 0 ? a.x + F.base_el : a.p + F.base_el);
-#pragma unroll
-        for (int i = 0; i < NP; ++i) rs_pp[i] = make_rsrc(a.pprev[i] + F.base_el);
-        rs_u = make_rsrc((FULL && HAS_U) ? a.u + F.base_el : a.p + F.base_el);
+        rs_x = make_rsrc(XM != 0 ? a.x + F.base_el : a_p + F.base_el);
+#pragma unroll
+        for (int i = 0; i < NP; ++i) rs_pp[i] = make_rsrc(a_pprev[i] + F.base_el);
+        rs_u = make_rsrc((FULL && HAS_U) ? a.u + F.base_el : a_p + F.base_el);
         f_idx = -1; f_so = F.so_first; f_y = DESC ? F.ystart + 1 : F.ystart - 1;
+        if constexpr (PERSIST) { f_last = F.nrows - 1; f_res0 = resident_first(*cl, f_last + 1); f_resn = resident_count(*cl, f_last + 1); }
     };
     auto fetch = [&]() -> Raw {
         if (f_have && f_idx > F.nrows) {
@@ -998,9 +1057,11 @@
         int vo = own ? F.vo_own : (f_idx < 0 ? F.vo_first : F.vo_last);
         if (!f_have) vo = kOob;
         const int vown = own ? F.vo_own : kOob;
+        int vown_r = vown;
+        if constexpr (PERSIST) { if (own && (unsigned)((DESC ? f_last - f_idx : f_idx) - f_res0) < (unsigned)f_resn) vown_r = kOob; }
         Raw w;
         w.p = buf_load<vec_t>(rs_p, vo, f_so);
-        w.r = buf_load<vec_t>(rs_r, vown, f_so);
+        w.r = buf_load<vec_t>(rs_r, vown_r, f_so);
         if (XM != 0) w.x = buf_load<vec_t>(rs_x, vown, f_so);
 #pragma unroll
         for (int i = 0; i < NP; ++i) w.pp[i] = buf_load<vec_t>(rs_pp[i], vown, f_so);
@@ -1020,8 +1081,9 @@
     rsrc_t rs_ro = rs_p, rs_xo = rs_p;
     auto promote = [&]() {
         C = F;
+        if constexpr (PERSIST) { c_res0 = f_res0; c_resn = f_resn; c_last = f_last; }
         rs_ro = make_rsrc(a.r + C.base_el);
-        rs_xo = make_rsrc(XM != 0 ? a.x + C.base_el : a.p + C.base_el);
+        rs_xo = make_rsrc(XM != 0 ? a.x + C.base_el : a_p + C.base_el);
         c_idx = -1; c_so = C.so_c0; c_y = C.ystart;
         const int xint0 = C.bot ? g.half + 1 : 1;
 #pragma unroll
@@ -1035,7 +1097,12 @@
 
     double alpha_d, rz = 0.0;
     StateLite s;
-    if (a.src.mbox) {
+    if constexpr (PERSIST) {
+        const PreParts pre = prefetch_parts<true>(a.partA + FA_PAP * a.strideA, a.partA + (FA_PAP + FA_LO) * a.strideA, a.nA, a.esA);
+        s = cl->s;
+        const double pap = dd_value(reduce_parts_dd_pre<true>(pre, a.partA + FA_PAP * a.strideA, a.partA + (FA_PAP + FA_LO) * a.strideA, a.nA, a.esA, lds));
+        alpha_d = s.rr / pap;
+    } else if (a.src.mbox) {
         __shared__ double recs[kMaxRecDst * kRecWords];
         const PreParts pre = prefetch_parts(a.partA + FA_PAP * a.strideA, a.partA + (FA_PAP + FA_LO) * a.strideA, a.nA, 1);
         PreParts pre_rz{0, 0, 0, 0};
@@ -1043,7 +1110,7 @@
         s = load_state_lite(a.s_in);
         if (s.done) {
             if (threadIdx.x == 0) { store_flagged_zero(a.fl, a.slotB + blockIdx.x, FB_LL_COUNT); if (blockIdx.x == 0) copy_state(a.s_out, a.s_in); }
-            return;
+            return PHASE_OVER;
         }
         {
             double* R = recs + a.src.me * kRecWords;
@@ -1057,7 +1124,7 @@
         }
         if (!gather_records(a.src, recs)) {
             if (threadIdx.x == 0) { store_flagged_zero(a.fl, a.slotB + blockIdx.x, FB_LL_COUNT); if (blockIdx.x == 0) fail_transport(a.s_out, a.s_in); }
-            return;
+            return PHASE_OVER;
         }
         alpha_from_records(s, a.rule, recs, a.src.world, &alpha_d, &rz);
     } else {
@@ -1065,7 +1132,7 @@
         PreParts pre_rz{0, 0, 0, 0};
         if (FULL) pre_rz = prefetch_parts(a.partA + FA_RZ * a.strideA, a.partA + (FA_RZ + FA_LO) * a.strideA, a.nA, a.esA);
         s = load_state_lite(a.s_in);
-        if (s.done) { if (blockIdx.x == 0 && threadIdx.x == 0) copy_state(a.s_out, a.s_in); return; }
+        if (s.done) { if (blockIdx.x == 0 && threadIdx.x == 0) copy_state(a.s_out, a.s_in); return PHASE_OVER; }
         const double pap = dd_value(reduce_parts_dd_pre(pre, a.partA + FA_PAP * a.strideA, a.partA + (FA_PAP + FA_LO) * a.strideA, a.nA, a.esA, lds));
         if (a.rule == 0) {
             rz = FULL ? dd_value(reduce_parts_dd_pre(pre_rz, a.partA + FA_RZ * a.strideA, a.partA + (FA_RZ + FA_LO) * a.strideA, a.nA, a.esA, lds))
@@ -1079,7 +1146,10 @@
     MI355CG_WT_MID
     T aprev[NP > 0 ? NP : 1] = {(T)0};
 #pragma unroll
-    for (int i = 0; i < NP; ++i) aprev[i] = (T)scalar_load(&a.s_in->alpha_hist[(s.it - i) & (kRing - 1)]);
+    for (int i = 0; i < NP; ++i) {
+        if constexpr (PERSIST) aprev[i] = (T)cl->ah[i];
+        else aprev[i] = (T)scalar_load(&a.s_in->alpha_hist[(s.it - i) & (kRing - 1)]);
+    }
     const T cA = (T)g.A, cxk = (T)g.xk, cyk = (T)g.yk;
     dd s_rr = dd_zero(), s_d2 = dd_zero(), s_e2 = dd_zero();
     double s_rmax = 0, s_dmax = 0, s_emax = 0;
@@ -1107,6 +1177,11 @@
                     const vec_t& top = DESC ? p_b : w.p;
                     const vec_t& bot = DESC ? w.p : p_b;
                     vec_t rn, xn;
+                    vec_t* res = nullptr;
+                    if constexpr (PERSIST) {
+                        const int slot = (DESC ? c_last + 1 - c_idx : c_idx - 1) - c_res0;
+                        if ((unsigned)slot < (unsigned)c_resn) { res = reinterpret_cast<vec_t*>(chunk_lds() + cl->res_off + slot * (kWave * VEC)); c.r = *res; }
+                    }
 #pragma unroll
                     for (int j = 0; j < VEC; ++j) {
                         const T cc = c.p[j];
@@ -1141,6 +1216,7 @@
                         }
                     }
                     buf_store(rn, rs_ro, C.vo_own, c_so);
+                    if constexpr (PERSIST) { if (res) *res = rn; }
                     if (XM != 0) buf_store(xn, rs_xo, C.vo_own, c_so);
                     if (DESC) { c_so -= row_step<T>(g, c_y - 1); --c_y; } else { c_so += row_step<T>(g, c_y); ++c_y; }
                     p_b = c.p; c = w;
@@ -1174,8 +1250,101 @@
             CgState* o = a.s_out;
             o->it = s.it + 1; o->first = 0; o->alpha = alpha_d; o->rz = rz; o->alpha_hist[(s.it + 1) & (kRing - 1)] = alpha_d;
             o->stop = stop_word != 0;
-        }
-    }
+            if constexpr (PERSIST) *cl->stopw = stop_word != 0;
+        }
+    }
+    if constexpr (PERSIST) {
+        cl->ah[2] = cl->ah[1]; cl->ah[1] = cl->ah[0]; cl->ah[0] = uniform_f64(alpha_d);
+        cl->s.it = s.it + 1; cl->s.first = 0; cl->s.alpha = cl->ah[0]; cl->s.rz = rz;
+    }
+    return PHASE_RAN;
+}
+
+template <typename T, int VEC, int XM, bool HAS_U, int DEPTH, bool DESC>
+__global__ __launch_bounds__(kBlock) void k_update_st(const UpdateStArgs<T> a) {
+    __shared__ double lds[2 * kWaves];
+    update_phase<T, VEC, XM, HAS_U, DEPTH, DESC, false>(a, a.g, a.wl, a.p, a.pprev, lds, nullptr);
+}
+
+constexpr int kSeamPitch = 64;
+enum { SEAM_CLS = 0, SEAM_TOP = kXcds, SEAM_GEN = kXcds + 1, SEAM_ERR = 2 * kXcds + 1, SEAM_STOP = 2 * kXcds + 2, SEAM_WORDS = 2 * kXcds + 3 };
+constexpr int kChunkStage = 32;
+struct SeamSpec { unsigned* w; u64 budget; };
+__device__ __forceinline__ bool grid_seam(const SeamSpec& sp, unsigned round) {
+    asm volatile("s_waitcnt vmcnt(0)" ::: "memory");
+    __syncthreads();
+    int bad = 0;
+    if (threadIdx.x == 0) {
+        const unsigned cls = blockIdx.x % kXcds, in_cls = (gridDim.x - cls + kXcds - 1) / kXcds, ncls = min((unsigned)gridDim.x, (unsigned)kXcds);
+        __builtin_amdgcn_fence(__ATOMIC_RELEASE, "agent");
+        asm volatile("s_waitcnt vmcnt(0)" ::: "memory");
+        if (__hip_atomic_fetch_add(sp.w + (SEAM_CLS + cls) * kSeamPitch, 1u, __ATOMIC_RELAXED, __HIP_MEMORY_SCOPE_AGENT) == round * in_cls - 1u) {
+            if (__hip_atomic_fetch_add(sp.w + SEAM_TOP * kSeamPitch, 1u, __ATOMIC_RELAXED, __HIP_MEMORY_SCOPE_AGENT) == round * ncls - 1u) {
+#pragma unroll
+                for (int k = 0; k < kXcds; ++k) __hip_atomic_store(sp.w + (SEAM_GEN + k) * kSeamPitch, round, __ATOMIC_RELAXED, __HIP_MEMORY_SCOPE_AGENT);
+            }
+        }
+        const unsigned* gen = sp.w + (SEAM_GEN + cls) * kSeamPitch;
+        const u64 t0 = wall_clock64();
+        unsigned spins = 0;
+        while (__hip_atomic_load(gen, __ATOMIC_RELAXED, __HIP_MEMORY_SCOPE_AGENT) < round) {
+            __builtin_amdgcn_s_sleep(1);
+            if ((++spins & 63u) == 0 &&
+                (__hip_atomic_load(sp.w + SEAM_ERR * kSeamPitch, __ATOMIC_RELAXED, __HIP_MEMORY_SCOPE_AGENT) != 0u || wall_clock64() - t0 > sp.budget)) {
+                __hip_atomic_store(sp.w + SEAM_ERR * kSeamPitch, 1u, __ATOMIC_RELAXED, __HIP_MEMORY_SCOPE_AGENT);
+                bad = 1;
+                break;
+            }
+        }
+        __builtin_amdgcn_fence(__ATOMIC_ACQUIRE, "agent");
+        asm volatile("s_waitcnt vmcnt(0)" ::: "memory");
+    }
+    return __syncthreads_or(bad) == 0;
+}
+
+template <typename T>
+struct ChunkArgs {
+    StencilArgs<T> st;
+    UpdateStArgs<T> up;
+    T* ring[4];
+    int cur, m;
+    SeamSpec seam;
+    int res_rows, res_tail;
+};
+
+template <typename T, int VEC, int DEPTH, int DEPTH_X>
+__global__ __launch_bounds__(kBlock, 2) void k_cg_chunk(const ChunkArgs<T> a) {
+    double* lds = chunk_lds();
+    const int lane = threadIdx.x & (kWave - 1);
+    const int wave = __builtin_amdgcn_readfirstlane(threadIdx.x / kWave);
+    ChunkLoop cl;
+    cl.s = load_state_lite(a.st.s_in);
+#pragma unroll
+    for (int i = 0; i < 3; ++i) cl.ah[i] = scalar_load(&a.st.s_in->alpha_hist[(cl.s.it - i) & (kRing - 1)]);
+    cl.res_off = kChunkStage + wave * a.res_rows * (kWave * VEC) + lane * VEC;
+    cl.rows = a.res_rows; cl.tail = a.res_tail; cl.fill = 1;
+    cl.stopw = a.seam.w + SEAM_STOP * kSeamPitch;
+    const bool writer = blockIdx.x == 0 && threadIdx.x == 0;
+    if (cl.s.done) { if (writer) copy_state(a.st.s_out, a.st.s_in); return; }
+    unsigned round = 0;
+    bool ok = true;
+    for (int j = 0; j < a.m; ++j) {
+        if (j > 0 && !(ok = grid_seam(a.seam, ++round))) break;
+        const int k0 = (a.cur + j) & 3, k1 = (k0 + 1) & 3;
+        const T* pin = k0 == 0 ? a.ring[0] : k0 == 1 ? a.ring[1] : k0 == 2 ? a.ring[2] : a.ring[3];
+        T* pout = k1 == 0 ? a.ring[0] : k1 == 1 ? a.ring[1] : k1 == 2 ? a.ring[2] : a.ring[3];
+        if (stencil_phase<T, VEC, true, false, DEPTH, true, false, true>(a.st, a.st.g, a.st.wl, a.st.r, pin, pout, lds, &cl) != PHASE_RAN) {
+            if (writer) copy_state(a.up.s_out, a.up.s_in);
+            return;
+        }
+        cl.fill = 0;
+        if (!(ok = grid_seam(a.seam, ++round))) break;
+        const T* pprev[kRing - 1] = {pin, k0 == 0 ? a.ring[3] : k0 == 1 ? a.ring[0] : k0 == 2 ? a.ring[1] : a.ring[2],
+                                     k0 == 0 ? a.ring[2] : k0 == 1 ? a.ring[3] : k0 == 2 ? a.ring[0] : a.ring[1], pin, pin, pin, pin};
+        if (k1 == 0) update_phase<T, VEC, 4, false, DEPTH_X, true, true>(a.up, a.st.g, a.st.wl, pout, pprev, lds, &cl);
+        else update_phase<T, VEC, 0, false, DEPTH, true, true>(a.up, a.st.g, a.st.wl, pout, pprev, lds, &cl);
+    }
+    if (!ok && writer) { CgState* o = a.up.s_out; o->done = 1; o->reason = kReasonTransport; o->converged = 0; }
 }
 
 struct CheckArgs {
diff --git a/iterative_solvers_amd/csrc/mi355cg.hip b/iterative_solvers_amd/csrc/mi355cg.hip
--- a/iterative_solvers_amd/csrc/mi355cg.hip
+++ b/iterative_solvers_amd/csrc/mi355cg.hip
@@ -145,6 +145,12 @@
     mi355cg_params graph_prm{};
     bool graph_stop = false;
     int use_graph = -1;
+
+    bool persist = false;
+    int persist_rows = 0;
+    int persist_tail = 0;
+    size_t persist_lds = 0;
+    unsigned* seam = nullptr;
 
     hipEvent_t ev_loop[2] = {nullptr, nullptr};
     MgHier* mg = nullptr;
@@ -272,6 +278,7 @@
     return pl;
 }
 constexpr int kMaxRowsF64 = 800, kMaxRowsF32 = 64;
+constexpr int kPersistAutoMinN = 2048;
 
 void build_plans(mi355cg_ctx* c) {
     const Geom& g = c->g;
@@ -421,6 +428,83 @@
     a.partB = pb.ptr; a.nB = pb.n; a.strideB = pb.fstride; a.esB = pb.estride; a.src = pb.rec;
     a.s_in = c->sB; a.summary = c->summary; a.hist = c->hist; a.rp = cfg.rp; a.want_diag = cfg.want_diag;
     hipLaunchKernelGGL(k_check, dim3(1), dim3(kBlock), 0, stream, a);
+}
+
+constexpr unsigned long long kSeamBudgetTicks = 200000000ull;
+constexpr size_t kSeamBytes = sizeof(unsigned) * SEAM_WORDS * kSeamPitch;
+constexpr int kPersistWgLdsBytes = 80 * 1024;
+
+bool one_item_per_wave(const Plan& pl) {
+    const WorkList& wl = pl.wl;
+    if (wl.nitems == 0) return false;
+    if (wl.ncls == kXcds) {
+        for (int k = 0; k < kXcds; ++k) {
+            const int nb = (pl.grid - k + kXcds - 1) / kXcds;
+            if (wl.cls0[k + 1] - wl.cls0[k] > nb * kWaves) return false;
+        }
+        return true;
+    }
+    return wl.nitems <= pl.grid * kWaves;
+}
+
+int persist_setup(mi355cg_ctx* c) {
+    c->persist = false; c->persist_rows = 0;
+    const char* mode = getenv("MI355CG_PERSIST");
+    const bool force = mode && !strcmp(mode, "1"), off = mode && !strcmp(mode, "0");
+    if (off || c->is_slab || c->is_csr || c->dtype != MI355CG_F64 || c->has_gc || c->dyn_rows > 0 || c->xsteps != 4 || c->depth != 3) return MI355CG_OK;
+    if (!one_item_per_wave(c->whole) || c->whole.grid > 512) return MI355CG_OK;
+    if (!force && c->gp.n < kPersistAutoMinN) return MI355CG_OK;
+    hipDeviceProp_t prop;
+    HIPCK(hipGetDeviceProperties(&prop, c->device));
+    const int cus = prop.multiProcessorCount;
+    if (cus <= 0) return MI355CG_OK;
+    const int per_cu = (c->whole.grid + cus - 1) / cus;
+    if (per_cu > 2) return MI355CG_OK;
+    auto kern = k_cg_chunk<double, 2, 3, 2>;
+    const int row_bytes = kWave * 2 * (int)sizeof(double);
+    const int stage = kChunkStage * (int)sizeof(double);
+    int rows = std::max(0, (kPersistWgLdsBytes - stage) / (kWaves * row_bytes));
+    int ty_max = 0;
+    for (int k = 0; k < c->whole.wl.np; ++k) ty_max = std::max(ty_max, c->whole.wl.p[k].ty);
+    rows = std::min(rows, ty_max);
+    rows = std::min(rows, std::max(0, env_int("MI355CG_PERSIST_ROWS", rows)));
+    if (hipFuncSetAttribute((const void*)kern, hipFuncAttributeMaxDynamicSharedMemorySize, kPersistWgLdsBytes) != hipSuccess) { (void)hipGetLastError(); return MI355CG_OK; }
+    for (;; --rows) {
+        const size_t lds = (size_t)stage + (size_t)rows * kWaves * row_bytes;
+        int nb = 0;
+        if (hipOccupancyMaxActiveBlocksPerMultiprocessor(&nb, kern, kBlock, lds) != hipSuccess) { (void)hipGetLastError(); return MI355CG_OK; }
+        if (std::min(nb, 6) * cus >= c->whole.grid && std::min(nb, 6) >= per_cu) { c->persist_lds = lds; break; }
+        if (rows == 0) return MI355CG_OK;
+    }
+    if (hipMalloc((void**)&c->seam, kSeamBytes) != hipSuccess) { (void)hipGetLastError(); c->seam = nullptr; return MI355CG_OK; }
+    HIPCK(hipMemset(c->seam, 0, kSeamBytes));
+    c->persist_rows = rows;
+    c->persist_tail = env_int("MI355CG_PERSIST_END", 0) != 0 ? 1 : 0;
+    c->persist = true;
+    return MI355CG_OK;
+}
+
+int launch_chunk_persistent(mi355cg_ctx* c, const IterCfg& cfg, int m) {
+    ChunkArgs<double> a{};
+    const Geom g = kernel_geom<double, 2>(c);
+    a.st.g = g; a.st.wl = c->whole.wl;
+    a.st.r = c->r;
+    a.st.partB = c->partB; a.st.nB = c->nB_own; a.st.strideB = c->strideB; a.st.esB = 1;
+    a.st.partA = c->partA; a.st.strideA = c->strideA; a.st.slotA = 0;
+    a.st.s_in = c->sB; a.st.s_out = c->sA; a.st.hist = c->hist; a.st.rp = cfg.rp; a.st.want_diag = 0; a.st.store_ghosts = 0;
+    a.up.r = c->r; a.up.x = c->x; a.up.u = nullptr;
+    a.up.partA = c->partA; a.up.nA = c->whole.grid; a.up.strideA = c->strideA; a.up.esA = 1;
+    a.up.partB = c->partB; a.up.strideB = c->strideB; a.up.slotB = 0;
+    a.up.s_in = c->sA; a.up.s_out = c->sB; a.up.rule = cfg.rp.rule; a.up.reverse = 0;
+    a.up.stop_req = c->stop_dev;
+    for (int k = 0; k < 4; ++k) a.ring[k] = c->p[k];
+    a.cur = c->cur; a.m = m;
+    a.seam = SeamSpec{c->seam, kSeamBudgetTicks};
+    a.res_rows = c->persist_rows; a.res_tail = c->persist_tail;
+    HIPCK(hipMemsetAsync(c->seam, 0, kSeamBytes, c->stream));
+    hipLaunchKernelGGL((k_cg_chunk<double, 2, 3, 2>), dim3(c->whole.grid), dim3(kBlock), c->persist_lds, c->stream, a);
+    c->cur = (c->cur + m) % c->xsteps;
+    return MI355CG_OK;
 }
 
 IterCfg make_cfg(const mi355cg_params* prm) {
@@ -1406,6 +1490,7 @@
     if (hipMalloc((void**)&c->qctr, sizeof(int) * 2 * kXcds * kQueueSubs * kQueuePitch) != hipSuccess || hipMemset(c->qctr, 0, sizeof(int) * 2 * kXcds * kQueueSubs * kQueuePitch) != hipSuccess) { rc = fail(MI355CG_ERR_HIP, "queue counter allocation failed"); return cleanup(); }
     if (hipHostMalloc((void**)&c->stop_h, sizeof(int)) != hipSuccess) { rc = fail(MI355CG_ERR_HIP, "stop word allocation failed"); return cleanup(); }
     *c->stop_h = 0;
+    if (!part && (rc = persist_setup(c))) return cleanup();
     HIPCK(hipDeviceSynchronize());
 
     if (env_int("MI355CG_DEVICE_SETUP", 0)) {
@@ -1507,7 +1592,7 @@
     if (c->stream) hipStreamSynchronize(c->stream);
     void* dev[] = {c->x, c->r, c->p[0], c->p[1], c->p[2], c->p[3], c->p[4], c->p[5], c->p[6], c->p[7], c->ap, c->b, c->u, c->scratch[0], c->scratch[1], c->xf, c->rf,
                    c->pf[0], c->pf[1], c->pf[2], c->pf[3], c->pf[4], c->pf[5], c->pf[6], c->pf[7], c->apf,
-                   c->packed, c->partA, c->partB, c->partR, c->sumsA, c->sumsB, c->sA, c->sB, c->summary, c->hist, c->qctr};
+                   c->packed, c->partA, c->partB, c->partR, c->sumsA, c->sumsB, c->sA, c->sB, c->summary, c->hist, c->qctr, c->seam};
     for (void* p : dev) if (p) hipFree(p);
     if (c->csr_row_map) hipFree(c->csr_row_map);
     if (c->csr_entries) hipFree(c->csr_entries);
@@ -1712,7 +1797,9 @@
             }
             return MI355CG_OK;
         };
-        if (graph_ok && m >= 8) {
+        if (c->persist && cfg.x2 && !c->profiling) {
+            if (int rc = launch_chunk_persistent(c, cfg, m)) return rc;
+        } else if (graph_ok && m >= 8) {
             std::vector<char> flags(m);
             for (int k = 0; k < m; ++k) flags[k] = cfg.has_u && need_u(it_done + k + 1);
             mi355cg_ctx::ChunkGraph* hit = nullptr;
@@ -1738,6 +1825,11 @@
         }
         HIPCK(hipGetLastError());
         if (int rc = poll()) return rc;
+        if (c->summary_h->done && c->summary_h->reason == kReasonTransport) {
+            c->persist = false;
+            c->stop_dev = nullptr;
+            return fail(MI355CG_ERR_STATE, "a grid-wide seam of the persistent chunk launch was not completed within its budget; the handle falls back to two launches per iteration");
+        }
         const int it_now = c->summary_h->it;
         if (cb) for (int it = it_done + 1; it <= it_now; ++it) {
             const HistEntry& h = c->hist_h[it % kHist];
@@ -1838,6 +1930,15 @@
     if (pitch_upper) *pitch_upper = c->g.Pu;
     if (grid_stencil) *grid_stencil = c->whole.grid;
     if (grid_update) *grid_update = c->whole.grid;
+    if (rows_per_item) *rows_per_item = c->whole.ty;
+    return MI355CG_OK;
+}
+
+int mi355cg_get_loop_info(mi355cg_handle c, int* persistent, int* resident_rows, int* rows_per_item) {
+    if (!c) return fail(MI355CG_ERR_INVALID, "null handle");
+    const bool on = c->persist && !c->profiling && !c->mg;
+    if (persistent) *persistent = on ? 1 : 0;
+    if (resident_rows) *resident_rows = on ? c->persist_rows : 0;
     if (rows_per_item) *rows_per_item = c->whole.ty;
     return MI355CG_OK;
 }
diff --git a/iterative_solvers_amd/solver.py b/iterative_solvers_amd/solver.py
--- a/iterative_solvers_amd/solver.py
+++ b/iterative_solvers_amd/solver.py
@@ -198,6 +198,11 @@
         _capi.check(self._lib.mi355cg_get_layout(self._h, C.byref(L), *[C.byref(i) for i in v]))
         return {"padded_len": L.value, "pitch_bottom": v[0].value, "pitch_upper": v[1].value,
                 "grid_stencil": v[2].value, "grid_update": v[3].value, "rows_per_item": v[4].value}
+
+    def loop_info(self):
+        v = [C.c_int() for _ in range(3)]
+        _capi.check(self._lib.mi355cg_get_loop_info(self._h, *[C.byref(i) for i in v]))
+        return {"persistent": v[0].value, "resident_rows": v[1].value, "rows_per_item": v[2].value}
 
 
 def default_params(rule: int) -> _capi.Params:
```

After: 5599 iters/s. 21.6% lower.
